# marvinli00/genie2

Hardware: AMD Instinct MI355X
Metric: denoise-steps/sec (N=256, T=1000, batch=8) (higher is better)
Workload: dtype f32 (pair-stack products as 3 f16 MFMAs on 2xf16-split operands, f32 accumulate); 1 GPU; unconditional N=256, T=1000, batch=8 per GPU, random-init base Denoiser (15.7M params), scale=0.6, reverse-loop steps 995..676; parallelism=replica per GPU x1, no data-path collective

## Files before the change

genie2_amd/csrc/common.h:

```cpp
#pragma once
#include <hip/hip_runtime.h>
#include <stdint.h>
#include "../../include/genie_hip.h"

typedef float f32x16 __attribute__((ext_vector_type(16)));
typedef float f32x4 __attribute__((ext_vector_type(4)));

#define GENIE_LN_EPS 1e-5f

#ifdef __HIPCC__

__device__ __forceinline__ f32x16 mfma_8k(const float4 a, const float4 b, f32x16 c) {
    c = __builtin_amdgcn_mfma_f32_32x32x2f32(a.x, b.x, c, 0, 0, 0);
    c = __builtin_amdgcn_mfma_f32_32x32x2f32(a.y, b.y, c, 0, 0, 0);
    c = __builtin_amdgcn_mfma_f32_32x32x2f32(a.z, b.z, c, 0, 0, 0);
    c = __builtin_amdgcn_mfma_f32_32x32x2f32(a.w, b.w, c, 0, 0, 0);
    return c;
}

__device__ __forceinline__ f32x16 zero16() {
    f32x16 z;
#pragma unroll
    for (int i = 0; i < 16; ++i) z[i] = 0.f;
    return z;
// ... 5 lines not shown
    return *reinterpret_cast<const float4*>(wp + ((size_t)(nb * KB + kb) * 64 + lane) * 4);
}

typedef float v4f __attribute__((ext_vector_type(4)));

__device__ __forceinline__ const float* wfrag_ptr(const float* __restrict__ wp, int KB, int nb, int kb, int lane) {
    return wp + ((size_t)(nb * KB + kb) * 64 + lane) * 4;
}
__device__ __forceinline__ void wf_issue(v4f& d, const float* p) {
    asm volatile("global_load_dwordx4 %0, %1, off" : "=v"(d) : "v"(p) : "memory");
}
template <int N>
__device__ __forceinline__ void wf_wait(v4f& a) {
    asm volatile("s_waitcnt vmcnt(%1)" : "+v"(a) : "i"(N) : "memory");
    __builtin_amdgcn_sched_barrier(0);
}
template <int N>
__device__ __forceinline__ void wf_wait(v4f& a, v4f& b) {
    asm volatile("s_waitcnt vmcnt(%2)" : "+v"(a), "+v"(b) : "i"(N) : "memory");
    __builtin_amdgcn_sched_barrier(0);
}
__device__ __forceinline__ f32x16 mfma_8k(const v4f a, const float4 b, f32x16 c) {
    c = __builtin_amdgcn_mfma_f32_32x32x2f32(a.x, b.x, c, 0, 0, 0);
    c = __builtin_amdgcn_mfma_f32_32x32x2f32(a.y, b.y, c, 0, 0, 0);
    c = __builtin_amdgcn_mfma_f32_32x32x2f32(a.z, b.z, c, 0, 0, 0);
    c = __builtin_amdgcn_mfma_f32_32x32x2f32(a.w, b.w, c, 0, 0, 0);
    return c;
}
__device__ __forceinline__ f32x16 mfma_8k(const float4 a, const v4f b, f32x16 c) {
    c = __builtin_amdgcn_mfma_f32_32x32x2f32(a.x, b.x, c, 0, 0, 0);
    c = __builtin_amdgcn_mfma_f32_32x32x2f32(a.y, b.y, c, 0, 0, 0);
    c = __builtin_amdgcn_mfma_f32_32x32x2f32(a.z, b.z, c, 0, 0, 0);
    c = __builtin_amdgcn_mfma_f32_32x32x2f32(a.w, b.w, c, 0, 0, 0);
    return c;
}

__device__ __forceinline__ float4 lfrag(const float* lds, int ld, int r0, int kb, int lane) {
    return *reinterpret_cast<const float4*>(lds + (r0 + (lane & 31)) * ld + kb * 8 + 4 * (lane >> 5));
}

__device__ __forceinline__ float4 lfrag_t(const float* lds, int ld, int i0, int kb, int lane) {
    const float* p = lds + (kb * 8 + 4 * (lane >> 5)) * ld + i0 + (lane & 31);
    return make_float4(p[0], p[ld], p[2 * ld], p[3 * ld]);
}

__device__ __forceinline__ float sigmoidf_(float x) { return 1.0f / (1.0f + expf(-x)); }

__device__ __forceinline__ void ln_rows_128(float* tile, int ld, const float* __restrict__ gamma,
                                            const float* __restrict__ beta, int tid) {
    const int row = tid >> 2, part = tid & 3;
    float* p = tile + row * ld + part * 32;
    float v[32];
#pragma unroll
    for (int q = 0; q < 8; ++q) {
        float4 t = *reinterpret_cast<float4*>(p + 4 * q);
        v[4 * q] = t.x; v[4 * q + 1] = t.y; v[4 * q + 2] = t.z; v[4 * q + 3] = t.w;
    }
    float s = 0.f;
#pragma unroll
    for (int q = 0; q < 32; ++q) s += v[q];
    s += __shfl_xor(s, 1); s += __shfl_xor(s, 2);
    const float mean = s * (1.0f / 128.0f);
    float ss = 0.f;
#pragma unroll
    for (int q = 0; q < 32; ++q) { float d = v[q] - mean; ss += d * d; }
    ss += __shfl_xor(ss, 1); ss += __shfl_xor(ss, 2);
    const float rstd = 1.0f / sqrtf(ss * (1.0f / 128.0f) + GENIE_LN_EPS);
#pragma unroll
    for (int q = 0; q < 8; ++q) {
        const int c = part * 32 + 4 * q;
        float4 g = *reinterpret_cast<const float4*>(gamma + c);
        float4 b = *reinterpret_cast<const float4*>(beta + c);
        float4 o;
        o.x = (v[4 * q] - mean) * rstd * g.x + b.x;
        o.y = (v[4 * q + 1] - mean) * rstd * g.y + b.y;
        o.z = (v[4 * q + 2] - mean) * rstd * g.z + b.z;
        o.w = (v[4 * q + 3] - mean) * rstd * g.w + b.w;
        *reinterpret_cast<float4*>(p + 4 * q) = o;
    }
}


__device__ __forceinline__ void rot_to_quat_dev(const float* r, int code, float* q) {
    const float xx = r[0], xy = r[1], xz = r[2], yx = r[3], yy = r[4], yz = r[5], zx = r[6], zy = r[7], zz = r[8];
    const float d0 = 1.f + xx + yy + zz, d1 = 1.f + xx - yy - zz, d2 = 1.f + yy - xx - zz, d3 = 1.f + zz - xx - yy;
    float c0, c1, c2, c3;
    if (d0 >= d1 && d0 >= d2 && d0 >= d3)      { c0 = d0;      c1 = zy - yz; c2 = xz - zx; c3 = yx - xy; }
    else if (d1 >= d2 && d1 >= d3)             { c0 = zy - yz; c1 = d1;      c2 = xy + yx; c3 = xz + zx; }
    else if (d2 >= d3)                         { c0 = xz - zx; c1 = xy + yx; c2 = d2;      c3 = yz + zy; }
    else                                       { c0 = yx - xy; c1 = xz + zx; c2 = yz + zy; c3 = d3; }
    const float inv = 1.0f / sqrtf(c0 * c0 + c1 * c1 + c2 * c2 + c3 * c3);
    q[0] = c0 * inv; q[1] = c1 * inv; q[2] = c2 * inv; q[3] = c3 * inv;
    if (code > 0) {
        const int m = (code - 1) >> 1;
        const bool want_neg = ((code - 1) & 1) != 0;
        const float comp = q[m];
        if ((comp < 0.f) != want_neg) { q[0] = -q[0]; q[1] = -q[1]; q[2] = -q[2]; q[3] = -q[3]; }
    }
}

#endif


enum KernelClass {
    KC_SINGLE_INPUT = 0, KC_GEMM_ROWS, KC_LAYERNORM, KC_PAIR_STATIC, KC_PAIR_INIT,
    KC_TRIMUL_PROJ, KC_TRIMUL_CONTRACT, KC_TRIMUL_OUT, KC_PAIR_TRANSITION,
    KC_IPA_BIAS, KC_IPA_PREP, KC_IPA_ATTN, KC_BB_UPDATE, KC_STRUCT_ROWS, KC_P_SAMPLE, KC_MISC, KC_PAIR_FUSED_A, KC_PAIR_FUSED_B,
    KC_TR_GEMM, KC_TR_EW, KC_TR_LN, KC_TR_TRANSPOSE, KC_TR_IPA, KC_TR_MISC,
    KC_TRIATT_PROJ, KC_TRIATT_CORE, KC_TRIATT_TRANSPOSE, KC_COUNT
};

struct HxTransW { const unsigned char* img; float *b1s, *b2s; float sx, c1, c2; };

struct HxTriW {
    const unsigned char *img_proj, *img_out;
    float *bias_proj, *bgs, *bzs;
    float sx, cpa, cpb, cg, cx, cgo, cz;
};
struct HxFusedW { const unsigned char* img; };
struct TriMulW {
    float *proj_w;
    float *proj_b;
    float *g_w, *g_b;
    float *z_w, *z_b;
    float *ln_in_g, *ln_in_b, *ln_out_g, *ln_out_b;
    HxTriW hx;
};
struct TriAttW {
    float *ln_g, *ln_b;
    float *wb;
    float *proj_w, *proj_b;
    float *out_w, *out_b;
    float sq, sk, sv;
};
struct PairLayerW {
    TriMulW out, in;
    TriAttW ta_start, ta_end;
    float *pt_ln_g, *pt_ln_b, *pt_w1, *pt_b1, *pt_w2, *pt_b2;
    HxTransW hx_pt;
    HxFusedW fa, fb;
};
struct StructLayerW {
    float *proj_w, *proj_b;
    float *head_w;
    float *out_w, *out_b;
    float *ln_ipa_g, *ln_ipa_b;
    float *t1_w, *t1_b, *t2_w, *t2_b, *t3_w, *t3_b;
    float *ln_tr_g, *ln_tr_b;
    float *bb_w, *bb_b;
};

struct HxGemmW { const float* w; const unsigned char* img; float inv_s; };

struct genie_train_ws;
struct genie_ctx {
    genie_dims_t d;
    genie_train_ws* train;
    int device;
    char err[512];

    bool have_weights;
    float* wdev;
    bool hx;
    unsigned char* hxdev;
    HxGemmW hxg[128]; int n_hxg;
    unsigned hx_launches;
    size_t wdev_floats;
    float *single_w;
    float *pij_w;
    float *relpos_t;
    float *templ_w;
    float *motif_w;
    float *ipa_bias_w, *ipa_bias_b;
    PairLayerW* pair;
    StructLayerW* st;

    bool have_tables;
    float *pos_tab, *chain_tab, *t_tab, *sched;
    int n_pos, n_chain;
    float* sched_host;

    int B, N, NP;
    bool have_feats, has_motif;
    int32_t *f_aatype, *f_rmask, *f_ridx, *f_cidx;
    float *f_pos;
    uint8_t *f_fsm, *f_fstm, *f_ifm;
    float *rmaskf;

    void* ws; size_t ws_bytes;
    float *p, *acm, *bcm, *xcm, *pstatic, *ipa_bias;
    float *spart;
    unsigned *pmax;
    float *xsingle, *s0, *s, *s1, *s2, *h1, *h2, *pij, *proj, *cat;
    float *kT, *v, *qp, *kpT, *vp;
    float *vf, *vmax;
    float *ta_tb, *ta_xn, *ta_qkvg;
    float *rots_w, *trans_w;
    int32_t* tsteps;
    float *loop_z;

    bool prof;
    struct ProfRec { int cls; hipEvent_t a, b; };
    ProfRec* prof_recs; int prof_n, prof_cap;
    double prof_ms[KC_COUNT]; int64_t prof_cnt[KC_COUNT];
    double train_gemm_flop;

    hipStream_t st2; hipEvent_t ev_fork, ev_join;
};

void launch_single_input(genie_ctx* h, hipStream_t st, const int32_t* timesteps);
void launch_gemm_rows(genie_ctx* h, hipStream_t st, const float* A, int lda, int M, int K,
                      const float* Wp, int Nout, const float* bias, const float* res, int ldr,
                      const float* rowmask, int relu, float* out, int ldo, int prof_class = KC_GEMM_ROWS);
void launch_layernorm_rows(genie_ctx* h, hipStream_t st, const float* in, float* out, int M, int C,
                           const float* g, const float* b);
void launch_pair_static(genie_ctx* h, hipStream_t st);
void launch_pair_init(genie_ctx* h, hipStream_t st, const float* trans, const float* rots,
                      const int8_t* codes);
void launch_trimul(genie_ctx* h, hipStream_t st, const TriMulW& w, bool outgoing);
void launch_pair_transition(genie_ctx* h, hipStream_t st, const PairLayerW& w);
void launch_triatt(genie_ctx* h, hipStream_t st, const TriAttW& w, bool starting);
void triatt_ws_floats(const genie_dims_t& d, int B, int N, size_t* tb, size_t* xn, size_t* qkvg);
bool launch_pair_stack_fused(genie_ctx* h, hipStream_t st, float* tap_trimul_out0, float* tap_layer0);
void launch_ipa_bias(genie_ctx* h, hipStream_t st);
void launch_ipa_prep(genie_ctx* h, hipStream_t st, int b0 = 0, int nb = -1);
void launch_ipa_attn(genie_ctx* h, hipStream_t st, int layer, const float* head_w, int b0 = 0, int nb = -1);
size_t ipa_vf_floats(const genie_dims_t& d, int B, int N);
bool ipa_attn_splits(const genie_ctx* h);
void launch_q_sample(genie_ctx* h, hipStream_t st, const float* x0, const float* z, const float* c0, const float* c1, float* trans_out);
void launch_training_loss(genie_ctx* h, hipStream_t st, const float* zp, const float* z, float w, float* losses, float* grad);
void launch_adam(hipStream_t st, size_t n, float* p, const float* g, float* m, float* v, double lr, double b1, double b2, double eps, int step);
void launch_any_nonzero(genie_ctx* h, hipStream_t st, const uint8_t* x, size_t n, unsigned* flag);
bool launch_struct_tail(genie_ctx* h, hipStream_t st, const StructLayerW& S, const float* trans_in, float* z_out, int b0 = 0, int nb = -1);
bool struct_tail_fused(const genie_ctx* h, const StructLayerW& S);
void launch_bb_update(genie_ctx* h, hipStream_t st, const StructLayerW& w, const float* trans_in,
                      float* z_out);
void launch_frenet(genie_ctx* h, hipStream_t st, int mode, int step, float scale, float* trans,
                   float* rots, const float* z, const float* eps);
void launch_reverse_step(genie_ctx* h, hipStream_t st, float a, float bz, float c_scaled, float* trans, float* rots, const float* z,
                         const float* eps);
void launch_fill_i32(genie_ctx* h, hipStream_t st, int32_t* p, int n, int v);
void train_ws_free(genie_ctx* h);

void prof_begin(genie_ctx* h, hipStream_t st, int cls);
void prof_end(genie_ctx* h, hipStream_t st);

struct ProfScope {
    genie_ctx* h; hipStream_t st; bool on;
    ProfScope(genie_ctx* h_, hipStream_t st_, int cls, bool enable = true) : h(h_), st(st_), on(enable && h_->prof) { if (on) prof_begin(h, st, cls); }
    ~ProfScope() { if (on) prof_end(h, st); }
};
```

genie2_amd/csrc/genie_api.hip:

```cpp
#include <stdio.h>
#include <stdlib.h>
#include <string.h>
#include <math.h>
#include <algorithm>
#include <cmath>
#include <new>
#include <string>
#include <vector>

#include "common.h"

void pair_kernels_init();
void pair_fused_kernels_init();
void single_kernels_init(const genie_dims_t& d, int n_max);
void launch_scale_copy(genie_ctx* h, hipStream_t st, const float* in, float* out, int n, float s);
size_t ipa_attn_lds(const genie_dims_t& d, int N);

static char g_create_err[512] = "";

void set_handle_free_error(const char* msg) { snprintf(g_create_err, sizeof g_create_err, "%s", msg); }

#define SET_ERR(h, ...) do { snprintf((h)->err, sizeof((h)->err), __VA_ARGS__); } while (0)
#define HIP_TRY(h, call) do { hipError_t e_ = (call); if (e_ != hipSuccess) { \
    SET_ERR(h, "%s failed: %s (%s:%d)", #call, hipGetErrorString(e_), __FILE__, __LINE__); return GENIE_E_HIP; } } while (0)

static const char* kKernelNames[KC_COUNT] = {
    "single_input", "gemm_rows", "layernorm_rows", "pair_static", "pair_init", "trimul_proj", "trimul_contract",
    "trimul_out", "pair_transition", "ipa_bias", "ipa_prep", "ipa_attn", "bb_update", "struct_rows", "p_sample_frenet", "misc",
    "pair_fused_a", "pair_fused_b", "train_gemm", "train_elementwise", "train_layernorm", "train_transpose", "train_ipa", "train_misc",
    "tri_att_proj", "tri_att_core", "tri_att_transpose"};

void prof_begin(genie_ctx* h, hipStream_t st, int cls) {
    if (h->prof_n == h->prof_cap) {
        const int nc = h->prof_cap ? h->prof_cap * 2 : 1024;
        h->prof_recs = (genie_ctx::ProfRec*)realloc(h->prof_recs, nc * sizeof(genie_ctx::ProfRec));
        h->prof_cap = nc;
    }
    genie_ctx::ProfRec& r = h->prof_recs[h->prof_n];
    r.cls = cls;
    (void)hipEventCreate(&r.a);
    (void)hipEventCreate(&r.b);
    (void)hipEventRecord(r.a, st);
}
void prof_end(genie_ctx* h, hipStream_t st) {
    (void)hipEventRecord(h->prof_recs[h->prof_n].b, st);
    h->prof_n++;
}

static int single_in(const genie_dims_t& d) { return d.c_pos_emb + d.c_chain_emb + d.c_timestep_emb + 23; }
static int ipa_proj_n(const genie_dims_t& d) {
    return d.n_head_ipa * (3 * d.c_hidden_ipa + 3 * d.n_qk_point + 3 * (d.n_qk_point + d.n_v_point));
}
static int ipa_cat_n(const genie_dims_t& d) { return d.n_head_ipa * (d.c_p + d.c_hidden_ipa + 4 * d.n_v_point); }

static const char* check_dims(const genie_dims_t& d) {
    if (d.c_p != 128 || d.c_hidden_mul != 128) return "kernels are specialised for c_p == c_hidden_mul == 128";
    if (d.c_s % 8 || d.c_s > 512) return "c_s must be a multiple of 8 and <= 512";
    if (d.template_dist_n_bin > 40 || d.template_dist_n_bin < 1) return "template_dist_n_bin must be in [1, 40]";
    if (d.n_head_ipa > 16) return "n_head_ipa must be <= 16";
    if (d.pair_transition_n < 1 || d.n_timestep < 1 || d.relpos_k < 0) return "bad dims";
    if (d.n_structure_layer < 1 || d.n_structure_block < 1 || d.n_pair_transform_layer < 0) return "bad layer counts";
    if ((d.n_head_ipa * d.c_hidden_ipa) % 4 || ipa_cat_n(d) % 4 || ipa_proj_n(d) % 4) return "IPA widths must be multiples of 4";
    if (d.n_head_tri < 0) return "n_head_tri must be >= 0";
    if (d.n_head_tri > 0 && d.c_hidden_tri_att != 16 && d.c_hidden_tri_att != 32) return "c_hidden_tri_att must be 16 or 32";
    if (d.n_head_tri > 0 && d.n_head_tri * d.c_hidden_tri_att != 128) return "n_head_tri * c_hidden_tri_att must be 128 (4 heads of 32 or 8 of 16)";
    return nullptr;
}

size_t genie_weight_count(const genie_dims_t* dp) {
    const genie_dims_t& d = *dp;
    size_t n = 0;
    const size_t cs = d.c_s, cp = d.c_p, ch = d.c_hidden_mul;
    n += cs * single_in(d);
    n += 2 * cp * cs + cp * (2 * d.relpos_k + 3) + cp * (d.template_dist_n_bin + 6) + cp * (d.template_dist_n_bin + 2);
    const size_t tm = 4 * (ch * cp + ch) + (cp * cp + cp) + (cp * ch + cp) + 2 * cp + 2 * ch;
    const size_t pt = 2 * cp + (d.pair_transition_n * cp * cp + d.pair_transition_n * cp) + (cp * d.pair_transition_n * cp + cp);
    const size_t hc = (size_t)d.n_head_tri * d.c_hidden_tri_att;
    const size_t ta = d.n_head_tri > 0 ? 2 * cp + d.n_head_tri * cp + 3 * hc * cp + (cp * hc + cp) + (hc * cp + hc) : 0;
    n += (size_t)d.n_pair_transform_layer * (2 * tm + 2 * ta + pt);
    const size_t H = d.n_head_ipa, C = d.c_hidden_ipa, Pq = d.n_qk_point, Pv = d.n_v_point;
    size_t sl = H;
    sl += (H * C) * cs + H * C + (2 * H * C) * cs + 2 * H * C + (3 * H * Pq) * cs + 3 * H * Pq + (3 * H * (Pq + Pv)) * cs + 3 * H * (Pq + Pv);
    sl += H * cp + H + cs * ipa_cat_n(d) + cs;
    sl += 2 * cs + 3 * (cs * cs + cs) + 2 * cs + 6 * cs + 6;
    n += (size_t)d.n_structure_layer * sl;
    return n;
}

int genie_create(const genie_dims_t* dims, int device, genie_handle_t* out) {
    if (!dims || !out) { snprintf(g_create_err, sizeof g_create_err, "genie_create: null argument"); return GENIE_E_ARG; }
    if (const char* m = check_dims(*dims)) { snprintf(g_create_err, sizeof g_create_err, "genie_create: %s", m); return GENIE_E_ARG; }
    int ndev = 0;
    if (hipGetDeviceCount(&ndev) != hipSuccess || device < 0 || device >= ndev) {
        snprintf(g_create_err, sizeof g_create_err, "genie_create: no HIP device %d (found %d)", device, ndev);
        return GENIE_E_HIP;
    }
    genie_ctx* h = new (std::nothrow) genie_ctx();
    if (!h) return GENIE_E_NOMEM;
    memset(h, 0, sizeof(*h));
    h->d = *dims;
    h->device = device;
    if (hipSetDevice(device) != hipSuccess) { delete h; snprintf(g_create_err, sizeof g_create_err, "hipSetDevice failed"); return GENIE_E_HIP; }
    h->pair = new PairLayerW[dims->n_pair_transform_layer > 0 ? dims->n_pair_transform_layer : 1]();
    h->st = new StructLayerW[dims->n_structure_layer]();
    pair_kernels_init();
    pair_fused_kernels_init();
    {
        const char* m = getenv("GENIE_MATH");
        h->hx = !(m && !strcmp(m, "f32"));
    }
    {
        int lo = 0, hi = 0;
        (void)hipDeviceGetStreamPriorityRange(&lo, &hi);
        if (hipStreamCreateWithPriority(&h->st2, hipStreamNonBlocking, hi) != hipSuccess) h->st2 = nullptr;
    }
    if (h->st2 && (hipEventCreateWithFlags(&h->ev_fork, hipEventDisableTiming) != hipSuccess ||
                   hipEventCreateWithFlags(&h->ev_join, hipEventDisableTiming) != hipSuccess)) {
        (void)hipStreamDestroy(h->st2);
        h->st2 = nullptr;
    }
    *out = h;
    return GENIE_OK;
}

static void free_batch(genie_ctx* h) {
    if (h->ws) { (void)hipFree(h->ws); h->ws = nullptr; h->ws_bytes = 0; }
    h->have_feats = false;
}

void genie_destroy(genie_handle_t h) {
    if (!h) return;
    (void)hipSetDevice(h->device);
    free_batch(h);
    train_ws_free(h);
    if (h->wdev) (void)hipFree(h->wdev);
    if (h->hxdev) (void)hipFree(h->hxdev);
    if (h->pos_tab) (void)hipFree(h->pos_tab);
    free(h->sched_host);
    for (int i = 0; i < h->prof_n; ++i) { (void)hipEventDestroy(h->prof_recs[i].a); (void)hipEventDestroy(h->prof_recs[i].b); }
    free(h->prof_recs);
    if (h->st2) { (void)hipStreamSynchronize(h->st2); (void)hipEventDestroy(h->ev_fork); (void)hipEventDestroy(h->ev_join); (void)hipStreamDestroy(h->st2); }
    delete[] h->pair;
    delete[] h->st;
    delete h;
}

const char* genie_last_error(genie_handle_t h) { return h ? h->err : g_create_err; }
size_t genie_workspace_bytes(genie_handle_t h) { return h ? h->ws_bytes : 0; }

namespace {
struct Img {
    std::vector<float> data;
    size_t add(size_t n) {
        const size_t off = (data.size() + 63) & ~(size_t)63;
        data.resize(off + n, 0.f);
        return off;
    }
    size_t raw(const float* src, size_t n) { const size_t o = add(n); memcpy(&data[o], src, n * sizeof(float)); return o; }
    size_t pack(const float* W, int rows, int cols) {
        const int NB = (rows + 31) / 32, KB = (cols + 7) / 8;
        const size_t o = add((size_t)NB * KB * 256);
        float* p = &data[o];
        for (int nb = 0; nb < NB; ++nb)
            for (int kb = 0; kb < KB; ++kb)
                for (int lane = 0; lane < 64; ++lane)
                    for (int e = 0; e < 4; ++e) {
                        const int r = nb * 32 + (lane & 31), k = kb * 8 + 4 * (lane >> 5) + e;
                        p[(((size_t)nb * KB + kb) * 64 + lane) * 4 + e] = (r < rows && k < cols) ? W[(size_t)r * cols + k] : 0.f;
                    }
        return o;
    }
};
uint16_t f2h(float f) {
    uint32_t x; memcpy(&x, &f, 4);
    const uint16_t sign = (uint16_t)((x >> 16) & 0x8000);
    x &= 0x7FFFFFFFu;
    if (x >= 0x7F800000u) return (uint16_t)(sign | (x > 0x7F800000u ? 0x7E00 : 0x7C00));
    if (x >= 0x477FF000u) return (uint16_t)(sign | 0x7C00);
    if (x < 0x38800000u) {
        float a; memcpy(&a, &x, 4);
        return (uint16_t)(sign | (uint16_t)nearbyintf(a * 16777216.0f));
    }
    const uint32_t mant = x & 0x7FFFFFu, rem = mant & 0x1FFFu;
    uint32_t r = (((x >> 23) - 112u) << 10) | (mant >> 13);
    if (rem > 0x1000u || (rem == 0x1000u && (r & 1u))) ++r;
    return (uint16_t)(sign | r);
}
float h2f(uint16_t v) {
    const int e = (v >> 10) & 31, m = v & 1023;
    float r = e == 0 ? ldexpf((float)m, -24) : e == 31 ? (m ? NAN : INFINITY) : ldexpf((float)(1024 + m), e - 25);
    return (v & 0x8000) ? -r : r;
}
float p2floor(double x) { return (x > 0 && std::isfinite(x)) ? (float)ldexp(1.0, (int)floor(log2(x))) : 1.0f; }
struct HxImg {
    std::vector<uint16_t> d;
    size_t begin() { d.resize((d.size() + 127) & ~(size_t)127); return d.size() * 2; }
    template <class F> void unit(F get) {
        const size_t o = d.size();
        d.resize(o + 1024);
        for (int lane = 0; lane < 64; ++lane)
            for (int e = 0; e < 8; ++e) {
                const float v = get(lane & 31, lane >> 5, e);
                const uint16_t hi = f2h(v);
                d[o + lane * 8 + e] = hi;
                d[o + 512 + lane * 8 + e] = f2h(v - h2f(hi));
            }
    }
};
double max_abs(const float* w, size_t n) { double m = 0; for (size_t i = 0; i < n; ++i) m = std::max(m, (double)fabsf(w[i])); return m; }
double hx_bound(const float* W, const float* b, int rows, int cols) {
    double m = 0;
    for (int r = 0; r < rows; ++r) {
        double ss = 0;
        for (int k = 0; k < cols; ++k) ss += (double)W[(size_t)r * cols + k] * W[(size_t)r * cols + k];
        m = std::max(m, sqrt(ss * cols) + fabs((double)b[r]));
    }
    return m;
}
constexpr float HX_SX = 1024.0f;

struct Cur {
    const float* p; size_t left;
    const float* take(size_t n) { if (n > left) { left = 0; return nullptr; } const float* r = p; p += n; left -= n; return r; }
};
void fold_ln(std::vector<float>& W, std::vector<float>& b, int rows, int cols, const float* g, const float* beta) {
    for (int r = 0; r < rows; ++r) {
        double acc = b[r];
        for (int k = 0; k < cols; ++k) acc += (double)W[(size_t)r * cols + k] * beta[k];
        b[r] = (float)acc;
        for (int k = 0; k < cols; ++k) W[(size_t)r * cols + k] *= g[k];
    }
}
std::vector<float> vcat(std::initializer_list<std::pair<const float*, size_t>> parts) {
    std::vector<float> v;
    for (auto& pr : parts) v.insert(v.end(), pr.first, pr.first + pr.second);
    return v;
}
}

int genie_load_weights(genie_handle_t h, const float* blob, size_t n_floats) {
    if (!h || !blob) return GENIE_E_ARG;
    const genie_dims_t& d = h->d;
    if (n_floats != genie_weight_count(&d)) {
        SET_ERR(h, "genie_load_weights: got %zu floats, dims need %zu", n_floats, genie_weight_count(&d));
        return GENIE_E_ARG;
    }
    HIP_TRY(h, hipSetDevice(h->device));
    const size_t cs = d.c_s, cp = d.c_p, ch = d.c_hidden_mul;
    Cur c{blob, n_floats};
    Img img;
    HxImg hx;
    std::vector<std::pair<float**, size_t>> fix;
    std::vector<std::pair<const unsigned char**, size_t>> hxfix;
    auto slot = [&](float** s, size_t off) { fix.push_back({s, off}); };
    struct GemmFix { float** slot; size_t hx_off; float inv_s; };
    std::vector<GemmFix> gfix;
    auto pack_gemm = [&](float** s, const float* W, int rows, int cols) {
        slot(s, img.pack(W, rows, cols));
        const float sw = p2floor(16384.0 / max_abs(W, (size_t)rows * cols));
        gfix.push_back({s, hx.begin(), 1.0f / sw});
        const int NB = (rows + 31) / 32, KC = (cols + 15) / 16;
        for (int nb = 0; nb < NB; ++nb)
            for (int kc = 0; kc < KC; ++kc)
                hx.unit([&](int j, int hh, int e) {
                    const int r = 32 * nb + j, k = 16 * kc + 8 * hh + e;
                    return (r < rows && k < cols) ? W[(size_t)r * cols + k] * sw : 0.f; });
    };

    size_t ones_off, zeros_off;
    {
        std::vector<float> one(512, 1.f), zero(512, 0.f);
        ones_off = img.raw(one.data(), one.size());
        zeros_off = img.raw(zero.data(), zero.size());
    }
    const int nsi = single_in(d);
    pack_gemm(&h->single_w, c.take(cs * nsi), (int)cs, nsi);
    {
        const float* wi = c.take(cp * cs);
        const float* wj = c.take(cp * cs);
        auto v = vcat({{wi, cp * cs}, {wj, cp * cs}});
        pack_gemm(&h->pij_w, v.data(), (int)(2 * cp), (int)cs);
    }
    {
        const int nr = 2 * d.relpos_k + 3;
        const float* w = c.take(cp * nr);
        std::vector<float> t((size_t)nr * cp);
        for (int o = 0; o < (int)cp; ++o) for (int k = 0; k < nr; ++k) t[(size_t)k * cp + o] = w[(size_t)o * nr + k];
        slot(&h->relpos_t, img.raw(t.data(), t.size()));
    }
    {
        const int kt = d.template_dist_n_bin + 6, km = d.template_dist_n_bin + 2;
        const float* wt = c.take(cp * kt);
        const float* wm = c.take(cp * km);
        std::vector<float> t((size_t)cp * 48, 0.f), m((size_t)cp * 48, 0.f);
// ... 128 lines not shown
    {
        auto ck = [](int kc, int hh, int e) { return 16 * kc + (e & 3) + 8 * (e >> 2) + 4 * hh; };
        auto emit_O = [&](const TmSave& t) {
            for (int which = 0; which < 2; ++which)
                for (int st = 0; st < 2; ++st)
                    for (int obl = 0; obl < 2; ++obl)
                        for (int kc = 0; kc < 8; ++kc) {
                            const std::vector<float>& m = which == 0 ? t.zw : t.gw;
                            const float sc = which == 0 ? t.szo : t.sgo;
                            const size_t ob = 2 * st + obl;
                            hx.unit([&](int i, int hh, int e) { return m[(32 * ob + i) * cp + ck(kc, hh, e)] * sc; });
                        }
        };
        auto emit_T = [&](const PtSave& t) {
            const size_t nh = (size_t)d.pair_transition_n * cp;
            for (size_t hb = 0; hb < nh / 32; ++hb) {
                for (int kc = 0; kc < 8; ++kc)
                    hx.unit([&](int i, int hh, int e) { return t.w1v[(32 * hb + i) * cp + ck(kc, hh, e)] * t.s1; });
                for (int cc = 0; cc < 2; ++cc)
                    for (int ob = 0; ob < 4; ++ob)
                        hx.unit([&](int j, int hh, int e) { return t.w2[(size_t)(32 * ob + j) * nh + 32 * hb + ck(cc, hh, e)] * t.s2; });
            }
        };
        auto emit_P = [&](const TmSave& t) {
            for (size_t pass = 0; pass < 8; ++pass)
                for (int kc = 0; kc < 8; ++kc) {
                    hx.unit([&](int i, int hh, int e) { return t.w[(32 * pass + i) * cp + ck(kc, hh, e)] * t.sp; });
                    hx.unit([&](int i, int hh, int e) { return t.w[(2 * ch + 32 * pass + i) * cp + ck(kc, hh, e)] * t.sg; });
                }
        };
        for (int l = 0; l < d.n_pair_transform_layer; ++l) {
            hxfix.push_back({&h->pair[l].fa.img, hx.begin()});
            emit_O(tm_save[2 * l]); emit_P(tm_save[2 * l + 1]);
            hxfix.push_back({&h->pair[l].fb.img, hx.begin()});
            emit_O(tm_save[2 * l + 1]); emit_T(pt_save[l]);
            if (l + 1 < d.n_pair_transform_layer) emit_P(tm_save[2 * l + 2]);
        }
    }
    const size_t H = d.n_head_ipa, C = d.c_hidden_ipa, Pq = d.n_qk_point, Pv = d.n_v_point;
    const size_t ncat = ipa_cat_n(d);
    std::vector<float> wb_all, bb_all;
    for (int l = 0; l < d.n_structure_layer; ++l) {
        StructLayerW& S = h->st[l];
        const float* hw = c.take(H);
        const float* q_w = c.take(H * C * cs);            const float* q_b = c.take(H * C);
        const float* kv_w = c.take(2 * H * C * cs);       const float* kv_b = c.take(2 * H * C);
        const float* qp_w = c.take(3 * H * Pq * cs);      const float* qp_b = c.take(3 * H * Pq);
        const float* kp_w = c.take(3 * H * (Pq + Pv) * cs); const float* kp_b = c.take(3 * H * (Pq + Pv));
        const float* b_w = c.take(H * cp);                const float* b_b = c.take(H);
        const float* o_w = c.take(cs * ncat);             const float* o_b = c.take(cs);
        const float* li_g = c.take(cs); const float* li_b = c.take(cs);
        const float* t1w = c.take(cs * cs); const float* t1b = c.take(cs);
        const float* t2w = c.take(cs * cs); const float* t2b = c.take(cs);
        const float* t3w = c.take(cs * cs); const float* t3b = c.take(cs);
        const float* lt_g = c.take(cs); const float* lt_b = c.take(cs);
        const float* bw = c.take(6 * cs); const float* bbs = c.take(6);
        if (!bbs) { SET_ERR(h, "genie_load_weights: blob too short"); return GENIE_E_ARG; }
        slot(&S.head_w, img.raw(hw, H));
        auto w = vcat({{q_w, H * C * cs}, {kv_w, 2 * H * C * cs}, {qp_w, 3 * H * Pq * cs}, {kp_w, 3 * H * (Pq + Pv) * cs}});
        auto bv = vcat({{q_b, H * C}, {kv_b, 2 * H * C}, {qp_b, 3 * H * Pq}, {kp_b, 3 * H * (Pq + Pv)}});
        pack_gemm(&S.proj_w, w.data(), ipa_proj_n(d), (int)cs);
        slot(&S.proj_b, img.raw(bv.data(), bv.size()));
        wb_all.insert(wb_all.end(), b_w, b_w + H * cp);
        bb_all.insert(bb_all.end(), b_b, b_b + H);
        pack_gemm(&S.out_w, o_w, (int)cs, (int)ncat); slot(&S.out_b, img.raw(o_b, cs));
        slot(&S.ln_ipa_g, img.raw(li_g, cs)); slot(&S.ln_ipa_b, img.raw(li_b, cs));
        pack_gemm(&S.t1_w, t1w, (int)cs, (int)cs); slot(&S.t1_b, img.raw(t1b, cs));
        pack_gemm(&S.t2_w, t2w, (int)cs, (int)cs); slot(&S.t2_b, img.raw(t2b, cs));
        pack_gemm(&S.t3_w, t3w, (int)cs, (int)cs); slot(&S.t3_b, img.raw(t3b, cs));
        slot(&S.ln_tr_g, img.raw(lt_g, cs)); slot(&S.ln_tr_b, img.raw(lt_b, cs));
        slot(&S.bb_w, img.raw(bw, 6 * cs)); slot(&S.bb_b, img.raw(bbs, 6));
    }
    pack_gemm(&h->ipa_bias_w, wb_all.data(), (int)(d.n_structure_layer * H), (int)cp);
    slot(&h->ipa_bias_b, img.raw(bb_all.data(), bb_all.size()));
    if (c.left != 0) { SET_ERR(h, "genie_load_weights: %zu floats left over", c.left); return GENIE_E_ARG; }

    if (h->wdev) { (void)hipFree(h->wdev); h->wdev = nullptr; }
    img.add(64);
    HIP_TRY(h, hipMalloc((void**)&h->wdev, img.data.size() * sizeof(float)));
    HIP_TRY(h, hipMemcpy(h->wdev, img.data.data(), img.data.size() * sizeof(float), hipMemcpyHostToDevice));
    h->wdev_floats = img.data.size();
    for (auto& f : fix) *f.first = h->wdev + f.second;
    if (h->hxdev) { (void)hipFree(h->hxdev); h->hxdev = nullptr; }
    hx.begin();
    HIP_TRY(h, hipMalloc((void**)&h->hxdev, hx.d.size() * 2 + 256));
    HIP_TRY(h, hipMemcpy(h->hxdev, hx.d.data(), hx.d.size() * 2, hipMemcpyHostToDevice));
    for (auto& f : hxfix) *f.first = h->hxdev + f.second;
    h->n_hxg = 0;
    const int hxg_cap = (int)(sizeof(h->hxg) / sizeof(h->hxg[0]));
    if ((int)gfix.size() > hxg_cap) { SET_ERR(h, "genie_load_weights: %zu row-GEMM weights exceed the %d hx image slots", gfix.size(), hxg_cap); return GENIE_E_ARG; }
    for (auto& g : gfix) h->hxg[h->n_hxg++] = HxGemmW{*g.slot, h->hxdev + g.hx_off, g.inv_s};
    h->have_weights = true;
    return GENIE_OK;
}

int genie_set_tables(genie_handle_t h, const float* pos_tab, int n_pos, const float* chain_tab, int n_chain,
                     const float* t_tab, const float* sched) {
    if (!h || !pos_tab || !chain_tab || !t_tab || !sched || n_pos < 1 || n_chain < 1) return GENIE_E_ARG;
    HIP_TRY(h, hipSetDevice(h->device));
    const genie_dims_t& d = h->d;
    const size_t T1 = d.n_timestep + 1;
    const size_t a = (size_t)n_pos * d.c_pos_emb, b = (size_t)n_chain * d.c_chain_emb, c = T1 * d.c_timestep_emb, s = 4 * T1;
    if (h->pos_tab) (void)hipFree(h->pos_tab);
    HIP_TRY(h, hipMalloc((void**)&h->pos_tab, (a + b + c + s) * sizeof(float)));
    h->chain_tab = h->pos_tab + a;
    h->t_tab = h->chain_tab + b;
    h->sched = h->t_tab + c;
    HIP_TRY(h, hipMemcpy(h->pos_tab, pos_tab, a * sizeof(float), hipMemcpyHostToDevice));
    HIP_TRY(h, hipMemcpy(h->chain_tab, chain_tab, b * sizeof(float), hipMemcpyHostToDevice));
    HIP_TRY(h, hipMemcpy(h->t_tab, t_tab, c * sizeof(float), hipMemcpyHostToDevice));
    HIP_TRY(h, hipMemcpy(h->sched, sched, s * sizeof(float), hipMemcpyHostToDevice));
    free(h->sched_host);
    h->sched_host = (float*)malloc(s * sizeof(float));
    memcpy(h->sched_host, sched, s * sizeof(float));
    h->n_pos = n_pos;
    h->n_chain = n_chain;
    h->have_tables = true;
    return GENIE_OK;
}

__global__ void k_mask_to_float(const int32_t* m, float* f, int n) {
    const int i = blockIdx.x * blockDim.x + threadIdx.x;
    if (i < n) f[i] = (float)m[i];
}

int genie_prepare_features(genie_handle_t h, genie_stream_t stream, int B, int N, const genie_features_t* f) {
    if (!h || !f || B < 1 || N < 2) return GENIE_E_ARG;
    if (!h->have_weights) { SET_ERR(h, "genie_prepare_features: weights not loaded"); return GENIE_E_STATE; }
    const genie_dims_t& d = h->d;
    if (ipa_attn_lds(d, N) > 160 * 1024) { SET_ERR(h, "N = %d exceeds the attention kernel's LDS budget", N); return GENIE_E_ARG; }
    if ((size_t)24 * N * sizeof(float) > 160 * 1024) { SET_ERR(h, "N = %d exceeds the Frenet kernel's LDS budget (96 B per residue)", N); return GENIE_E_ARG; }
    {
        const size_t np = (size_t)((N + 31) / 32 * 32);
        const size_t pair_bytes = (size_t)B * np * np * d.c_p * sizeof(float);
        if (pair_bytes >= ((size_t)1 << 31)) {
            SET_ERR(h, "batch %d x N %d: a pair tensor of %zu bytes exceeds the 2 GiB the kernels address; split the batch", B, N, pair_bytes);
            return GENIE_E_ARG;
        }
    }
    HIP_TRY(h, hipSetDevice(h->device));
    hipStream_t st = (hipStream_t)stream;
    const int NP = (N + 31) / 32 * 32;
    const size_t M = (size_t)B * N, P = M * N;
    const size_t cs = d.c_s, cp = d.c_p;
    const int H = d.n_head_ipa, C = d.c_hidden_ipa, Pq = d.n_qk_point, Pv = d.n_v_point;
    const int ldx = (single_in(d) + 7) / 8 * 8;

    struct Seg { void** p; size_t bytes; };
    std::vector<Seg> segs;
    auto want = [&](void* pp, size_t bytes) { segs.push_back({(void**)pp, (bytes + 255) & ~(size_t)255}); };
    want(&h->p, P * cp * 4); want(&h->pstatic, P * cp * 4);
    want(&h->acm, (size_t)B * cp * NP * NP * 4); want(&h->bcm, (size_t)B * cp * NP * NP * 4); want(&h->xcm, (size_t)B * cp * NP * NP * 4);
    want(&h->ipa_bias, (size_t)d.n_structure_layer * H * P * 4);
    want(&h->xsingle, M * ldx * 4);
    want(&h->s0, M * cs * 4); want(&h->s, M * cs * 4); want(&h->s1, M * cs * 4); want(&h->s2, M * cs * 4);
    want(&h->h1, M * cs * 4); want(&h->h2, M * cs * 4);
    want(&h->pij, M * 2 * cp * 4); want(&h->proj, M * ipa_proj_n(d) * 4); want(&h->cat, M * ipa_cat_n(d) * 4);
    want(&h->kT, M * H * C * 4); want(&h->v, M * H * C * 4); want(&h->qp, M * H * Pq * 3 * 4);
    want(&h->kpT, M * H * Pq * 3 * 4); want(&h->vp, M * H * Pv * 3 * 4);
    want(&h->vf, ipa_vf_floats(d, B, N) * 4); want(&h->vmax, M * 2 * 4);
    want(&h->rots_w, M * 9 * 4); want(&h->trans_w, M * 3 * 4); want(&h->loop_z, M * 3 * 4);
    want(&h->tsteps, (size_t)B * 4); want(&h->rmaskf, M * 4); want(&h->pmax, 4); want(&h->spart, 3 * M * cs * 4);
    want(&h->f_aatype, M * 20 * 4); want(&h->f_rmask, M * 4); want(&h->f_ridx, M * 4); want(&h->f_cidx, M * 4);
    want(&h->f_pos, M * 3 * 4); want(&h->f_fsm, M); want(&h->f_fstm, P); want(&h->f_ifm, M);
    if (d.n_head_tri > 0) {
        size_t ntb, nxn, nq;
        triatt_ws_floats(d, B, N, &ntb, &nxn, &nq);
        want(&h->ta_tb, ntb * 4); want(&h->ta_xn, nxn * 4); want(&h->ta_qkvg, nq * 4);
    }
    size_t total = 0;
    for (auto& s : segs) total += s.bytes;
    if (total > h->ws_bytes) {
        free_batch(h);
        hipError_t e = hipMalloc(&h->ws, total);
        if (e != hipSuccess) { SET_ERR(h, "workspace hipMalloc(%zu MB) failed: %s", total >> 20, hipGetErrorString(e)); return GENIE_E_NOMEM; }
        h->ws_bytes = total;
    }
    size_t off = 0;
    for (auto& s : segs) { *s.p = (char*)h->ws + off; off += s.bytes; }
    h->B = B; h->N = N; h->NP = NP;

    HIP_TRY(h, hipMemcpyAsync(h->f_aatype, f->aatype, M * 20 * 4, hipMemcpyDeviceToDevice, st));
    HIP_TRY(h, hipMemcpyAsync(h->f_pos, f->atom_positions, M * 3 * 4, hipMemcpyDeviceToDevice, st));
    HIP_TRY(h, hipMemcpyAsync(h->f_rmask, f->residue_mask, M * 4, hipMemcpyDeviceToDevice, st));
    HIP_TRY(h, hipMemcpyAsync(h->f_ridx, f->residue_index, M * 4, hipMemcpyDeviceToDevice, st));
    HIP_TRY(h, hipMemcpyAsync(h->f_cidx, f->chain_index, M * 4, hipMemcpyDeviceToDevice, st));
    HIP_TRY(h, hipMemcpyAsync(h->f_fsm, f->fixed_sequence_mask, M, hipMemcpyDeviceToDevice, st));
    HIP_TRY(h, hipMemcpyAsync(h->f_fstm, f->fixed_structure_mask, P, hipMemcpyDeviceToDevice, st));
    HIP_TRY(h, hipMemcpyAsync(h->f_ifm, f->interface_mask, M, hipMemcpyDeviceToDevice, st));
    hipLaunchKernelGGL(k_mask_to_float, dim3((unsigned)((M + 255) / 256)), dim3(256), 0, st, h->f_rmask, h->rmaskf, (int)M);
    HIP_TRY(h, hipMemsetAsync(h->acm, 0, (size_t)B * cp * NP * NP * 4, st));
    HIP_TRY(h, hipMemsetAsync(h->vf, 0, ipa_vf_floats(d, B, N) * 4, st));
    HIP_TRY(h, hipMemsetAsync(h->bcm, 0, (size_t)B * cp * NP * NP * 4, st));
    single_kernels_init(d, N);
    {
        unsigned any = 0;
        HIP_TRY(h, hipMemsetAsync(h->pmax, 0, sizeof(unsigned), st));
        launch_any_nonzero(h, st, h->f_fstm, P, h->pmax);
        HIP_TRY(h, hipMemcpyAsync(&any, h->pmax, sizeof(unsigned), hipMemcpyDeviceToHost, st));
        HIP_TRY(h, hipStreamSynchronize(st));
        h->has_motif = any != 0;
    }
    launch_pair_static(h, st);
    HIP_TRY(h, hipGetLastError());
    h->have_feats = true;
    return GENIE_OK;
}

static int denoise_internal(genie_ctx* h, hipStream_t st, const float* trans, const float* rots, const int32_t* ts_dev,
                            const int8_t* codes, float* z_out, const genie_taps_t* taps) {
    const genie_dims_t& d = h->d;
    const int B = h->B, N = h->N, M = B * N;
    const size_t P = (size_t)M * N;
    const int cs = d.c_s, cp = d.c_p;
    const int ldx = (single_in(d) + 7) / 8 * 8;
    auto d2d = [&](void* dst, const void* src, size_t bytes) { return hipMemcpyAsync(dst, src, bytes, hipMemcpyDeviceToDevice, st); };

    h->hx_launches = 1;
    launch_scale_copy(h, st, trans, h->trans_w, M * 3, d.rescale);
    HIP_TRY(h, d2d(h->rots_w, rots, (size_t)M * 9 * 4));

    launch_single_input(h, st, ts_dev);
    launch_gemm_rows(h, st, h->xsingle, ldx, M, ldx, h->single_w, cs, nullptr, nullptr, 0, h->rmaskf, 0, h->s0, cs);
    if (taps && taps->s) HIP_TRY(h, d2d(taps->s, h->s0, (size_t)M * cs * 4));

    launch_gemm_rows(h, st, h->s0, cs, M, cs, h->pij_w, 2 * cp, nullptr, nullptr, 0, nullptr, 0, h->pij, 2 * cp);
    launch_pair_init(h, st, h->trans_w, h->rots_w, codes);
    if (taps && taps->p_init) HIP_TRY(h, d2d(taps->p_init, h->p, P * cp * 4));

    const bool fused = launch_pair_stack_fused(h, st, taps ? taps->p_trimul_out0 : nullptr, taps ? taps->p_layer0 : nullptr);
    for (int l = 0; l < (fused ? 0 : d.n_pair_transform_layer); ++l) {
        launch_trimul(h, st, h->pair[l].out, true);
        if (l == 0 && taps && taps->p_trimul_out0) HIP_TRY(h, d2d(taps->p_trimul_out0, h->p, P * cp * 4));
        launch_trimul(h, st, h->pair[l].in, false);
        if (d.n_head_tri > 0) {
            launch_triatt(h, st, h->pair[l].ta_start, true);
            launch_triatt(h, st, h->pair[l].ta_end, false);
            if (l == 0 && taps && taps->p_tri_att0) HIP_TRY(h, d2d(taps->p_tri_att0, h->p, P * cp * 4));
        }
        launch_pair_transition(h, st, h->pair[l]);
        if (l == 0 && taps && taps->p_layer0) HIP_TRY(h, d2d(taps->p_layer0, h->p, P * cp * 4));
    }
    if (taps && taps->p) HIP_TRY(h, d2d(taps->p, h->p, P * cp * 4));

    launch_ipa_bias(h, st);
    HIP_TRY(h, d2d(h->s, h->s0, (size_t)M * cs * 4));
    if (taps && taps->states) HIP_TRY(h, d2d(taps->states, h->s0, (size_t)M * cs * 4));
    int n_state = 1;
    const int nproj = ipa_proj_n(d), ncat = ipa_cat_n(d);
    bool split = h->st2 && B >= 2 && M >= 1024 && ipa_attn_splits(h) && !getenv("GENIE_NO_STRUCT_SPLIT");
    for (int l = 0; split && l < d.n_structure_layer; ++l) split = struct_tail_fused(h, h->st[l]);
    const int n_half = split ? 2 : 1;
    const int n_layers = d.n_structure_block * d.n_structure_layer;
    hipStream_t hstream[2] = {st, h->st2};
    if (split) {
        HIP_TRY(h, hipEventRecord(h->ev_fork, st));
        HIP_TRY(h, hipStreamWaitEvent(h->st2, h->ev_fork, 0));
    }
    for (int half = 0; half < n_half; ++half) {
        hipStream_t hs = hstream[half];
        const int b0 = (int)((long long)B * half / n_half), nb = (int)((long long)B * (half + 1) / n_half) - b0;
        const size_t r0 = (size_t)b0 * N, nr = (size_t)nb * N;
        int li = 0;
        for (int blk = 0; blk < d.n_structure_block; ++blk) {
            for (int l = 0; l < d.n_structure_layer; ++l, ++li) {
                const StructLayerW& S = h->st[l];
                const bool last = li == n_layers - 1;
                launch_gemm_rows(h, hs, h->s + r0 * cs, cs, (int)nr, cs, S.proj_w, nproj, S.proj_b, nullptr, 0, nullptr, 0, h->proj + r0 * nproj, nproj);
                launch_ipa_prep(h, hs, b0, nb);
                launch_ipa_attn(h, hs, l, S.head_w, b0, nb);
                if (li == 0 && taps && taps->ipa_cat0) HIP_TRY(h, hipMemcpyAsync(taps->ipa_cat0 + r0 * ncat, h->cat + r0 * ncat, nr * ncat * 4, hipMemcpyDeviceToDevice, hs));
                auto state_tap = [&]() -> hipError_t {
                    return (taps && taps->states) ? hipMemcpyAsync(taps->states + (size_t)(1 + li) * M * cs + r0 * cs, h->s + r0 * cs, nr * cs * 4, hipMemcpyDeviceToDevice, hs)
                                                  : hipSuccess;
                };
                if (launch_struct_tail(h, hs, S, last ? trans : nullptr, last ? z_out : nullptr, b0, nb)) { HIP_TRY(h, state_tap()); continue; }
                launch_gemm_rows(h, hs, h->cat, ncat, M, ncat, S.out_w, cs, S.out_b, h->s, cs, nullptr, 0, h->s1, cs);
                launch_layernorm_rows(h, hs, h->s1, h->s2, M, cs, S.ln_ipa_g, S.ln_ipa_b);
                launch_gemm_rows(h, hs, h->s2, cs, M, cs, S.t1_w, cs, S.t1_b, nullptr, 0, nullptr, 1, h->h1, cs);
                launch_gemm_rows(h, hs, h->h1, cs, M, cs, S.t2_w, cs, S.t2_b, nullptr, 0, nullptr, 1, h->h2, cs);
                launch_gemm_rows(h, hs, h->h2, cs, M, cs, S.t3_w, cs, S.t3_b, h->s2, cs, nullptr, 0, h->s1, cs);
                launch_layernorm_rows(h, hs, h->s1, h->s, M, cs, S.ln_tr_g, S.ln_tr_b);
                launch_bb_update(h, hs, S, last ? trans : nullptr, last ? z_out : nullptr);
                HIP_TRY(h, state_tap());
            }
        }
    }
    if (split) {
        for (int q = 1; q < n_half; ++q) {
            HIP_TRY(h, hipEventRecord(h->ev_join, hstream[q]));
            HIP_TRY(h, hipStreamWaitEvent(st, h->ev_join, 0));
        }
    }
    (void)n_state;
    if (taps && taps->s_final) HIP_TRY(h, d2d(taps->s_final, h->s, (size_t)M * cs * 4));
    if (taps && taps->rots_out) HIP_TRY(h, d2d(taps->rots_out, h->rots_w, (size_t)M * 9 * 4));
    if (taps && taps->trans_out) launch_scale_copy(h, st, h->trans_w, taps->trans_out, M * 3, 1.0f / d.rescale);
    HIP_TRY(h, hipGetLastError());
    return GENIE_OK;
}

static int check_ready(genie_ctx* h, const char* who) {
    if (!h) return GENIE_E_ARG;
    if (!h->have_weights || !h->have_tables || !h->have_feats) {
        SET_ERR(h, "%s: call genie_load_weights, genie_set_tables and genie_prepare_features first", who);
        return GENIE_E_STATE;
    }
    if (hipSetDevice(h->device) != hipSuccess) { SET_ERR(h, "hipSetDevice failed"); return GENIE_E_HIP; }
    return GENIE_OK;
}

int genie_denoise(genie_handle_t h, genie_stream_t stream, const float* trans, const float* rots, const int32_t* timesteps,
                  const int8_t* quat_codes, float* z_out, const genie_taps_t* taps) {
    if (int rc = check_ready(h, "genie_denoise")) return rc;
    if (!trans || !rots || !timesteps || !z_out) { SET_ERR(h, "genie_denoise: null tensor"); return GENIE_E_ARG; }
    return denoise_internal(h, (hipStream_t)stream, trans, rots, timesteps, quat_codes, z_out, taps);
}

int genie_frenet(genie_handle_t h, genie_stream_t stream, const float* trans, float* rots_out) {
    if (!h || !h->have_feats) { if (h) SET_ERR(h, "genie_frenet: no batch bound"); return h ? GENIE_E_STATE : GENIE_E_ARG; }
    if (!trans || !rots_out) return GENIE_E_ARG;
    HIP_TRY(h, hipSetDevice(h->device));
    launch_frenet(h, (hipStream_t)stream, 0, 0, 0.f, const_cast<float*>(trans), rots_out, nullptr, nullptr);
    HIP_TRY(h, hipGetLastError());
    return GENIE_OK;
}

int genie_adam_step(genie_stream_t stream, size_t n, float* p, const float* g, float* m, float* v, double lr, double beta1, double beta2,
                    double eps, int step) {
    if (!p || !g || !m || !v || step < 1) return GENIE_E_ARG;
    if (n == 0) return GENIE_OK;
    launch_adam((hipStream_t)stream, n, p, g, m, v, lr, beta1, beta2, eps, step);
    return hipGetLastError() == hipSuccess ? GENIE_OK : GENIE_E_HIP;
}

int genie_q_sample(genie_handle_t h, genie_stream_t stream, const float* x0, const float* z, const float* c_x0, const float* c_z,
                   float* trans_out, float* rots_out) {
    if (!h || !h->have_feats) { if (h) SET_ERR(h, "genie_q_sample: no batch bound"); return h ? GENIE_E_STATE : GENIE_E_ARG; }
    if (!x0 || !z || !c_x0 || !c_z || !trans_out || !rots_out) { SET_ERR(h, "genie_q_sample: null tensor"); return GENIE_E_ARG; }
    HIP_TRY(h, hipSetDevice(h->device));
    launch_q_sample(h, (hipStream_t)stream, x0, z, c_x0, c_z, trans_out);
    launch_frenet(h, (hipStream_t)stream, 0, 0, 0.f, trans_out, rots_out, nullptr, nullptr);
    HIP_TRY(h, hipGetLastError());
    return GENIE_OK;
}

int genie_training_loss(genie_handle_t h, genie_stream_t stream, const float* z_pred, const float* z, float condition_loss_weight,
                        float* losses_out, float* grad_out) {
    if (!h || !h->have_feats) { if (h) SET_ERR(h, "genie_training_loss: no batch bound"); return h ? GENIE_E_STATE : GENIE_E_ARG; }
    if (!z_pred || !z || !losses_out) { SET_ERR(h, "genie_training_loss: null tensor"); return GENIE_E_ARG; }
    HIP_TRY(h, hipSetDevice(h->device));
    launch_training_loss(h, (hipStream_t)stream, z_pred, z, condition_loss_weight, losses_out, grad_out);
    HIP_TRY(h, hipGetLastError());
    return GENIE_OK;
}

int genie_p_sample(genie_handle_t h, genie_stream_t stream, int step, float scale, float* trans_inout, float* rots_out,
                   const float* z, const float* eps) {
    if (int rc = check_ready(h, "genie_p_sample")) return rc;
    if (step < 1 || step > h->d.n_timestep || !trans_inout || !rots_out || !z) { SET_ERR(h, "genie_p_sample: bad argument"); return GENIE_E_ARG; }
    launch_frenet(h, (hipStream_t)stream, 1, step, scale, trans_inout, rots_out, z, eps);
    HIP_TRY(h, hipGetLastError());
    return GENIE_OK;
}

int genie_sample_loop(genie_handle_t h, genie_stream_t stream, float scale, const float* noise, const int8_t* quat_codes,
                      int first_step, int last_step, float* trans_io, float* rots_io, float* record) {
    if (int rc = check_ready(h, "genie_sample_loop")) return rc;
    const int T = h->d.n_timestep;
    if (!noise || !trans_io || !rots_io || first_step > T || last_step < 1 || first_step < last_step) {
        SET_ERR(h, "genie_sample_loop: bad argument");
        return GENIE_E_ARG;
    }
    hipStream_t st = (hipStream_t)stream;
    const size_t n3 = (size_t)h->B * h->N * 3, nn = (size_t)h->B * h->N * h->N;
    if (first_step == T) {
        HIP_TRY(h, hipMemcpyAsync(trans_io, noise, n3 * 4, hipMemcpyDeviceToDevice, st));
        launch_frenet(h, st, 0, 0, 0.f, trans_io, rots_io, nullptr, nullptr);
    }
    int it = 0;
    for (int step = first_step; step >= last_step; --step, ++it) {
        launch_fill_i32(h, st, h->tsteps, h->B, step);
        const int8_t* codes = quat_codes ? quat_codes + (size_t)it * nn : nullptr;
        if (int rc = denoise_internal(h, st, trans_io, rots_io, h->tsteps, codes, h->loop_z, nullptr)) return rc;
        const float* eps = (step == 1) ? nullptr : noise + (size_t)(T - step + 1) * n3;
        launch_frenet(h, st, 1, step, scale, trans_io, rots_io, h->loop_z, eps);
        if (record) HIP_TRY(h, hipMemcpyAsync(record + (size_t)it * n3, trans_io, n3 * 4, hipMemcpyDeviceToDevice, st));
    }
    HIP_TRY(h, hipGetLastError());
    return GENIE_OK;
}

int genie_reverse_step(genie_handle_t h, genie_stream_t stream, float a, float bz, float c_scaled, float* trans_inout, float* rots_out,
                       const float* z, const float* eps) {
    if (int rc = check_ready(h, "genie_reverse_step")) return rc;
    if (!trans_inout || !rots_out || !z) { SET_ERR(h, "genie_reverse_step: null tensor"); return GENIE_E_ARG; }
    if (!std::isfinite(a) || !std::isfinite(bz) || !std::isfinite(c_scaled)) {
        SET_ERR(h, "genie_reverse_step: non-finite coefficient (a = %g, bz = %g, c_scaled = %g)", a, bz, c_scaled);
        return GENIE_E_ARG;
    }
    launch_reverse_step(h, (hipStream_t)stream, a, bz, c_scaled, trans_inout, rots_out, z, eps);
    HIP_TRY(h, hipGetLastError());
    return GENIE_OK;
}

int genie_sample_loop_steps(genie_handle_t h, genie_stream_t stream, int n_iter, const int32_t* steps, const float* coef, const float* noise,
                            const int8_t* quat_codes, int start_from_noise, float* trans_io, float* rots_io, float* record) {
    if (int rc = check_ready(h, "genie_sample_loop_steps")) return rc;
    const int T = h->d.n_timestep;
    if (n_iter < 1) { SET_ERR(h, "genie_sample_loop_steps: n_iter = %d, needs at least 1", n_iter); return GENIE_E_ARG; }
    if (!steps || !coef || !trans_io || !rots_io) { SET_ERR(h, "genie_sample_loop_steps: null steps, coef, trans_io or rots_io"); return GENIE_E_ARG; }
    if (!noise && (start_from_noise || n_iter > 1)) {
        SET_ERR(h, "genie_sample_loop_steps: null noise (needed for the initial state and for every iteration but the last)");
        return GENIE_E_ARG;
    }
    for (int i = 0; i < n_iter; ++i) {
        if (steps[i] < 1 || steps[i] > T) { SET_ERR(h, "genie_sample_loop_steps: steps[%d] = %d outside 1..%d", i, steps[i], T); return GENIE_E_ARG; }
        if (i && steps[i] >= steps[i - 1]) {
            SET_ERR(h, "genie_sample_loop_steps: steps not strictly decreasing (steps[%d] = %d after %d)", i, steps[i], steps[i - 1]);
            return GENIE_E_ARG;
        }
        for (int k = 0; k < 3; ++k)
            if (!std::isfinite(coef[3 * i + k])) { SET_ERR(h, "genie_sample_loop_steps: non-finite coefficient coef[%d][%d]", i, k); return GENIE_E_ARG; }
    }
    hipStream_t st = (hipStream_t)stream;
    const size_t n3 = (size_t)h->B * h->N * 3, nn = (size_t)h->B * h->N * h->N;
    if (start_from_noise) {
        HIP_TRY(h, hipMemcpyAsync(trans_io, noise, n3 * 4, hipMemcpyDeviceToDevice, st));
        launch_frenet(h, st, 0, 0, 0.f, trans_io, rots_io, nullptr, nullptr);
    }
    for (int it = 0; it < n_iter; ++it) {
        launch_fill_i32(h, st, h->tsteps, h->B, steps[it]);
        const int8_t* codes = quat_codes ? quat_codes + (size_t)it * nn : nullptr;
        if (int rc = denoise_internal(h, st, trans_io, rots_io, h->tsteps, codes, h->loop_z, nullptr)) return rc;
        const float* eps = (it == n_iter - 1) ? nullptr : noise + (size_t)(it + 1) * n3;
        launch_reverse_step(h, st, coef[3 * it], coef[3 * it + 1], coef[3 * it + 2], trans_io, rots_io, h->loop_z, eps);
        if (record) HIP_TRY(h, hipMemcpyAsync(record + (size_t)it * n3, trans_io, n3 * 4, hipMemcpyDeviceToDevice, st));
    }
    HIP_TRY(h, hipGetLastError());
    return GENIE_OK;
}

int genie_set_math(genie_handle_t h, int mode) {
    if (!h || (mode != GENIE_MATH_F32 && mode != GENIE_MATH_HX)) return GENIE_E_ARG;
    h->hx = mode == GENIE_MATH_HX;
    return GENIE_OK;
}
int genie_get_math(genie_handle_t h) { return h && h->hx ? GENIE_MATH_HX : GENIE_MATH_F32; }

int genie_profile_enable(genie_handle_t h, int enable) {
    if (!h) return GENIE_E_ARG;
    h->prof = enable != 0;
    return GENIE_OK;
}

int genie_profile_read(genie_handle_t h, const char** names, double* total_ms, int64_t* launches, int cap) {
    if (!h) return GENIE_E_ARG;
    (void)hipSetDevice(h->device);
    for (int i = 0; i < h->prof_n; ++i) {
        genie_ctx::ProfRec& r = h->prof_recs[i];
        (void)hipEventSynchronize(r.b);
        float ms = 0.f;
        if (hipEventElapsedTime(&ms, r.a, r.b) == hipSuccess) { h->prof_ms[r.cls] += ms; h->prof_cnt[r.cls] += 1; }
        (void)hipEventDestroy(r.a);
        (void)hipEventDestroy(r.b);
    }
    h->prof_n = 0;
    int n = 0;
    for (int k = 0; k < KC_COUNT && n < cap; ++k) {
        if (names) names[n] = kKernelNames[k];
        if (total_ms) total_ms[n] = h->prof_ms[k];
        if (launches) launches[n] = h->prof_cnt[k];
        ++n;
    }
    for (int k = 0; k < KC_COUNT; ++k) { h->prof_ms[k] = 0; h->prof_cnt[k] = 0; }
    return n;
}
```

genie2_amd/csrc/genie_train.hip:

```cpp
#include <math.h>
#include <stdio.h>
#include <string.h>
#include <vector>
#include "common.h"
#include "train.h"

namespace {
struct TriOff { size_t ap_w, ap_b, ag_w, ag_b, bp_w, bp_b, bg_w, bg_b, g_w, g_b, z_w, z_b, lni_g, lni_b, lno_g, lno_b; };
struct PairOff { TriOff out, in; size_t ln_g, ln_b, w1, b1, w2, b2; };
struct StructOff {
    size_t head, q_w, q_b, kv_w, kv_b, qp_w, qp_b, kvp_w, kvp_b, b_w, b_b, o_w, o_b, ln1_g, ln1_b, t1w, t1b, t2w, t2b, t3w, t3b, ln2_g, ln2_b,
        bb_w, bb_b;
};
struct Offs { size_t single_w, wi, wj, wrel, wt, wm; std::vector<PairOff> pair; std::vector<StructOff> st; size_t total; };

Offs make_offsets(const genie_dims_t& d) {
    Offs o;
    size_t c = 0;
    auto take = [&](size_t n) { const size_t r = c; c += n; return r; };
    const size_t cs = d.c_s, cp = d.c_p, ch = d.c_hidden_mul;
    const size_t nsi = d.c_pos_emb + d.c_chain_emb + d.c_timestep_emb + 23;
    o.single_w = take(cs * nsi);
    o.wi = take(cp * cs); o.wj = take(cp * cs);
    o.wrel = take(cp * (2 * d.relpos_k + 3));
// ... 21 lines not shown
        s.kv_w = take(2 * H * C * cs); s.kv_b = take(2 * H * C);
        s.qp_w = take(3 * H * Pq * cs); s.qp_b = take(3 * H * Pq);
        s.kvp_w = take(3 * H * (Pq + Pv) * cs); s.kvp_b = take(3 * H * (Pq + Pv));
        s.b_w = take(H * cp); s.b_b = take(H);
        s.o_w = take(cs * ncat); s.o_b = take(cs);
        s.ln1_g = take(cs); s.ln1_b = take(cs);
        s.t1w = take(cs * cs); s.t1b = take(cs); s.t2w = take(cs * cs); s.t2b = take(cs); s.t3w = take(cs * cs); s.t3b = take(cs);
        s.ln2_g = take(cs); s.ln2_b = take(cs);
        s.bb_w = take(6 * cs); s.bb_b = take(6);
        o.st.push_back(s);
    }
    o.total = c;
    return o;
}

struct Arena {
    char* base = nullptr; size_t off = 0, peak = 0; bool dry = true;
    float* f(size_t n) {
        const size_t bytes = (n * sizeof(float) + 255) & ~(size_t)255;
        float* r = dry ? nullptr : reinterpret_cast<float*>(base + off);
        off += bytes;
        if (off > peak) peak = off;
        return r;
    }
};

struct TriSave { float *xhat, *rstd, *ap, *ag, *bp, *bg, *acm, *bcm, *xhat_o, *rstd_o, *u, *g; };
struct TransSave { float *xhat, *rstd, *h; unsigned* hmask; };
struct PairSave { TriSave out, in; TransSave tr; };
struct StructSave {
    float *s_in, *q, *kv, *qplin, *kvplin, *qp, *kp, *vp, *att, *cat, *xhat1, *rstd1, *s2, *h1, *h2, *xhat2, *rstd2, *s4, *bb, *R, *T;
};
}

struct genie_train_ws { void* kept = nullptr; size_t kept_bytes = 0; void* tmp = nullptr; size_t tmp_bytes = 0; FoldEntry* fold_tab = nullptr; int fold_n = 0; };

void train_ws_free(genie_ctx* h) {
    if (!h->train) return;
    if (h->train->kept) (void)hipFree(h->train->kept);
    if (h->train->tmp) (void)hipFree(h->train->tmp);
    if (h->train->fold_tab) (void)hipFree(h->train->fold_tab);
    delete h->train;
    h->train = nullptr;
}

#define TR_ERR(...) do { snprintf(h->err, sizeof(h->err), __VA_ARGS__); } while (0)

namespace {
struct Run {
    genie_ctx* h; hipStream_t st; bool dry; int terms;
    const float* W; float* G;
    Arena K, T;
    int B, N, M; long long P;

    void gemm(const GemmP& p) {
        if (dry) return;
        h->train_gemm_flop += 2.0 * p.M * p.N * (double)p.K * p.batch;
        ProfScope ps_(h, st, KC_TR_GEMM);
        launch_gemm(st, p, terms);
    }
    void lin_fwd(const float* X, long long ldx, long long R, int K, size_t w, long long b_off, int O, float* Y, int mode = 0, bool relu = false) {
        GemmP p{X, W + w, Y, b_off >= 0 ? W + b_off : nullptr, (int)R, O, K, ldx, 1, 1, K, O, 1, 1, 1, 0, 0, 0, 0, 0, 0, 1, 1.0f, mode};
        p.relu = relu ? 1 : 0;
        gemm(p);
    }
    void lin_bwd_x(const float* dY, long long R, int O, size_t w, int K, float* dX, long long lddx, bool accumulate, const float* relu_out = nullptr,
                   const unsigned* relu_mask = nullptr) {
        GemmP p{dY, W + w, dX, nullptr, (int)R, K, O, O, 1, K, 1, lddx, 1, 1, 1, 0, 0, 0, 0, 0, 0, 1, 1.0f, accumulate ? 1 : 0};
        if (relu_mask) p.mask_in = relu_mask;
        else p.gate = relu_out;
        gemm(p);
    }
    void lin_bwd_x_ptr(const float* dY, long long R, int O, const float* Wc, int K, float* dX, long long lddx) {
        GemmP p{dY, Wc, dX, nullptr, (int)R, K, O, O, 1, K, 1, lddx, 1, 1, 1, 0, 0, 0, 0, 0, 0, 1, 1.0f, 0};
        gemm(p);
    }
    void lin_bwd_w(const float* dY, long long R, int O, const float* X, long long ldx, int K, size_t w, long long b_off) {
        if (!G) return;
        GemmP p{dY, X, G + w, nullptr, O, K, (int)R, 1, O, ldx, 1, K, 1, 1, 1, 0, 0, 0, 0, 0, 0, gemm_splits(O, K, R, 1), 1.0f, 2};
        p.asum = b_off >= 0 ? G + b_off : nullptr;
        gemm(p);
    }
    void lin_fwd_ln(const float* Xhat, long long R, int K, int O, float* Y, const float* fold, bool relu = false, const float* fold_b = nullptr,
                    unsigned* mask_out = nullptr) {
        GemmP p{Xhat, fold, Y, fold_b ? fold_b : fold ? fold + (size_t)O * K : nullptr, (int)R, O, K, K, 1, 1, K, O, 1, 1, 1, 0, 0, 0, 0, 0, 0, 1, 1.0f, 0};
        p.relu = relu ? 1 : 0;
        p.mask_out = mask_out;
        gemm(p);
    }
    void lin_fwd_ln_cat(const float* Xhat, long long R, int K, int O, int nb, float* const* Y, const float* fold, const float* fold_b) {
        GemmP p{Xhat, fold, Y[0], fold_b, (int)R, nb * O, K, K, 1, 1, K, O, 1, 1, 1, 0, 0, 0, 0, 0, 0, 1, 1.0f, 0};
        p.cblk = O; p.cblk_m = 0;
        for (int k = 0; k < nb; ++k) p.ctab[k] = Y[k] - Y[0];
        gemm(p);
    }
    void lin_bwd_w_ln(const float* dY, long long R, int O, const float* Xhat, int K, size_t w, size_t b_off, size_t g_off, size_t beta_off, long long lddy = 0) {
        if (!G) return;
        GemmP p{dY, Xhat, G + w, nullptr, O, K, (int)R, 1, lddy ? lddy : O, K, 1, K, 1, 1, 1, 0, 0, 0, 0, 0, 0, gemm_splits(O, K, R, 1), 1.0f, 2};
        p.asum = G + b_off;
        p.colscale = W + g_off;
        gemm(p);
    }
    void lin_bwd_w_ln_cat(const float* dYcat, long long R, int O, int nb, const float* Xhat, int K, const size_t* w, const size_t* b_off, size_t g_off,
                          size_t beta_off) {
        if (!G) return;
        GemmP p{dYcat, Xhat, G, nullptr, nb * O, K, (int)R, 1, (long long)nb * O, K, 1, K, 1, 1, 1, 0, 0, 0, 0, 0, 0, gemm_splits((long long)nb * O, K, R, 1), 1.0f, 2};
        p.asum = G;
        p.colscale = W + g_off;
        p.cblk = O; p.cblk_m = 1;
        for (int k = 0; k < nb; ++k) { p.ctab[k] = (long long)w[k]; p.atab[k] = (long long)b_off[k]; }
        gemm(p);
    }
    void ln_fwd(const float* x, size_t g, size_t b, float* y, float* xhat, float* rstd, long long R, int C) {
        if (dry) return;
        ProfScope ps_(h, st, KC_TR_LN);
        launch_ln_fwd(st, x, W + g, W + b, y, xhat, rstd, R, C);
    }
    void ln_bwd(const float* dy, const float* xhat, const float* rstd, size_t g, size_t b, float* dx, long long R, int C, bool accumulate) {
        if (dry) return;
        ProfScope ps_(h, st, KC_TR_LN);
        launch_ln_bwd(st, dy, xhat, rstd, W + g, dx, R, C, accumulate ? 1 : 0, G ? G + g : nullptr, G ? G + b : nullptr);
    }
    template <class F> void ew(long long n, F f) { if (dry) return; ProfScope ps_(h, st, KC_TR_EW); launch_ew(st, n, f); }
    void transpose(const float* in, float* out, int Bt, int R, int C, bool to_cm) { if (dry) return; ProfScope ps_(h, st, KC_TR_TRANSPOSE); launch_transpose(st, in, out, Bt, R, C, to_cm); }
};
}

static int train_run(genie_ctx* h, hipStream_t st, bool dry, const float* Wd, float* Gd, const float* trans0, const float* rots0,
                     const int32_t* ts_dev, const float* z_target, const int8_t* codes, float cond_w, const genie_train_opts_t& opt,
                     float* losses_out, float* z_pred_out, size_t* kept_bytes, size_t* tmp_bytes, const float* dz_in = nullptr,
                     float* dtrans_out = nullptr) {
    const genie_dims_t& d = h->d;
    const Offs O = make_offsets(d);
    Run r;
    r.h = h; r.st = st; r.dry = dry; r.terms = opt.fast_math == 1 ? 1 : (opt.fast_math == 2 ? 2 : 3); r.W = Wd; r.G = Gd;
    r.B = h->B; r.N = h->N; r.M = h->B * h->N; r.P = (long long)r.M * h->N;
    r.K.dry = r.T.dry = dry;
    if (!dry) { r.K.base = (char*)h->train->kept; r.T.base = (char*)h->train->tmp; }
    const int B = r.B, N = r.N, M = r.M;
    const long long P = r.P;
    const int cs = d.c_s, cp = d.c_p, ch = d.c_hidden_mul;
    const int nh = d.pair_transition_n * cp;
    const int H = d.n_head_ipa, C = d.c_hidden_ipa, Pq = d.n_qk_point, Pv = d.n_v_point;
    const int ncat = H * (cp + C + 4 * Pv);
    const int nbin = d.template_dist_n_bin, kt = nbin + 6, km = nbin + 2, kr = 2 * d.relpos_k + 3, nf = kt + km + kr;
    const int nsi = d.c_pos_emb + d.c_chain_emb + d.c_timestep_emb + 23, ldx = (nsi + 7) / 8 * 8;
    const bool train = opt.train_mode != 0;
    const float r_tri = train ? opt.tri_dropout : 0.f, r_ipa = train ? opt.ipa_dropout : 0.f, r_tr = train ? opt.transition_dropout : 0.f;
    const uint32_t seed = opt.seed;
    const float* rm = h->rmaskf;
    const int L = d.n_pair_transform_layer, SL = d.n_structure_layer;
    Arena& K = r.K; Arena& T = r.T;

    if (!dry) launch_single_input(h, st, ts_dev);
    const float* xs = h->xsingle;
    float* tr = K.f((size_t)M * 3);
    { const float sc = d.rescale; r.ew((long long)M * 3, [=] __device__(long long i) { tr[i] = trans0[i] * sc; }); }
    float* s0 = K.f((size_t)M * cs);
    r.lin_fwd(xs, ldx, M, nsi, O.single_w, -1, cs, s0);
    r.ew((long long)M * cs, [=] __device__(long long i) { s0[i] *= rm[i / cs]; });
    float* Fm = K.f((size_t)P * nf);
    if (!dry) launch_pair_features(st, tr, rots0, codes, rm, h->f_fstm, h->f_fsm, h->f_pos, h->f_ridx, h->f_cidx, Fm, B, N, nbin,
                                   d.template_dist_min, d.template_dist_step, d.relpos_k);
    float* z = K.f((size_t)P * cp);
    {
        size_t mark = T.off;
        float* pi = T.f((size_t)M * cp); float* pj = T.f((size_t)M * cp);
        r.lin_fwd(s0, cs, M, cs, O.wi, -1, cp, pi);
        r.lin_fwd(s0, cs, M, cs, O.wj, -1, cp, pj);
        r.lin_fwd(Fm, nf, P, kt, O.wt, -1, cp, z, 0);
        r.lin_fwd(Fm + kt, nf, P, km, O.wm, -1, cp, z, 1);
        r.lin_fwd(Fm + kt + km, nf, P, kr, O.wrel, -1, cp, z, 1);
        if (cp % 4 == 0) {
            r.ew(P * cp / 4, [=] __device__(long long e4) {
                const long long e = e4 * 4, row = e / cp; const int c = (int)(e % cp);
                const int j = (int)(row % N); const long long bi = row / N; const long long b = bi / N;
                const float m = rm[bi] * rm[b * N + j];
                float4 zv = *reinterpret_cast<const float4*>(z + e);
                const float4 a = *reinterpret_cast<const float4*>(pi + bi * cp + c), bb = *reinterpret_cast<const float4*>(pj + (b * N + j) * cp + c);
                zv.x = (zv.x + a.x + bb.x) * m; zv.y = (zv.y + a.y + bb.y) * m; zv.z = (zv.z + a.z + bb.z) * m; zv.w = (zv.w + a.w + bb.w) * m;
                *reinterpret_cast<float4*>(z + e) = zv;
            });
        } else
        r.ew(P * cp, [=] __device__(long long e) {
            const long long row = e / cp; const int c = (int)(e % cp);
            const int j = (int)(row % N); const long long bi = row / N; const long long b = bi / N;
            z[e] = (z[e] + pi[bi * cp + c] + pj[(b * N + j) * cp + c]) * (rm[bi] * rm[b * N + j]);
        });
        T.off = mark;
    }
    std::vector<PairSave> ps(L);
    std::vector<FoldEntry> fold_plan;
    std::vector<size_t> fold_tri((size_t)L * 2 * 7), fold_tr(L);
    size_t fold_floats = 0;
    {
        auto plan = [&](size_t w, size_t b, size_t g, size_t be, int Oo, int Kk) {
            fold_plan.push_back(FoldEntry{(long long)w, (long long)b, (long long)g, (long long)be, (long long)fold_floats,
                                          (long long)(fold_floats + (size_t)Oo * Kk), -1, Oo, Kk});
            const size_t at = fold_floats;
            fold_floats += ((size_t)Oo * Kk + Oo + 63) / 64 * 64;
            return at;
        };
        auto plan5 = [&](const size_t (&w)[5], const size_t (&b)[5], size_t g, size_t be, int Oo, int Kk, size_t* f) {
            const size_t raw0 = fold_floats + ((size_t)5 * Oo * Kk + 5 * Oo + 63) / 64 * 64;
            for (int k = 0; k < 5; ++k) {
                f[k] = fold_floats + (size_t)k * Oo * Kk;
                fold_plan.push_back(FoldEntry{(long long)w[k], (long long)b[k], (long long)g, (long long)be, (long long)f[k],
                                              (long long)(fold_floats + (size_t)5 * Oo * Kk + (size_t)k * Oo), (long long)(raw0 + (size_t)k * Oo * Kk), Oo, Kk});
            }
            f[6] = raw0;
            fold_floats = raw0 + (size_t)5 * Oo * Kk;
        };
        for (int l = 0; l < L; ++l) {
            for (int dir = 0; dir < 2; ++dir) {
                const TriOff& t = dir == 0 ? O.pair[l].out : O.pair[l].in;
                size_t* f = &fold_tri[((size_t)l * 2 + dir) * 7];
                if (ch == cp) {
                    const size_t w5[5] = {t.ap_w, t.ag_w, t.bp_w, t.bg_w, t.g_w}, b5[5] = {t.ap_b, t.ag_b, t.bp_b, t.bg_b, t.g_b};
                    plan5(w5, b5, t.lni_g, t.lni_b, ch, cp, f);
                } else {
                    f[0] = plan(t.ap_w, t.ap_b, t.lni_g, t.lni_b, ch, cp); f[1] = plan(t.ag_w, t.ag_b, t.lni_g, t.lni_b, ch, cp);
                    f[2] = plan(t.bp_w, t.bp_b, t.lni_g, t.lni_b, ch, cp); f[3] = plan(t.bg_w, t.bg_b, t.lni_g, t.lni_b, ch, cp);
                    f[4] = plan(t.g_w, t.g_b, t.lni_g, t.lni_b, cp, cp);
                }
                f[5] = plan(t.z_w, t.z_b, t.lno_g, t.lno_b, cp, ch);
            }
            fold_tr[l] = plan(O.pair[l].w1, O.pair[l].b1, O.pair[l].ln_g, O.pair[l].ln_b, nh, cp);
        }
    }
    float* foldbuf = K.f(fold_floats);
    if (!dry && !fold_plan.empty()) {
        genie_train_ws* tw = h->train;
        if (tw->fold_n != (int)fold_plan.size()) {
            if (tw->fold_tab) (void)hipFree(tw->fold_tab);
            (void)hipMalloc((void**)&tw->fold_tab, fold_plan.size() * sizeof(FoldEntry));
            (void)hipMemcpyAsync(tw->fold_tab, fold_plan.data(), fold_plan.size() * sizeof(FoldEntry), hipMemcpyHostToDevice, st);
            (void)hipStreamSynchronize(st);
            tw->fold_n = (int)fold_plan.size();
        }
        ProfScope ps_(h, st, KC_TR_EW);
        launch_fold_ln_table(st, Wd, foldbuf, tw->fold_tab, tw->fold_n, nh > ch ? (nh > cp ? nh : cp) : (ch > cp ? ch : cp));
    }
    const bool cmf = train_cm_fusable(ch);
    auto tri_fwd = [&](const TriOff& t, TriSave& s, bool outgoing, uint32_t tag, const size_t* fo) {
        s.xhat = K.f(P * cp); s.rstd = K.f(P); s.ag = K.f(P * ch); s.bg = K.f(P * ch);
        if (!cmf) { s.ap = K.f(P * ch); s.bp = K.f(P * ch); }
        s.acm = K.f(P * ch); s.bcm = K.f(P * ch); s.xhat_o = K.f(P * ch); s.rstd_o = K.f(P); s.u = K.f(P * cp); s.g = K.f(P * cp);
        size_t mark = T.off;
        if (cmf) { s.ap = T.f(P * ch); s.bp = T.f(P * ch); }
        r.ln_fwd(z, t.lni_g, t.lni_b, nullptr, s.xhat, s.rstd, P, cp);
        auto fw = [&](int k) -> const float* { return dry ? nullptr : foldbuf + fo[k]; };
        const bool cat5 = ch == cp;
        if (cat5) {
            float* const Y5[5] = {s.ap, s.ag, s.bp, s.bg, s.g};
            r.lin_fwd_ln_cat(s.xhat, P, cp, ch, 5, Y5, fw(0), dry ? nullptr : fw(0) + (size_t)5 * ch * cp);
        } else {
            r.lin_fwd_ln(s.xhat, P, cp, ch, s.ap, fw(0));
            r.lin_fwd_ln(s.xhat, P, cp, ch, s.ag, fw(1));
            r.lin_fwd_ln(s.xhat, P, cp, ch, s.bp, fw(2));
            r.lin_fwd_ln(s.xhat, P, cp, ch, s.bg, fw(3));
        }
        float *xcm, *xn;
        if (cmf) {
            if (!dry) { ProfScope ps_(h, st, KC_TR_TRANSPOSE); launch_gate_to_cm(st, s.ap, s.ag, s.bp, s.bg, rm, s.acm, s.bcm, B, N, ch); }
            xcm = T.f(P * ch);
            xn = s.ap;
        } else {
            float* arm = T.f(P * ch); float* brm = T.f(P * ch);
            const float *ap = s.ap, *ag = s.ag, *bp = s.bp, *bg = s.bg;
            r.ew(P * ch, [=] __device__(long long e) {
                const long long row = e / ch; const int j = (int)(row % N); const long long bi = row / N; const long long b = bi / N;
                const float m = rm[bi] * rm[b * N + j];
                arm[e] = ap[e] * m / (1.0f + expf(-ag[e]));
                brm[e] = bp[e] * m / (1.0f + expf(-bg[e]));
            });
            r.transpose(arm, s.acm, B, N * N, ch, true); r.transpose(brm, s.bcm, B, N * N, ch, true);
            xcm = arm; xn = arm;
        }
        {
            GemmP g{s.acm, s.bcm, xcm, nullptr, N, N, N, 0, 0, 0, 0, N, 1, B * ch, ch, (long long)ch * N * N, (long long)N * N,
                    (long long)ch * N * N, (long long)N * N, (long long)ch * N * N, (long long)N * N, 1, 1.0f, 0};
            if (outgoing) { g.am = N; g.ak = 1; g.bk = 1; g.bn = N; }
            else { g.am = 1; g.ak = N; g.bk = N; g.bn = 1; }
            r.gemm(g);
        }
        (void)xn;
        if (cmf) {
            if (!dry) { ProfScope ps_(h, st, KC_TR_LN); launch_ln_from_cm(st, xcm, Wd + t.lno_g, Wd + t.lno_b, nullptr, s.xhat_o, s.rstd_o, B, N * N, ch); }
        } else {
            float* xrm = T.f(P * ch);
            r.transpose(xcm, xrm, B, N * N, ch, false);
            r.ln_fwd(xrm, t.lno_g, t.lno_b, nullptr, s.xhat_o, s.rstd_o, P, ch);
        }
        r.lin_fwd_ln(s.xhat_o, P, ch, cp, s.u, fw(5));
        if (!cat5) r.lin_fwd_ln(s.xhat, P, cp, cp, s.g, fw(4));
        {
            float *u = s.u, *g = s.g;
            if (cp % 4 == 0) {
                r.ew(P * cp / 4, [=] __device__(long long e4) {
                    const long long e = e4 * 4, row = e / cp; const int c = (int)(e % cp);
                    const int j = (int)(row % N); const long long b = row / ((long long)N * N);
                    float4 gv = *reinterpret_cast<const float4*>(g + e);
                    const float4 uv = *reinterpret_cast<const float4*>(u + e);
                    float4 zv = *reinterpret_cast<const float4*>(z + e);
                    gv.x = 1.0f / (1.0f + expf(-gv.x)); gv.y = 1.0f / (1.0f + expf(-gv.y)); gv.z = 1.0f / (1.0f + expf(-gv.z)); gv.w = 1.0f / (1.0f + expf(-gv.w));
                    *reinterpret_cast<float4*>(g + e) = gv;
                    const uint64_t di = (uint64_t)((b * N + j) * cp + c);
                    const bool dr = r_tri > 0.f;
// ... 453 lines not shown
```

genie2_amd/csrc/pair_kernels.hip:

```cpp
#include "common.h"

#define LDZ 132


template <bool AMAX = false>
__device__ __forceinline__ float load_tile64(float* tile, const float* __restrict__ src, size_t row_stride,
                                             int nvalid, int tid) {
    const int c4 = tid & 31;
    const int r0 = tid >> 5;
    float4 v[8];
    const int last = max(nvalid - 1, 0);
#pragma unroll
    for (int u = 0; u < 8; ++u) {
        const int r = min(r0 + 8 * u, last);
        v[u] = *reinterpret_cast<const float4*>(src + (size_t)r * row_stride + c4 * 4);
    }
#pragma unroll
    for (int u = 0; u < 8; ++u) {
        const int r = r0 + 8 * u;
        if (r >= nvalid) v[u] = make_float4(0.f, 0.f, 0.f, 0.f);
        *reinterpret_cast<float4*>(tile + r * LDZ + c4 * 4) = v[u];
    }
    float am = 0.f;
    if constexpr (AMAX) {
// ... 36 lines not shown
    };
    auto gload = [&](int w, int kc) {
        int mi, i0, j0;
        decode(w, mi, i0, j0);
        const int mclamp = min(mi, n_mat - 1);
        const int mbase = mclamp * NP * NP * 4 + kc * 128;
#pragma unroll
        for (int u = 0; u < NU; ++u) {
            const int ia = min(i0 + 32 * u, NP - 32), jb = min(j0 + 32 * u, NP - 32);
            rA[u] = __builtin_bit_cast(v4, __builtin_amdgcn_raw_buffer_load_b128(ra, vload, mbase + ia * NP * 4, 0));
            rB[u] = __builtin_bit_cast(v4, __builtin_amdgcn_raw_buffer_load_b128(rb, vload, mbase + jb * NP * 4, 0));
            if (i0 + 32 * u >= NP) rA[u] = v4{0.f, 0.f, 0.f, 0.f};
            if (j0 + 32 * u >= NP) rB[u] = v4{0.f, 0.f, 0.f, 0.f};
        }
    };
    auto swrite = [&](int buf) {
        float* sa = sm + buf * 2 * TM * LDK + slds;
#pragma unroll
        for (int u = 0; u < NU; ++u) {
            *reinterpret_cast<v4*>(sa + 32 * u * LDK) = rA[u];
            *reinterpret_cast<v4*>(sa + TM * LDK + 32 * u * LDK) = rB[u];
        }
    };

    f32x16 acc[WT][WT];
#pragma unroll
    for (int m = 0; m < WT; ++m)
#pragma unroll
        for (int n = 0; n < WT; ++n) acc[m][n] = zero16();

    int w = blockIdx.x;
    if (w >= n_tiles) return;
    const int my_tiles = (n_tiles - 1 - w) / gridDim.x + 1;
    const int total = my_tiles * nk;
    gload(w, 0);
    swrite(0);
    __syncthreads();
    int kc = 0;
    for (int it = 0; it < total; ++it) {
        const bool last_chunk = kc == nk - 1;
        const int wn_next = last_chunk ? w + gridDim.x : w;
        const int kc_next = last_chunk ? 0 : kc + 1;
        if (it + 1 < total) gload(wn_next, kc_next);
        const float* sa = sm + (it & 1) * 2 * TM * LDK;
        const float* sb = sa + TM * LDK;
#pragma unroll
        for (int kb = 0; kb < 4; ++kb) {
            float4 af[WT], bf[WT];
#pragma unroll
            for (int m = 0; m < WT; ++m) af[m] = lfrag(sa, LDK, (wm * WT + m) * 32, kb, lane);
#pragma unroll
            for (int n = 0; n < WT; ++n) bf[n] = lfrag(sb, LDK, (wn * WT + n) * 32, kb, lane);
#pragma unroll
            for (int m = 0; m < WT; ++m)
#pragma unroll
                for (int n = 0; n < WT; ++n) acc[m][n] = mfma_8k(af[m], bf[n], acc[m][n]);
        }
        if (last_chunk) {
            int mi, i0, j0;
            decode(w, mi, i0, j0);
            if (mi < n_mat) {
                const int vst = ((4 * (lane >> 5)) * NP + (lane & 31)) * 4;
#pragma unroll
                for (int m = 0; m < WT; ++m)
#pragma unroll
                    for (int n = 0; n < WT; ++n) {
                        const int ib = i0 + (wm * WT + m) * 32, jb = j0 + (wn * WT + n) * 32;
                        if (ib < NP && jb < NP) {
                            const int sbase = ((mi * NP + ib) * NP + jb) * 4;
#pragma unroll
                            for (int r = 0; r < 16; ++r) {
                                const float v = acc[m][n][r];
                                __builtin_amdgcn_raw_buffer_store_b32(__builtin_bit_cast(unsigned, v), rx, vst,
                                                                      sbase + ((r & 3) + 8 * (r >> 2)) * NP * 4, 0);
                            }
                        }
                        acc[m][n] = zero16();
                    }
            }
        }
        if (it + 1 < total) swrite((it + 1) & 1);
        __syncthreads();
        w = wn_next;
        kc = kc_next;
    }
}

__global__ __launch_bounds__(256) void k_ipa_bias(const float* __restrict__ z, const float* __restrict__ wp,
                                                  const float* __restrict__ bias, float* __restrict__ out,
                                                  int B, int N, int LH, int rev, unsigned* pmax) {
    extern __shared__ __attribute__((aligned(16))) float sm[];
    const int tid = threadIdx.x, lane = tid & 63, wave = tid >> 6;
    const int ntile = (N + 127) >> 7;
    const int bid = rev ? (int)(gridDim.x - 1 - blockIdx.x) : (int)blockIdx.x;
    const int st = bid % ntile;
    const int i = (bid / ntile) % N;
    const int b = bid / (ntile * N);
    const int t0 = st * 128;
    const int nvalid = min(128, N - t0);
    const float* src = z + (((size_t)b * N + i) * N + t0) * 128;
    float am = load_tile64<true>(sm, src, 128, nvalid, tid);
    if (nvalid > 64) {
        am = fmaxf(am, load_tile64<true>(sm + 64 * LDZ, src + (size_t)64 * 128, 128, nvalid - 64, tid));
    } else {
        for (int u = tid; u < 64 * LDZ / 4; u += 256) reinterpret_cast<float4*>(sm + 64 * LDZ)[u] = make_float4(0.f, 0.f, 0.f, 0.f);
    }
#pragma unroll
    for (int o = 32; o > 0; o >>= 1) am = fmaxf(am, __shfl_xor(am, o));
    if (lane == 0 && __float_as_uint(am) > *reinterpret_cast<volatile unsigned*>(pmax)) atomicMax(pmax, __float_as_uint(am));
    __syncthreads();
    const int nbo = (LH + 31) >> 5;
    const int t = wave * 32 + (lane & 31);
    for (int ob = 0; ob < nbo; ++ob) {
        f32x16 acc = zero16();
#pragma unroll 4
        for (int kb = 0; kb < 16; ++kb)
            acc = mfma_8k(wfrag(wp, 16, ob, kb, lane), lfrag(sm, LDZ, wave * 32, kb, lane), acc);
#pragma unroll
        for (int r = 0; r < 16; ++r) {
            const int o = ob * 32 + acc_row(r, lane);
            if (o < LH && t < nvalid) out[(((size_t)o * B + b) * N + i) * N + t0 + t] = acc[r] + bias[o];
        }
    }
}

__device__ __forceinline__ void soft_bins(float* frow, float d, float dmin, float dstep, int nbin, float pm, int part) {
    float x[10];
    float mx = -3.0e38f;
#pragma unroll
    for (int q = 0; q < 10; ++q) {
        const int k = part + 4 * q;
        x[q] = (k < nbin) ? -4.0f * fabsf(d - (dmin + (float)k * dstep)) : -3.0e38f;
        mx = fmaxf(mx, x[q]);
    }
    mx = fmaxf(mx, __shfl_xor(mx, 1));
    mx = fmaxf(mx, __shfl_xor(mx, 2));
    float s = 0.f;
#pragma unroll
    for (int q = 0; q < 10; ++q) {
        const int k = part + 4 * q;
        x[q] = (k < nbin) ? expf(x[q] - mx) : 0.f;
        s += x[q];
    }
    s += __shfl_xor(s, 1);
    s += __shfl_xor(s, 2);
#pragma unroll
    for (int q = 0; q < 10; ++q) {
        const int k = part + 4 * q;
        if (k < nbin) frow[k] = (x[q] / s) * pm;
    }
}

#define LDF 52
template <bool TABLE>
__global__ __launch_bounds__(256) void k_pair_init(const float* __restrict__ trans, const float* __restrict__ rots,
                                                   const int8_t* __restrict__ codes, const float* __restrict__ rmask,
                                                   const uint8_t* __restrict__ fstm, const float* __restrict__ pij,
                                                   const float* __restrict__ pstatic, const float* __restrict__ wt,
                                                   float* __restrict__ p, int N, float dmin, float dstep, int nbin,
                                                   const int32_t* __restrict__ ridx, const int32_t* __restrict__ cidx,
                                                   const float* __restrict__ relpos_t, int relpos_k) {
    __shared__ __attribute__((aligned(16))) float ft[64 * LDF];
    __shared__ float pmk[64];
    __shared__ int dsel[64];
    __shared__ float same[64];
    const int tid = threadIdx.x, lane = tid & 63, wave = tid >> 6;
    const int ntile = (N + 63) >> 6;
    const int st = blockIdx.x % ntile;
    const int i = (blockIdx.x / ntile) % N;
    const int b = blockIdx.x / (ntile * N);
    const int t0 = st * 64;
    const int nvalid = min(64, N - t0);
    {
        const int jl = tid >> 2, part = tid & 3;
        float* frow = ft + jl * LDF;
        if (jl < nvalid) {
            const int j = t0 + jl;
            const float pm = rmask[b * N + i] * rmask[b * N + j];
            const float* xi = trans + ((size_t)b * N + i) * 3;
            const float* xj = trans + ((size_t)b * N + j) * 3;
            const float dx = xi[0] - xj[0], dy = xi[1] - xj[1], dz = xi[2] - xj[2];
            const float d = sqrtf(1e-10f + ((dx * dx + dy * dy) + dz * dz));
            soft_bins(frow, d, dmin, dstep, nbin, pm, part);
            if (part == 0) {
                const float* Ri = rots + ((size_t)b * N + i) * 9;
                const float* Rj = rots + ((size_t)b * N + j) * 9;
                float r[9];
#pragma unroll
                for (int a = 0; a < 3; ++a)
#pragma unroll
                    for (int c = 0; c < 3; ++c)
                        r[a * 3 + c] = Rj[a * 3 + 0] * Ri[0 * 3 + c] + Rj[a * 3 + 1] * Ri[1 * 3 + c] + Rj[a * 3 + 2] * Ri[2 * 3 + c];
                float q[4];
                const size_t pidx = ((size_t)b * N + i) * N + j;
                rot_to_quat_dev(r, codes ? (int)codes[pidx] : 0, q);
                const float f = fstm[pidx] ? 1.f : 0.f;
                frow[nbin + 0] = q[0] * pm; frow[nbin + 1] = q[1] * pm; frow[nbin + 2] = q[2] * pm; frow[nbin + 3] = q[3] * pm;
                frow[nbin + 4] = f; frow[nbin + 5] = f;
                for (int k = nbin + 6; k < 48; ++k) frow[k] = 0.f;
                pmk[jl] = pm;
                if (TABLE) {
                    const bool sc = cidx[b * N + i] == cidx[b * N + j];
                    int dd = ridx[b * N + i] - ridx[b * N + j] + relpos_k;
                    dd = max(0, min(dd, 2 * relpos_k));
                    dsel[jl] = sc ? dd : 2 * relpos_k + 1;
                    same[jl] = sc ? 1.f : 0.f;
                }
            }
        } else {
            for (int k = part; k < 48; k += 4) frow[k] = 0.f;
            if (part == 0) pmk[jl] = 0.f;
        }
    }
    __syncthreads();
    f32x16 a0 = zero16(), a1 = zero16();
#pragma unroll
    for (int kb = 0; kb < 6; ++kb) {
        const float4 w = wfrag(wt, 6, wave, kb, lane);
        a0 = mfma_8k(lfrag(ft, LDF, 0, kb, lane), w, a0);
        a1 = mfma_8k(lfrag(ft, LDF, 32, kb, lane), w, a1);
    }
    const int ch = wave * 32 + (lane & 31);
    const float pi_c = pij[((size_t)b * N + i) * 256 + ch];
    const float w_same = TABLE ? relpos_t[(2 * relpos_k + 2) * 128 + ch] : 0.f;
    const size_t prow0 = ((size_t)b * N + i) * N + t0;
#pragma unroll
    for (int r = 0; r < 16; ++r) {
#pragma unroll
        for (int hf = 0; hf < 2; ++hf) {
            const int t = acc_row(r, lane) + 32 * hf;
            if (t < nvalid) {
                const float acc = hf ? a1[r] : a0[r];
                const float pj_c = pij[((size_t)b * N + t0 + t) * 256 + 128 + ch];
                const size_t o = (prow0 + t) * 128 + ch;
                const float stat = TABLE ? (relpos_t[dsel[t] * 128 + ch] + same[t] * w_same) + 0.f : pstatic[o];
                p[o] = (acc + pi_c + pj_c + stat) * pmk[t];
            }
        }
    }
}

#define LDM 52
template <bool MOTIF>
__global__ __launch_bounds__(256) void k_pair_static(const float* __restrict__ pos, const int32_t* __restrict__ ridx,
                                                     const int32_t* __restrict__ cidx, const uint8_t* __restrict__ fsm,
                                                     const uint8_t* __restrict__ fstm, const float* __restrict__ relpos_t,
                                                     const float* __restrict__ wm, float* __restrict__ pstatic, int N,
                                                     int relpos_k, float dmin, float dstep, int nbin) {
    __shared__ __attribute__((aligned(16))) float ft[64 * LDM];
    __shared__ int dsel[64];
    __shared__ float same[64];
    const int tid = threadIdx.x, lane = tid & 63, wave = tid >> 6;
    const int ntile = (N + 63) >> 6;
    const int st = blockIdx.x % ntile;
    const int i = (blockIdx.x / ntile) % N;
    const int b = blockIdx.x / (ntile * N);
    const int t0 = st * 64;
    const int nvalid = min(64, N - t0);
    {
        const int jl = tid >> 2, part = tid & 3;
        float* frow = ft + jl * LDM;
        if (jl < nvalid) {
            const int j = t0 + jl;
            const size_t pidx = ((size_t)b * N + i) * N + j;
            if (MOTIF) {
                const float f = fstm[pidx] ? 1.f : 0.f;
                const float pm = ((fsm[b * N + i] && fsm[b * N + j]) ? 1.f : 0.f) * f;
                const float* xi = pos + ((size_t)b * N + i) * 3;
                const float* xj = pos + ((size_t)b * N + j) * 3;
                const float dx = xi[0] - xj[0], dy = xi[1] - xj[1], dz = xi[2] - xj[2];
                const float d = sqrtf(1e-10f + ((dx * dx + dy * dy) + dz * dz));
                soft_bins(frow, d, dmin, dstep, nbin, pm, part);
                if (part == 0) { frow[nbin] = f; frow[nbin + 1] = f; for (int k = nbin + 2; k < 48; ++k) frow[k] = 0.f; }
            }
            if (part == 0) {
                const bool sc = cidx[b * N + i] == cidx[b * N + j];
                int dd = ridx[b * N + i] - ridx[b * N + j] + relpos_k;
                dd = max(0, min(dd, 2 * relpos_k));
                dsel[jl] = sc ? dd : 2 * relpos_k + 1;
                same[jl] = sc ? 1.f : 0.f;
            }
        } else if (MOTIF) {
            for (int k = part; k < 48; k += 4) frow[k] = 0.f;
        }
    }
    __syncthreads();
    f32x16 a0 = zero16(), a1 = zero16();
    if (MOTIF) {
#pragma unroll
        for (int kb = 0; kb < 6; ++kb) {
            const float4 w = wfrag(wm, 6, wave, kb, lane);
            a0 = mfma_8k(lfrag(ft, LDM, 0, kb, lane), w, a0);
            a1 = mfma_8k(lfrag(ft, LDM, 32, kb, lane), w, a1);
        }
    }
    const int ch = wave * 32 + (lane & 31);
    const float w_same = relpos_t[(2 * relpos_k + 2) * 128 + ch];
    const size_t prow0 = ((size_t)b * N + i) * N + t0;
#pragma unroll
    for (int r = 0; r < 16; ++r) {
#pragma unroll
        for (int hf = 0; hf < 2; ++hf) {
            const int t = acc_row(r, lane) + 32 * hf;
            if (t < nvalid) {
                const float acc = hf ? a1[r] : a0[r];
                pstatic[(prow0 + t) * 128 + ch] = (relpos_t[dsel[t] * 128 + ch] + same[t] * w_same) + acc;
            }
        }
    }
}

__global__ void k_any_nonzero(const uint8_t* __restrict__ x, size_t n, unsigned* __restrict__ flag) {
    unsigned any = 0;
    for (size_t i = (size_t)blockIdx.x * blockDim.x + threadIdx.x; i < n; i += (size_t)gridDim.x * blockDim.x) any |= x[i];
    if (any) atomicOr(flag, 1u);
}
void launch_any_nonzero(genie_ctx* h, hipStream_t st, const uint8_t* x, size_t n, unsigned* flag) {
    ProfScope ps(h, st, KC_MISC);
    hipLaunchKernelGGL(k_any_nonzero, dim3(256), dim3(256), 0, st, x, n, flag);
}

void launch_pair_static(genie_ctx* h, hipStream_t st) {
    ProfScope ps(h, st, KC_PAIR_STATIC);
    const int N = h->N, ntile = (N + 63) / 64;
    dim3 grid(h->B * N * ntile);
    if (h->has_motif)
        hipLaunchKernelGGL(k_pair_static<true>, grid, dim3(256), 0, st, h->f_pos, h->f_ridx, h->f_cidx, h->f_fsm, h->f_fstm,
                           h->relpos_t, h->motif_w, h->pstatic, N, h->d.relpos_k, h->d.template_dist_min,
                           h->d.template_dist_step, h->d.template_dist_n_bin);
    else
        hipLaunchKernelGGL(k_pair_static<false>, grid, dim3(256), 0, st, h->f_pos, h->f_ridx, h->f_cidx, h->f_fsm, h->f_fstm,
                           h->relpos_t, h->motif_w, h->pstatic, N, h->d.relpos_k, h->d.template_dist_min,
                           h->d.template_dist_step, h->d.template_dist_n_bin);
}

void launch_pair_init(genie_ctx* h, hipStream_t st, const float* trans, const float* rots, const int8_t* codes) {
    ProfScope ps(h, st, KC_PAIR_INIT);
    const int N = h->N, ntile = (N + 63) / 64;
    if (!h->has_motif)
        hipLaunchKernelGGL(k_pair_init<true>, dim3(h->B * N * ntile), dim3(256), 0, st, trans, rots, codes, h->rmaskf, h->f_fstm,
                           h->pij, h->pstatic, h->templ_w, h->p, N, h->d.template_dist_min, h->d.template_dist_step,
                           h->d.template_dist_n_bin, h->f_ridx, h->f_cidx, h->relpos_t, h->d.relpos_k);
    else
        hipLaunchKernelGGL(k_pair_init<false>, dim3(h->B * N * ntile), dim3(256), 0, st, trans, rots, codes, h->rmaskf, h->f_fstm,
                           h->pij, h->pstatic, h->templ_w, h->p, N, h->d.template_dist_min, h->d.template_dist_step,
                           h->d.template_dist_n_bin, h->f_ridx, h->f_cidx, h->relpos_t, h->d.relpos_k);
}

void launch_trimul_proj_wl(genie_ctx* h, hipStream_t st, const TriMulW& w, bool outgoing);
void launch_trimul_out_wl(genie_ctx* h, hipStream_t st, const TriMulW& w);
void launch_pair_transition_wl(genie_ctx* h, hipStream_t st, const PairLayerW& w);

void launch_trimul_hx(genie_ctx* h, hipStream_t st, const TriMulW& w, bool outgoing);
void launch_trimul(genie_ctx* h, hipStream_t st, const TriMulW& w, bool outgoing) {
    if (h->hx) { launch_trimul_hx(h, st, w, outgoing); return; }
    const int NP = h->NP;
    {
        ProfScope ps(h, st, KC_TRIMUL_PROJ);
        launch_trimul_proj_wl(h, st, w, outgoing);
    }
    {
        ProfScope ps(h, st, KC_TRIMUL_CONTRACT);
        const int BC = h->B * h->d.c_hidden_mul;
        const unsigned cm_bytes = (unsigned)((size_t)BC * NP * NP * 4);
        static int num_cu = 0;
        if (!num_cu) { int dev = 0; hipDeviceProp_t pr; (void)hipGetDevice(&dev); (void)hipGetDeviceProperties(&pr, dev); num_cu = pr.multiProcessorCount > 0 ? pr.multiProcessorCount : 256; }
        if (NP >= 128) {
            const int tiles = (NP + 127) / 128;
            const int n_tiles = tiles * tiles * ((BC + 7) / 8) * 8;
            const size_t lds = 2 * 2 * 128 * LDK * sizeof(float);
            hipLaunchKernelGGL(k_trimul_contract<2>, dim3(n_tiles < 2 * num_cu ? n_tiles : 2 * num_cu), dim3(256), lds, st, h->acm,
                               h->bcm, h->xcm, NP, BC, cm_bytes);
        } else {
            const int tiles = (NP + 63) / 64;
            const int n_tiles = tiles * tiles * ((BC + 7) / 8) * 8;
            const size_t lds = 2 * 2 * 64 * LDK * sizeof(float);
            hipLaunchKernelGGL(k_trimul_contract<1>, dim3(n_tiles < 4 * num_cu ? n_tiles : 4 * num_cu), dim3(256), lds, st, h->acm,
                               h->bcm, h->xcm, NP, BC, cm_bytes);
        }
    }
    {
        ProfScope ps(h, st, KC_TRIMUL_OUT);
        launch_trimul_out_wl(h, st, w);
    }
}

void launch_pair_transition_hx(genie_ctx* h, hipStream_t st, const PairLayerW& w);
void launch_pair_transition(genie_ctx* h, hipStream_t st, const PairLayerW& w) {
    ProfScope ps(h, st, KC_PAIR_TRANSITION);
    if (h->hx) launch_pair_transition_hx(h, st, w);
    else launch_pair_transition_wl(h, st, w);
}

bool launch_ipa_bias_hx(genie_ctx* h, hipStream_t st);
void launch_ipa_bias(genie_ctx* h, hipStream_t st) {
    ProfScope ps(h, st, KC_IPA_BIAS);
    if (launch_ipa_bias_hx(h, st)) return;
    const int N = h->N, ntile = (N + 127) / 128;
    const int LH = h->d.n_structure_layer * h->d.n_head_ipa;
    const size_t lds = 128 * LDZ * sizeof(float);
    (void)hipMemsetAsync(h->pmax, 0, sizeof(unsigned), st);
    hipLaunchKernelGGL(k_ipa_bias, dim3(h->B * N * ntile), dim3(256), lds, st, h->p, h->ipa_bias_w, h->ipa_bias_b, h->ipa_bias,
                       h->B, N, LH, h->hx ? (int)(h->hx_launches & 1) : 0, h->pmax);
}

void pair_wl_kernels_init();
void pair_hx_kernels_init();
void pair_kernels_init() {
    pair_wl_kernels_init();
    pair_hx_kernels_init();
    (void)hipFuncSetAttribute(reinterpret_cast<const void*>(k_trimul_contract<2>), hipFuncAttributeMaxDynamicSharedMemorySize,
                        2 * 2 * 128 * LDK * sizeof(float));
    (void)hipFuncSetAttribute(reinterpret_cast<const void*>(k_ipa_bias), hipFuncAttributeMaxDynamicSharedMemorySize,
                        128 * LDZ * sizeof(float));
}
```

genie2_amd/csrc/single_kernels.hip:

```cpp
#include <algorithm>
#include <type_traits>
#include "hx.h"

__global__ void k_single_input(float* __restrict__ x, int ldx, const float* __restrict__ pos_tab, int n_pos, int c_pos,
                               const float* __restrict__ chain_tab, int n_chain, int c_chain,
                               const float* __restrict__ t_tab, int c_t, const int32_t* __restrict__ timesteps,
                               const int32_t* __restrict__ ridx, const int32_t* __restrict__ cidx,
                               const int32_t* __restrict__ aatype, const uint8_t* __restrict__ fsm,
                               const uint8_t* __restrict__ ifm, int N, int n_timestep) {
    const int row = blockIdx.x;
    const int b = row / N;
    float* xr = x + (size_t)row * ldx;
    const int ri = min(max(ridx[row], 0), n_pos - 1);
    const int ci = min(max(cidx[row], 0), n_chain - 1);
    const int ts = min(max(timesteps[b], 0), n_timestep);
    const float f = fsm[row] ? 1.f : 0.f;
    const int o1 = c_pos, o2 = o1 + c_chain, o3 = o2 + c_t, o4 = o3 + 20;
    for (int c = threadIdx.x; c < ldx; c += blockDim.x) {
        float v;
        if (c < o1) v = pos_tab[(size_t)ri * c_pos + c];
        else if (c < o2) v = chain_tab[(size_t)ci * c_chain + (c - o1)];
        else if (c < o3) v = t_tab[(size_t)ts * c_t + (c - o2)];
        else if (c < o4) v = (float)aatype[(size_t)row * 20 + (c - o3)] * f;
        else if (c < o4 + 2) v = f;
// ... 823 lines not shown
            const float mean = row16_sum(sum) / (float)C;
            float ss = 0.f;
#pragma unroll
            for (int q = 0; q < C / 64; ++q) {
                const float dx = v[q].x - mean, dy = v[q].y - mean, dz = v[q].z - mean, dw = v[q].w - mean;
                ss += (dx * dx + dy * dy) + (dz * dz + dw * dw);
            }
            const float rstd = 1.0f / sqrtf(row16_sum(ss) / (float)C + GENIE_LN_EPS);
#pragma unroll
            for (int q = 0; q < C / 64; ++q) {
                const int c = 64 * q + 4 * l16;
                const float4 gq = *reinterpret_cast<const float4*>(g + c), bq = *reinterpret_cast<const float4*>(bta + c);
                float4 y;
                y.x = (v[q].x - mean) * rstd * gq.x + bq.x; y.y = (v[q].y - mean) * rstd * gq.y + bq.y;
                y.z = (v[q].z - mean) * rstd * gq.z + bq.z; y.w = (v[q].w - mean) * rstd * gq.w + bq.w;
                *reinterpret_cast<float4*>(T + rrow * SR_LD + c) = y;
                if (gout && r0 + rrow < M) *reinterpret_cast<float4*>(gout + (size_t)(r0 + rrow) * C + c) = y;
            }
        }
        __syncthreads();
    };

    auto dpp_max = [](float m, auto ctrl_tag) {
        constexpr int CTRL = decltype(ctrl_tag)::value;
        return fmaxf(m, __builtin_bit_cast(float, __builtin_amdgcn_update_dpp(0, __builtin_bit_cast(int, m), CTRL, 0xf, 0xf, false)));
    };
    auto split_store = [&](float4 v, int row, int kc) {
        float m = fmaxf(fmaxf(fabsf(v.x), fabsf(v.y)), fmaxf(fabsf(v.z), fabsf(v.w)));
        m = dpp_max(m, std::integral_constant<int, 0xB1>{});
        m = dpp_max(m, std::integral_constant<int, 0x4E>{});
        m = dpp_max(m, std::integral_constant<int, 0x124>{});
        m = dpp_max(m, std::integral_constant<int, 0x128>{});
        const int e = (int)((__builtin_bit_cast(unsigned, m) >> 23) & 255u);
        const bool tiny = e < 16;
        const float sc = tiny ? 1.0f : __builtin_bit_cast(float, (unsigned)(268 - e) << 23);
        const float isc = tiny ? 1.0f : __builtin_bit_cast(float, (unsigned)(e - 14) << 23);
        unsigned h01, l01, h23, l23;
        hx_split2(v.x, v.y, sc, h01, l01);
        hx_split2(v.z, v.w, sc, h23, l23);
        unsigned char* d = sa + kc * (2 * 32 * GH_ROWB) + row * GH_ROWB + l16 * 8;
        *reinterpret_cast<uint2*>(d) = make_uint2(h01, h23);
        *reinterpret_cast<uint2*>(d + 32 * GH_ROWB) = make_uint2(l01, l23);
        if (l16 == 0) sinv[kc * 32 + row] = isc;
    };

    auto linear = [&](const float* A, const unsigned char* __restrict__ Wx, const unsigned char* Wnext, float inv_sw,
                      const float* bias, bool relu, const float* res, float* out) {
        const unsigned char* wb = Wx + (size_t)wsel * KC * 2048;
#pragma unroll
        for (int i = 0; i < 32 * (C / 4) / NT; ++i) {
            const int u = tid + i * NT, rc = u >> 4, row = rc / NKC, kc = rc - row * NKC;
            split_store(*reinterpret_cast<const float4*>(A + row * SR_LD + kc * 64 + l16 * 4), row, kc);
        }
        __syncthreads();
        f32x16 acc = zero16();
        const int foff = (lane & 31) * GH_ROWB + (lane >> 5) * 16;
#pragma unroll 1
        for (int kc = 0; kc < NKC; ++kc) {
            const unsigned char* cur = sa + kc * (2 * 32 * GH_ROWB) + foff;
            f32x16 part = zero16();
#pragma unroll
            for (int q = 0; q < 4; ++q) {
                const h8 ah = *reinterpret_cast<const h8*>(cur + q * 32);
                const h8 al = *reinterpret_cast<const h8*>(cur + 32 * GH_ROWB + q * 32);
                wf_wait<2 * SR_PD - 2>(wh[q], wl[q]);
                const h8 bh = __builtin_bit_cast(h8, wh[q]), bl = __builtin_bit_cast(h8, wl[q]);
                MFH3(ah, al, bh, bl, part);
                __builtin_amdgcn_sched_barrier(0);
                unit_issue(wb, wh[q], wl[q], kc * 4 + q + SR_PD);
            }
            const float* si = sinv + kc * 32 + 4 * (lane >> 5);
#pragma unroll
            for (int g = 0; g < 4; ++g) {
                const float4 iv = *reinterpret_cast<const float4*>(si + 8 * g);
                acc[4 * g] = fmaf(part[4 * g], iv.x, acc[4 * g]); acc[4 * g + 1] = fmaf(part[4 * g + 1], iv.y, acc[4 * g + 1]);
                acc[4 * g + 2] = fmaf(part[4 * g + 2], iv.z, acc[4 * g + 2]); acc[4 * g + 3] = fmaf(part[4 * g + 3], iv.w, acc[4 * g + 3]);
            }
        }
#pragma unroll
        for (int u = 0; u < SR_PD; ++u) wf_wait<0>(wh[u], wl[u]);
        if (Wnext) ring_fill(Wnext);
        const int col = wave * 32 + (lane & 31);
        const float bc = bias[col];
#pragma unroll
        for (int r = 0; r < 16; ++r) {
            const int row = acc_row(r, lane);
            float v = fmaf(acc[r], inv_sw, bc);
            if (relu) v = fmaxf(v, 0.f);
            if (res) v += res[row * SR_LD + col];
            out[row * SR_LD + col] = v;
        }
        __syncthreads();
    };

    layernorm(T0, g1, be1, nullptr);
    linear(T0, W1, W2, i1, b1, true, nullptr, T1);
    linear(T1, W2, W3, i2, b2, true, nullptr, T1);
    linear(T1, W3, nullptr, i3, b3, false, T0, T1);
    for (int u = tid; u < 6 * C / 4; u += NT)
        reinterpret_cast<float4*>(T0)[u] = reinterpret_cast<const float4*>(bbw)[u];
    layernorm(T1, g2, be2, s_out);

    if (splitter) {
        float acc[6] = {0.f, 0.f, 0.f, 0.f, 0.f, 0.f};
#pragma unroll
        for (int q = 0; q < C / 64; ++q) {
            const int c = 64 * q + 4 * l16;
            const float4 xv = *reinterpret_cast<const float4*>(T1 + rrow * SR_LD + c);
#pragma unroll
            for (int o = 0; o < 6; ++o) {
                const float4 wv = *reinterpret_cast<const float4*>(T0 + o * C + c);
                acc[o] += (xv.x * wv.x + xv.y * wv.y) + (xv.z * wv.z + xv.w * wv.w);
            }
        }
#pragma unroll
        for (int o = 0; o < 6; ++o) acc[o] = row16_sum(acc[o]) + bbb[o];
        const int row = r0 + rrow;
        if (l16 == 0 && row < M) {
            const float qb = acc[0], qc = acc[1], qd = acc[2];
            const float den = sqrtf(((qb * qb + qc * qc) + qd * qd) + 1.0f);
            const float a = 1.0f / den, bq = qb / den, c = qc / den, d = qd / den;
            float U[9];
            U[0] = a * a + bq * bq - c * c - d * d; U[1] = 2 * bq * c - 2 * a * d;          U[2] = 2 * bq * d + 2 * a * c;
            U[3] = 2 * bq * c + 2 * a * d;          U[4] = a * a - bq * bq + c * c - d * d; U[5] = 2 * c * d - 2 * a * bq;
            U[6] = 2 * bq * d - 2 * a * c;          U[7] = 2 * c * d + 2 * a * bq;          U[8] = a * a - bq * bq - c * c + d * d;
            float* R = rots + (size_t)row * 9;
            float* t = trans + (size_t)row * 3;
            float Rn[9], rr[9];
#pragma unroll
            for (int k = 0; k < 9; ++k) rr[k] = frm[rrow * 12 + k];
#pragma unroll
            for (int xx = 0; xx < 3; ++xx)
#pragma unroll
                for (int y = 0; y < 3; ++y) Rn[xx * 3 + y] = rr[xx * 3 + 0] * U[0 * 3 + y] + rr[xx * 3 + 1] * U[1 * 3 + y] + rr[xx * 3 + 2] * U[2 * 3 + y];
            const float tx = rr[0] * acc[3] + rr[1] * acc[4] + rr[2] * acc[5] + frm[rrow * 12 + 9];
            const float ty = rr[3] * acc[3] + rr[4] * acc[4] + rr[5] * acc[5] + frm[rrow * 12 + 10];
            const float tz = rr[6] * acc[3] + rr[7] * acc[4] + rr[8] * acc[5] + frm[rrow * 12 + 11];
#pragma unroll
            for (int k = 0; k < 9; ++k) R[k] = Rn[k];
            t[0] = tx; t[1] = ty; t[2] = tz;
            if (z_out) {
                z_out[(size_t)row * 3 + 0] = trans_in[(size_t)row * 3 + 0] - tx * inv_rescale;
                z_out[(size_t)row * 3 + 1] = trans_in[(size_t)row * 3 + 1] - ty * inv_rescale;
                z_out[(size_t)row * 3 + 2] = trans_in[(size_t)row * 3 + 2] - tz * inv_rescale;
            }
        }
    }
}

__global__ __launch_bounds__(256) void k_p_sample_frenet(int mode, float* __restrict__ trans, float* __restrict__ rots,
                                                         const float* __restrict__ z, const float* __restrict__ eps,
                                                         const int32_t* __restrict__ rmask, const int32_t* __restrict__ cidx,
                                                         int N, float alpha, float sqrt_alpha, float somac, float sqrt_beta,
                                                         float scale, float a, float bz, float c_scaled) {
    extern __shared__ __attribute__((aligned(16))) float sm[];
    float* x = sm;
    float* tv = x + 3 * N;
    float* base = tv + 3 * N;
    float* st1 = base + 9 * N;
    __shared__ int s_len;
    const int b = blockIdx.x, tid = threadIdx.x;
    float* tr = trans + (size_t)b * N * 3;
    if (tid == 0) s_len = 0;
    __syncthreads();
    int cnt = 0;
    for (int n = tid; n < N; n += 256) cnt += rmask[b * N + n];
    atomicAdd(&s_len, cnt);
    if (mode == 1) {
        const float w_z = (1.0f - alpha) / somac;
        const float inv_sa = 1.0f / sqrt_alpha;
        for (int u = tid; u < 3 * N; u += 256) {
            const float m = (float)rmask[b * N + u / 3];
            float v = inv_sa * (tr[u] - w_z * z[(size_t)b * N * 3 + u]);
            v = v * m;
            if (eps) { v = v + scale * sqrt_beta * eps[(size_t)b * N * 3 + u]; v = v * m; }
            x[u] = v;
            tr[u] = v;
        }
    } else if (mode == 2) {
        for (int u = tid; u < 3 * N; u += 256) {
            const float m = (float)rmask[b * N + u / 3];
            float v = a * tr[u] + bz * z[(size_t)b * N * 3 + u];
            v = v * m;
            if (eps) { v = v + c_scaled * eps[(size_t)b * N * 3 + u]; v = v * m; }
            x[u] = v;
            tr[u] = v;
        }
    } else {
        for (int u = tid; u < 3 * N; u += 256) x[u] = tr[u];
    }
    __syncthreads();
    const int len = s_len;
    for (int n = tid; n < N - 1; n += 256) {
        const float dx = x[3 * n + 3] - x[3 * n], dy = x[3 * n + 4] - x[3 * n + 1], dz = x[3 * n + 5] - x[3 * n + 2];
        const float nr = sqrtf(1e-10f + ((dx * dx + dy * dy) + dz * dz));
        tv[3 * n] = dx / nr; tv[3 * n + 1] = dy / nr; tv[3 * n + 2] = dz / nr;
    }
    __syncthreads();
    for (int n = tid; n < N; n += 256) {
        float R[9] = {1.f, 0.f, 0.f, 0.f, 1.f, 0.f, 0.f, 0.f, 1.f};
        if (n >= 1 && n < len - 1) {
            const int m = n - 1;
            const float ax = tv[3 * m], ay = tv[3 * m + 1], az = tv[3 * m + 2];
            const float bx = tv[3 * m + 3], by = tv[3 * m + 4], bz = tv[3 * m + 5];
            float cx = ay * bz - az * by, cy = az * bx - ax * bz, cz = ax * by - ay * bx;
            const float nr = sqrtf(1e-10f + ((cx * cx + cy * cy) + cz * cz));
            cx /= nr; cy /= nr; cz /= nr;
            const float nx = cy * bz - cz * by, ny = cz * bx - cx * bz, nz = cx * by - cy * bx;
            R[0] = bx; R[1] = cx; R[2] = nx;
            R[3] = by; R[4] = cy; R[5] = ny;
            R[6] = bz; R[7] = cz; R[8] = nz;
        }
#pragma unroll
        for (int k = 0; k < 9; ++k) base[9 * n + k] = R[k];
    }
    __syncthreads();
    const int32_t* ch = cidx + b * N;
    for (int n = tid; n < N; n += 256) {
        int srcn = n;
        if (n < len && (n == 0 || ch[n] != ch[n - 1])) srcn = n + 1;
#pragma unroll
        for (int k = 0; k < 9; ++k) st1[9 * n + k] = (srcn < N) ? base[9 * srcn + k] : ((k % 4 == 0) ? 1.f : 0.f);
    }
    __syncthreads();
    float* ro = rots + (size_t)b * N * 9;
    for (int n = tid; n < N; n += 256) {
        int k = n;
        if (n < len) {
            while (k >= 0 && (k == len - 1 || ch[k] != ch[k + 1])) --k;
            if (k < 0) k = N - 1;
        }
#pragma unroll
        for (int q = 0; q < 9; ++q) ro[9 * n + q] = st1[9 * k + q];
    }
}

__global__ void k_fill_i32(int32_t* p, int n, int v) {
    const int i = blockIdx.x * blockDim.x + threadIdx.x;
    if (i < n) p[i] = v;
}

__global__ void k_scale_copy(const float* __restrict__ in, float* __restrict__ out, int n, float s) {
    const int i = blockIdx.x * blockDim.x + threadIdx.x;
    if (i < n) out[i] = in[i] * s;
}

template <int H, int C, int PQ, int PV, int Q, int MF>
__global__ __launch_bounds__(MF ? 128 * Q : 512, MF ? 4 : 1) void k_ipa_attn_q(const float* __restrict__ proj, int ldp, const float* __restrict__ kT,
                                                    const float* __restrict__ v, const float* __restrict__ qp,
                                                    const float* __restrict__ kpT, const float* __restrict__ vp,
                                                    const float* __restrict__ bias, const float* __restrict__ z,
                                                    const float* __restrict__ rots, const float* __restrict__ trans,
                                                    const float* __restrict__ rmask, const float* __restrict__ head_w,
                                                    float* __restrict__ cat, int B, int N, int layer, int rev,
                                                    const unsigned* __restrict__ pmax, int b0,
                                                    const float* __restrict__ vf, const float* __restrict__ vmax) {
    constexpr int NT = MF ? 128 * Q : 512;
    constexpr int CP = 128, HC = H * C, NQP = H * PQ * 3, NPT = H * PV * 3, NCAT = HC + H * PV * 4 + H * CP, HH = H / (NT / 256);
    static_assert(H % (NT / 256) == 0 && C % 4 == 0 && HC + NPT <= 512, "shape");
    static_assert(!MF || H <= 16, "matrix-pipe o_pair: 2 Q waves = Q queries x 2 channel halves");
    extern __shared__ __attribute__((aligned(16))) float sm[];
    const int NP8 = (N + 7) & ~7;
    const int NPA = NP8 + 4;
    float* att = sm;
    float* sq = att + Q * H * NPA;
    float* sqp = sq + Q * HC;
    float* shw = sqp + Q * NQP;
    float* opt = shw + 16;
    float* red = opt + Q * NPT;
    const int tid = threadIdx.x, lane = tid & 63, wave = tid >> 6;
    const int groups = (N + Q - 1) / Q;
    const int bid = rev ? (int)(gridDim.x - 1 - blockIdx.x) : (int)blockIdx.x;
    const int b = b0 + bid / groups, i0 = (bid % groups) * Q;
    const int nq = min(Q, N - i0);
    for (int u = tid; u < Q * HC; u += NT) { const int q = u / HC; sq[u] = proj[(size_t)(b * N + min(i0 + q, N - 1)) * ldp + (u - q * HC)]; }
    for (int u = tid; u < Q * NQP; u += NT) { const int q = u / NQP; sqp[u] = qp[(size_t)(b * N + min(i0 + q, N - 1)) * NQP + (u - q * NQP)]; }
    if (tid < H) {
        const float g = head_w[tid];
        const float sp = (g > 20.f) ? g : log1pf(expf(g));
        shw[tid] = sp * sqrtf(1.0f / (3.0f * ((float)PQ * 9.0f / 2.0f)));
    }
    __syncthreads();
    const float s_qk = sqrtf(1.0f / (3.0f * (float)C)), s_b = sqrtf(1.0f / 3.0f);
    {
        const int hg = tid >> 8;
        for (int j = tid & 255; j < NP8; j += 256) {
            const int jc = min(j, N - 1);
            const float mj = rmask[b * N + jc];
            float sqm[Q];
#pragma unroll
            for (int q = 0; q < Q; ++q) sqm[q] = 1e5f * (rmask[b * N + min(i0 + q, N - 1)] * mj - 1.0f);
#pragma unroll 1
            for (int h2 = 0; h2 < HH; ++h2) {
                const int hh = hg * HH + h2;
                const float* kc = kT + (((size_t)b * H + hh) * C) * N + jc;
                float kv[C];
#pragma unroll
                for (int c = 0; c < C; ++c) kv[c] = kc[(size_t)c * N];
                const float* kp = kpT + ((((size_t)b * H + hh) * PQ) * 3) * N + jc;
                float kpv[PQ * 3];
#pragma unroll
                for (int c = 0; c < PQ * 3; ++c) kpv[c] = kp[(size_t)c * N];
                float bia[Q];
#pragma unroll
                for (int q = 0; q < Q; ++q) bia[q] = bias[((((size_t)layer * H + hh) * B + b) * N + min(i0 + q, N - 1)) * N + jc];
                const float hw = shw[hh];
#pragma unroll
                for (int q = 0; q < Q; ++q) {
                    const float* qv = sq + q * HC + hh * C;
                    float qk = 0.f;
#pragma unroll
                    for (int c = 0; c < C; ++c) qk += qv[c] * kv[c];
                    float a = qk * s_qk;
                    a += s_b * bia[q];
                    const float* qpv = sqp + q * NQP + hh * PQ * 3;
                    float pt = 0.f;
#pragma unroll
                    for (int pp = 0; pp < PQ; ++pp) {
                        const float dx = qpv[pp * 3 + 0] - kpv[pp * 3 + 0];
                        const float dy = qpv[pp * 3 + 1] - kpv[pp * 3 + 1];
                        const float dz = qpv[pp * 3 + 2] - kpv[pp * 3 + 2];
                        pt += ((dx * dx + dy * dy) + dz * dz) * hw;
                    }
                    a += pt * (-0.5f);
                    a += sqm[q];
                    att[(q * H + hh) * NPA + j] = (j < N) ? a : -3.0e38f;
                }
            }
        }
    }
    __syncthreads();
    {
        auto dpp = [](float m, auto ctrl_tag) {
            constexpr int CTRL = decltype(ctrl_tag)::value;
            return __builtin_bit_cast(float, __builtin_amdgcn_update_dpp(0, __builtin_bit_cast(int, m), CTRL, 0xf, 0xf, false));
        };
        const int l16 = lane & 15;
        for (int rr = wave * 4 + (lane >> 4); rr < Q * H; rr += NT / 16) {
            float* ar = att + rr * NPA;
            float mx = -3.0e38f;
            for (int j = 4 * l16; j < NP8; j += 64) {
                const float4 v = *reinterpret_cast<const float4*>(ar + j);
                mx = fmaxf(mx, fmaxf(fmaxf(v.x, v.y), fmaxf(v.z, v.w)));
            }
            mx = fmaxf(mx, dpp(mx, std::integral_constant<int, 0xB1>{})); mx = fmaxf(mx, dpp(mx, std::integral_constant<int, 0x4E>{}));
            mx = fmaxf(mx, dpp(mx, std::integral_constant<int, 0x124>{})); mx = fmaxf(mx, dpp(mx, std::integral_constant<int, 0x128>{}));
            float sum = 0.f;
            for (int j = 4 * l16; j < NP8; j += 64) {
                float4 v = *reinterpret_cast<const float4*>(ar + j);
                v.x = expf(v.x - mx); v.y = expf(v.y - mx); v.z = expf(v.z - mx); v.w = expf(v.w - mx);
                *reinterpret_cast<float4*>(ar + j) = v;
                sum += (v.x + v.y) + (v.z + v.w);
            }
            sum += dpp(sum, std::integral_constant<int, 0xB1>{}); sum += dpp(sum, std::integral_constant<int, 0x4E>{});
            sum += dpp(sum, std::integral_constant<int, 0x124>{}); sum += dpp(sum, std::integral_constant<int, 0x128>{});
            for (int j = 4 * l16; j < NP8; j += 64) {
                float4 v = *reinterpret_cast<const float4*>(ar + j);
                v.x /= sum; v.y /= sum; v.z /= sum; v.w /= sum;
                *reinterpret_cast<float4*>(ar + j) = v;
            }
        }
    }
    __syncthreads();
    constexpr int JP = MF ? (NT / 64 >= H ? 1 : 2) : 1;
    constexpr int PARTS = JP;
    float* osum = opt + Q * NPT;
    if constexpr (MF) {
        static_assert(Q <= 16 && Q % 4 == 0 && C == 16 && PV * 3 <= 32 && (JP == 1 || ((NT / 64) % JP == 0 && H % (NT / 64 / JP) == 0)), "matrix-pipe o / o_pt");
        constexpr int HG = JP == 1 ? H : NT / 64 / JP, HL = H / HG, NBK = 1 + (PV * 3 + 15) / 16;
        const int KS = (N + 31) >> 5, ksm = (KS + JP - 1) / JP;
        const int hg = wave / JP, jh = wave % JP, m = lane & 15, g = lane >> 4;
        const int ks0 = jh * ksm, nks = hg < HG ? max(min(KS - ks0, ksm), 0) : 0, nit = nks * HL;
        float mv = 0.f, mp = 0.f;
        for (int j = lane; j < (N + 7) >> 3; j += 64) {
            const float2 t = *reinterpret_cast<const float2*>(vmax + ((size_t)b * ((N + 7) >> 3) + j) * 2);
            mv = fmaxf(mv, t.x); mp = fmaxf(mp, t.y);
        }
#pragma unroll
        for (int o = 32; o > 0; o >>= 1) { mv = fmaxf(mv, __shfl_xor(mv, o)); mp = fmaxf(mp, __shfl_xor(mp, o)); }
        const int exv = min(max((int)((__float_as_uint(mv) >> 23) & 0xff), 28), 254), exp_ = min(max((int)((__float_as_uint(mp) >> 23) & 0xff), 28), 254);
        const float sv = __uint_as_float((unsigned)(267 - exv) << 23), sp = __uint_as_float((unsigned)(267 - exp_) << 23);
        const float iv = __uint_as_float((unsigned)(exv - 27) << 23), ip = __uint_as_float((unsigned)(exp_ - 27) << 23);
        const float sa = (m < Q) ? 16384.0f : 0.0f;
        const float* ar = att + (size_t)min(m, Q - 1) * H * NPA + 8 * g;
        const float* vb = vf + ((size_t)b * H * NBK * KS) * 512 + lane * 8;
        f32x4 acc[NBK];
// ... 163 lines not shown
    for (int q = 0; q < nq; ++q) {
        const int row = b * N + i0 + q;
        float4 acc[H];
#pragma unroll
        for (int hh = 0; hh < H; ++hh) acc[hh] = make_float4(0.f, 0.f, 0.f, 0.f);
        const float* zr = z + ((size_t)row * N) * CP + c4 * 4;
        const float* aq = att + q * H * NPA;
        for (int jb = jg * 8; jb < NP8; jb += 128) {
            float4 zz[8];
#pragma unroll
            for (int k = 0; k < 8; ++k) zz[k] = *reinterpret_cast<const float4*>(zr + (size_t)min(jb + k, N - 1) * CP);
#pragma unroll
            for (int hh = 0; hh < H; ++hh) {
                const float4 a0 = *reinterpret_cast<const float4*>(aq + hh * NPA + jb), a1 = *reinterpret_cast<const float4*>(aq + hh * NPA + jb + 4);
                const float a[8] = {a0.x, a0.y, a0.z, a0.w, a1.x, a1.y, a1.z, a1.w};
#pragma unroll
                for (int k = 0; k < 8; ++k) {
                    acc[hh].x += a[k] * zz[k].x; acc[hh].y += a[k] * zz[k].y; acc[hh].z += a[k] * zz[k].z; acc[hh].w += a[k] * zz[k].w;
                }
            }
        }
#pragma unroll
        for (int hh = 0; hh < H; ++hh) {
            acc[hh].x += __shfl_xor(acc[hh].x, 32); acc[hh].y += __shfl_xor(acc[hh].y, 32);
            acc[hh].z += __shfl_xor(acc[hh].z, 32); acc[hh].w += __shfl_xor(acc[hh].w, 32);
        }
        if (wave < 4 && lane < 32) {
#pragma unroll
            for (int hh = 0; hh < H; ++hh) *reinterpret_cast<float4*>(red + ((size_t)wave * H + hh) * CP + c4 * 4) = acc[hh];
        }
        __syncthreads();
        if (wave >= 4 && lane < 32) {
#pragma unroll
            for (int hh = 0; hh < H; ++hh) {
                float4* pr = reinterpret_cast<float4*>(red + ((size_t)(wave - 4) * H + hh) * CP + c4 * 4);
                float4 t = *pr;
                t.x += acc[hh].x; t.y += acc[hh].y; t.z += acc[hh].z; t.w += acc[hh].w;
                *pr = t;
            }
        }
        __syncthreads();
        {
            float* op = cat + (size_t)row * NCAT + HC + H * PV * 4;
            constexpr int tot = H * CP;
            for (int u = tid; u < tot; u += 512) op[u] = (red[u] + red[tot + u]) + (red[2 * tot + u] + red[3 * tot + u]);
        }
        __syncthreads();
    }
    }
    if constexpr (PARTS == 2) {
        for (int u = tid; u < nq * (HC + NPT); u += NT) {
            const int q = u / (HC + NPT), col = u - q * (HC + NPT);
            const float sum = osum[q * (HC + NPT) + col] + osum[(Q + q) * (HC + NPT) + col];
            if (col < HC) cat[(size_t)(b * N + i0 + q) * NCAT + col] = sum;
            else opt[q * NPT + (col - HC)] = sum;
        }
        __syncthreads();
    }
    {
        constexpr int np = H * PV;
        for (int u = tid; u < nq * np; u += NT) {
            const int q = u / np, w = u - q * np;
            const int row = b * N + i0 + q;
            const float* R = rots + (size_t)row * 9;
            const float* t = trans + (size_t)row * 3;
            const float* o3 = opt + q * NPT + w * 3;
            const float x = o3[0] - t[0], y = o3[1] - t[1], zc = o3[2] - t[2];
            const float lx = R[0] * x + R[3] * y + R[6] * zc;
            const float ly = R[1] * x + R[4] * y + R[7] * zc;
            const float lz = R[2] * x + R[5] * y + R[8] * zc;
            float* crow = cat + (size_t)row * NCAT;
            crow[HC + w] = lx;
            crow[HC + np + w] = ly;
            crow[HC + 2 * np + w] = lz;
            crow[HC + 3 * np + w] = sqrtf(((lx * lx + ly * ly) + lz * lz) + 1e-8f);
        }
    }
}

__global__ void k_q_sample(const float* __restrict__ x0, const float* __restrict__ z, const float* __restrict__ c0,
                           const float* __restrict__ c1, float* __restrict__ out, int n_per_b, int total) {
    const int u = blockIdx.x * blockDim.x + threadIdx.x;
    if (u < total) { const int b = u / n_per_b; out[u] = c0[b] * x0[u] + c1[b] * z[u]; }
}

__global__ __launch_bounds__(256) void k_training_loss(const float* __restrict__ zp, const float* __restrict__ z,
                                                       const int32_t* __restrict__ rmask, const uint8_t* __restrict__ fsm, int B, int N,
                                                       float w, float* __restrict__ losses, float* __restrict__ stats, float* __restrict__ grad) {
    __shared__ float red[4][4];
    const int b = blockIdx.x, tid = threadIdx.x, lane = tid & 63, wave = tid >> 6;
    float v[4] = {0.f, 0.f, 0.f, 0.f};
    for (int n = tid; n < N; n += 256) {
        const size_t o = ((size_t)b * N + n) * 3;
        const float dx = zp[o] - z[o], dy = zp[o + 1] - z[o + 1], dz = zp[o + 2] - z[o + 2];
        const float err = sqrtf(1e-10f + ((dx * dx + dy * dy) + dz * dz));
        const float m = (float)rmask[b * N + n], f = fsm[b * N + n] ? 1.f : 0.f;
        const float mc = m * f, mi = m * (1.f - f);
        v[0] += err * mc; v[1] += err * mi; v[2] += mc; v[3] += mi;
    }
#pragma unroll
    for (int k = 0; k < 4; ++k) {
#pragma unroll
        for (int o = 32; o > 0; o >>= 1) v[k] += __shfl_xor(v[k], o);
        if (lane == 0) red[wave][k] = v[k];
    }
    __syncthreads();
#pragma unroll
    for (int k = 0; k < 4; ++k) v[k] = (red[0][k] + red[1][k]) + (red[2][k] + red[3][k]);
    if (tid == 0) {
        losses[2 + b] = v[0]; losses[2 + B + b] = v[1];
        stats[2 * b] = (v[0] + v[1]) / (v[2] + v[3]);
        stats[2 * b + 1] = (w * v[0] + v[1]) / (w * v[2] + v[3]);
    }
    if (grad) {
        const float coef = 1.0f / ((float)B * (w * v[2] + v[3]));
        for (int n = tid; n < N; n += 256) {
            const size_t o = ((size_t)b * N + n) * 3;
            const float dx = zp[o] - z[o], dy = zp[o + 1] - z[o + 1], dz = zp[o + 2] - z[o + 2];
            const float err = sqrtf(1e-10f + ((dx * dx + dy * dy) + dz * dz));
            const float m = (float)rmask[b * N + n], f = fsm[b * N + n] ? 1.f : 0.f;
            const float g = coef * (w * m * f + m * (1.f - f)) / err;
            grad[o] = g * dx; grad[o + 1] = g * dy; grad[o + 2] = g * dz;
        }
    }
}
__global__ void k_training_loss_mean(const float* __restrict__ stats, int B, float* __restrict__ losses) {
    if (threadIdx.x == 0) {
        float u = 0.f, wl = 0.f;
        for (int b = 0; b < B; ++b) { u += stats[2 * b]; wl += stats[2 * b + 1]; }
        losses[0] = u / (float)B; losses[1] = wl / (float)B;
    }
}

__global__ __launch_bounds__(256) void k_adam(float* __restrict__ p, const float* __restrict__ g, float* __restrict__ m,
                                              float* __restrict__ v, size_t n, float omb1, float b2, float omb2, float eps,
                                              float step_size, float sqrt_bc2) {
    for (size_t i = (size_t)blockIdx.x * 256 + threadIdx.x; i < n; i += (size_t)gridDim.x * 256) {
        const float gi = g[i];
        const float mi = m[i] + (gi - m[i]) * omb1;
        const float vi = v[i] * b2 + omb2 * (gi * gi);
        m[i] = mi; v[i] = vi;
        const float denom = sqrtf(vi) / sqrt_bc2 + eps;
        p[i] = p[i] - step_size * (mi / denom);
    }
}
void launch_adam(hipStream_t st, size_t n, float* p, const float* g, float* m, float* v, double lr, double b1, double b2, double eps,
                 int step) {
    const double bc1 = 1.0 - pow(b1, step), bc2 = 1.0 - pow(b2, step);
    const size_t blocks = (n + 255) / 256;
    hipLaunchKernelGGL(k_adam, dim3((unsigned)(blocks < 4096 ? blocks : 4096)), dim3(256), 0, st, p, g, m, v, n,
                       (float)(1.0 - b1), (float)b2, (float)(1.0 - b2), (float)eps, (float)(lr / bc1), (float)sqrt(bc2));
}

void launch_single_input(genie_ctx* h, hipStream_t st, const int32_t* timesteps) {
    ProfScope ps(h, st, KC_SINGLE_INPUT);
    const genie_dims_t& d = h->d;
    const int ldx = (d.c_pos_emb + d.c_chain_emb + d.c_timestep_emb + 23 + 7) / 8 * 8;
    hipLaunchKernelGGL(k_single_input, dim3(h->B * h->N), dim3(256), 0, st, h->xsingle, ldx, h->pos_tab, h->n_pos, d.c_pos_emb,
                       h->chain_tab, h->n_chain, d.c_chain_emb, h->t_tab, d.c_timestep_emb, timesteps, h->f_ridx, h->f_cidx,
                       h->f_aatype, h->f_fsm, h->f_ifm, h->N, d.n_timestep);
}

void launch_gemm_rows(genie_ctx* h, hipStream_t st, const float* A, int lda, int M, int K, const float* Wp, int Nout,
                      const float* bias, const float* res, int ldr, const float* rowmask, int relu, float* out, int ldo, int prof_class) {
    ProfScope ps(h, st, prof_class);
    dim3 grid((M + 31) / 32, (Nout + 127) / 128);
    if (h->hx) {
        for (int i = 0; i < h->n_hxg; ++i)
            if (h->hxg[i].w == Wp) {
                hipLaunchKernelGGL(k_gemm_rows_hx, grid, dim3(256), 0, st, A, lda, M, K, h->hxg[i].img, Nout, h->hxg[i].inv_s, bias, res,
                                   ldr, rowmask, relu, out, ldo, (size_t)0);
                return;
            }
    }
    hipLaunchKernelGGL(k_gemm_rows, grid, dim3(256), 0, st, A, lda, M, K, Wp, Nout, bias, res, ldr, rowmask, relu, out, ldo);
}

void launch_layernorm_rows(genie_ctx* h, hipStream_t st, const float* in, float* out, int M, int C, const float* g,
                           const float* b) {
    ProfScope ps(h, st, KC_LAYERNORM);
    hipLaunchKernelGGL(k_layernorm_rows, dim3((M + 3) / 4), dim3(256), 0, st, in, out, M, C, g, b);
}

static bool ipa_attn_mfma_av(const genie_ctx* h);
void launch_ipa_prep(genie_ctx* h, hipStream_t st, int b0, int nb) {
    ProfScope ps(h, st, KC_IPA_PREP);
    const genie_dims_t& d = h->d;
    if (nb < 0) { b0 = 0; nb = h->B; }
    const int ldp = d.n_head_ipa * (3 * d.c_hidden_ipa + 3 * d.n_qk_point + 3 * (d.n_qk_point + d.n_v_point));
    if (ipa_attn_mfma_av(h)) {
        hipLaunchKernelGGL(k_ipa_prep_frag, dim3(nb * ((h->N + 7) / 8)), dim3(256), 0, st, h->proj, ldp, h->rots_w, h->trans_w, h->kT, h->qp,
                           h->kpT, h->vf, h->vmax, h->N, d.n_head_ipa, d.c_hidden_ipa, d.n_qk_point, d.n_v_point, b0);
        return;
    }
    hipLaunchKernelGGL(k_ipa_prep, dim3(nb * h->N), dim3(256), 0, st, h->proj, ldp, h->rots_w, h->trans_w, h->kT, h->v, h->qp,
                       h->kpT, h->vp, h->N, d.n_head_ipa, d.c_hidden_ipa, d.n_qk_point, d.n_v_point, b0 * h->N);
}

static bool ipa_is_base(const genie_dims_t& d) {
    return d.n_head_ipa == 12 && d.c_hidden_ipa == 16 && d.n_qk_point == 4 && d.n_v_point == 8 && d.c_p == 128;
}
#define IPA_Q 4
static size_t ipa_attn_t1_lds(const genie_dims_t& d, int N) {
    return ((size_t)d.n_head_ipa * ((N + 7) & ~7) + 4 * d.n_head_ipa * d.c_p + d.n_head_ipa * d.n_v_point * 3) * sizeof(float);
}
static size_t ipa_attn_q_lds(const genie_dims_t& d, int N, bool mf = false);
static bool ipa_use_q(const genie_dims_t& d, int N) { return ipa_attn_q_lds(d, N) <= 160 * 1024; }
static size_t ipa_attn_t_lds(const genie_dims_t& d, int N) { return ipa_use_q(d, N) ? ipa_attn_q_lds(d, N) : ipa_attn_t1_lds(d, N); }
static size_t ipa_attn_q_lds(const genie_dims_t& d, int N, bool mf) {
    const size_t H = d.n_head_ipa, Q = IPA_Q;
    return (Q * H * (((N + 7) & ~7) + 4) + Q * H * d.c_hidden_ipa + Q * H * d.n_qk_point * 3 + 16 +
            Q * H * d.n_v_point * 3 + (mf ? 0 : 4 * H * d.c_p) +
            (mf ? 2 * Q * H * (d.c_hidden_ipa + 3 * d.n_v_point) : 0)) * sizeof(float);
}
size_t ipa_attn_lds(const genie_dims_t& d, int N) {
    if (ipa_is_base(d)) return ipa_attn_t_lds(d, N);
    return ((size_t)d.n_head_ipa * N + 8 * d.n_head_ipa * d.c_p + d.n_head_ipa * d.n_v_point * 3) * sizeof(float);
}

static bool ipa_attn_mfma_av(const genie_ctx* h) { return h->hx && ipa_is_base(h->d) && ipa_use_q(h->d, h->N); }
size_t ipa_vf_floats(const genie_dims_t& d, int B, int N) {
    return ipa_is_base(d) ? (size_t)B * d.n_head_ipa * (1 + (3 * d.n_v_point + 15) / 16) * ((N + 31) / 32) * 512 : 64;
}
bool ipa_attn_splits(const genie_ctx* h) { return ipa_is_base(h->d) && ipa_use_q(h->d, h->N); }
void launch_ipa_attn(genie_ctx* h, hipStream_t st, int layer, const float* head_w, int b0, int nb) {
    ProfScope ps(h, st, KC_IPA_ATTN);
    const genie_dims_t& d = h->d;
    if (nb < 0 || !ipa_attn_splits(h)) { b0 = 0; nb = h->B; }
    const int ldp = d.n_head_ipa * (3 * d.c_hidden_ipa + 3 * d.n_qk_point + 3 * (d.n_qk_point + d.n_v_point));
    if (ipa_is_base(d) && !ipa_use_q(d, h->N)) {
        hipLaunchKernelGGL((k_ipa_attn_t<12, 16, 4, 8>), dim3(h->B * h->N), dim3(256), ipa_attn_t1_lds(d, h->N), st, h->proj, ldp,
                           h->kT, h->v, h->qp, h->kpT, h->vp, h->ipa_bias, h->p, h->rots_w, h->trans_w, h->rmaskf, head_w, h->cat,
                           h->B, h->N, layer);
        return;
    }
    if (ipa_is_base(d)) {
        const dim3 grid(nb * ((h->N + IPA_Q - 1) / IPA_Q));
        const int rev = (int)((layer ^ h->hx_launches ^ 1) & 1);
        if (h->hx)
            hipLaunchKernelGGL((k_ipa_attn_q<12, 16, 4, 8, IPA_Q, 1>), grid, dim3(512), ipa_attn_q_lds(d, h->N, true), st, h->proj, ldp,
                               h->kT, h->v, h->qp, h->kpT, h->vp, h->ipa_bias, h->p, h->rots_w, h->trans_w, h->rmaskf, head_w, h->cat,
                               h->B, h->N, layer, rev, h->pmax, b0, h->vf, h->vmax);
        else
            hipLaunchKernelGGL((k_ipa_attn_q<12, 16, 4, 8, IPA_Q, 0>), grid, dim3(512), ipa_attn_q_lds(d, h->N), st, h->proj, ldp,
                               h->kT, h->v, h->qp, h->kpT, h->vp, h->ipa_bias, h->p, h->rots_w, h->trans_w, h->rmaskf, head_w, h->cat,
                               h->B, h->N, layer, rev, h->pmax, b0, nullptr, nullptr);
        return;
    }
    hipLaunchKernelGGL(k_ipa_attn, dim3(h->B * h->N), dim3(256), ipa_attn_lds(d, h->N), st, h->proj, ldp, h->kT, h->v, h->qp,
                       h->kpT, h->vp, h->ipa_bias, h->p, h->rots_w, h->trans_w, h->rmaskf, head_w, h->cat, h->B, h->N,
                       d.n_head_ipa, d.c_hidden_ipa, d.n_qk_point, d.n_v_point, d.c_p, layer);
}

void launch_bb_update(genie_ctx* h, hipStream_t st, const StructLayerW& w, const float* trans_in, float* z_out) {
    ProfScope ps(h, st, KC_BB_UPDATE);
    const int M = h->B * h->N;
    hipLaunchKernelGGL(k_bb_update, dim3((M + 3) / 4), dim3(256), 0, st, h->s, h->d.c_s, w.bb_w, w.bb_b, h->rots_w, h->trans_w,
                       M, trans_in, z_out, 1.0f / h->d.rescale);
}

static size_t struct_rows_lds() { return (size_t)2 * 32 * SR_LD * 4 + 6 * (2 * 32 * GH_ROWB + 32 * 4) + 32 * 12 * 4; }
static const HxGemmW* hx_image(const genie_ctx* h, const float* Wp) {
    for (int i = 0; i < h->n_hxg; ++i)
        if (h->hxg[i].w == Wp) return &h->hxg[i];
    return nullptr;
}
bool struct_tail_fused(const genie_ctx* h, const StructLayerW& S) {
    if (!h->hx || h->d.c_s != 384 || getenv("GENIE_NO_STRUCT_FUSE")) return false;
    return hx_image(h, S.out_w) && hx_image(h, S.t1_w) && hx_image(h, S.t2_w) && hx_image(h, S.t3_w);
}
bool launch_struct_tail(genie_ctx* h, hipStream_t st, const StructLayerW& S, const float* trans_in, float* z_out, int b0, int nb) {
    if (!struct_tail_fused(h, S)) return false;
    const HxGemmW *w0 = hx_image(h, S.out_w), *w1 = hx_image(h, S.t1_w), *w2 = hx_image(h, S.t2_w), *w3 = hx_image(h, S.t3_w);
    if (nb < 0) { b0 = 0; nb = h->B; }
    const int Mall = h->B * h->N, M = nb * h->N, cs = h->d.c_s, ncat = h->d.n_head_ipa * (h->d.c_p + h->d.c_hidden_ipa + 4 * h->d.n_v_point);
    const size_t zs = (size_t)Mall * cs, r0 = (size_t)b0 * h->N;
    {
        ProfScope ps(h, st, KC_GEMM_ROWS);
        hipLaunchKernelGGL(k_gemm_rows_hx, dim3((M + 31) / 32, (cs + 127) / 128, SR_KSPLIT), dim3(256), 0, st, h->cat + r0 * ncat, ncat, M, ncat,
                           w0->img, cs, w0->inv_s, nullptr, nullptr, 0, nullptr, 0, h->spart + r0 * cs, cs, zs);
    }
    ProfScope ps(h, st, KC_STRUCT_ROWS);
    const int nrb = (M + 31) / 32;
    hipLaunchKernelGGL((k_struct_rows_hx<12>), dim3(nrb + 64), dim3(768), struct_rows_lds(), st, h->spart + r0 * cs, SR_KSPLIT, zs, S.out_b, h->s + r0 * cs,
                       S.ln_ipa_g, S.ln_ipa_b, w1->img, w1->inv_s, S.t1_b, w2->img, w2->inv_s, S.t2_b, w3->img, w3->inv_s, S.t3_b,
                       S.ln_tr_g, S.ln_tr_b, S.bb_w, S.bb_b, h->s + r0 * cs, h->rots_w + r0 * 9, h->trans_w + r0 * 3, M, trans_in ? trans_in + r0 * 3 : nullptr,
                       z_out ? z_out + r0 * 3 : nullptr, 1.0f / h->d.rescale, nrb);
    return true;
}

void launch_q_sample(genie_ctx* h, hipStream_t st, const float* x0, const float* z, const float* c0, const float* c1, float* trans_out) {
    ProfScope ps(h, st, KC_MISC);
    const int total = h->B * h->N * 3;
    hipLaunchKernelGGL(k_q_sample, dim3((total + 255) / 256), dim3(256), 0, st, x0, z, c0, c1, trans_out, h->N * 3, total);
}
void launch_training_loss(genie_ctx* h, hipStream_t st, const float* zp, const float* z, float w, float* losses, float* grad) {
    ProfScope ps(h, st, KC_MISC);
    float* stats = h->loop_z;
    hipLaunchKernelGGL(k_training_loss, dim3(h->B), dim3(256), 0, st, zp, z, h->f_rmask, h->f_fsm, h->B, h->N, w, losses, stats, grad);
    hipLaunchKernelGGL(k_training_loss_mean, dim3(1), dim3(64), 0, st, stats, h->B, losses);
}

void launch_frenet(genie_ctx* h, hipStream_t st, int mode, int step, float scale, float* trans, float* rots, const float* z,
                   const float* eps) {
    ProfScope ps(h, st, KC_P_SAMPLE);
    float al = 1.f, sa = 1.f, so = 1.f, sb = 0.f;
    if (mode == 1) {
        const int T1 = h->d.n_timestep + 1;
        al = h->sched_host[0 * T1 + step];
        sa = h->sched_host[1 * T1 + step];
        so = h->sched_host[2 * T1 + step];
        sb = h->sched_host[3 * T1 + step];
    }
    const size_t lds = (size_t)(3 + 3 + 9 + 9) * h->N * sizeof(float);
    hipLaunchKernelGGL(k_p_sample_frenet, dim3(h->B), dim3(256), lds, st, mode, trans, rots, z, eps, h->f_rmask, h->f_cidx, h->N,
                       al, sa, so, sb, scale, 0.f, 0.f, 0.f);
}

void launch_reverse_step(genie_ctx* h, hipStream_t st, float a, float bz, float c_scaled, float* trans, float* rots, const float* z,
                         const float* eps) {
    ProfScope ps(h, st, KC_P_SAMPLE);
    const size_t lds = (size_t)(3 + 3 + 9 + 9) * h->N * sizeof(float);
    hipLaunchKernelGGL(k_p_sample_frenet, dim3(h->B), dim3(256), lds, st, 2, trans, rots, z, eps, h->f_rmask, h->f_cidx, h->N,
                       1.f, 1.f, 1.f, 0.f, 0.f, a, bz, c_scaled);
}

int genie_frenet_frames(genie_stream_t stream, int B, int N, const float* coords, const int32_t* chains, const int32_t* mask,
                        float* rots_out) {
    if (!coords || !chains || !mask || !rots_out || B < 1 || N < 2) return GENIE_E_ARG;
    const size_t lds = (size_t)24 * N * sizeof(float);
    if (lds > 160 * 1024) return GENIE_E_ARG;
    if (lds > 64 * 1024)
        (void)hipFuncSetAttribute(reinterpret_cast<const void*>(k_p_sample_frenet), hipFuncAttributeMaxDynamicSharedMemorySize, (int)lds);
    hipLaunchKernelGGL(k_p_sample_frenet, dim3(B), dim3(256), lds, (hipStream_t)stream, 0, const_cast<float*>(coords), rots_out,
                       (const float*)nullptr, (const float*)nullptr, mask, chains, N, 1.f, 1.f, 1.f, 0.f, 0.f, 0.f, 0.f, 0.f);
    return hipGetLastError() == hipSuccess ? GENIE_OK : GENIE_E_HIP;
}

void launch_fill_i32(genie_ctx* h, hipStream_t st, int32_t* p, int n, int v) {
    ProfScope ps(h, st, KC_MISC);
    hipLaunchKernelGGL(k_fill_i32, dim3((n + 255) / 256), dim3(256), 0, st, p, n, v);
}

void launch_scale_copy(genie_ctx* h, hipStream_t st, const float* in, float* out, int n, float s) {
    ProfScope ps(h, st, KC_MISC);
    hipLaunchKernelGGL(k_scale_copy, dim3((n + 255) / 256), dim3(256), 0, st, in, out, n, s);
}

void single_kernels_init(const genie_dims_t& d, int n_max) {
    (void)hipFuncSetAttribute(reinterpret_cast<const void*>(k_p_sample_frenet), hipFuncAttributeMaxDynamicSharedMemorySize,
                        (int)std::min<size_t>((size_t)24 * n_max * sizeof(float), 160 * 1024));
    (void)hipFuncSetAttribute(reinterpret_cast<const void*>(k_struct_rows_hx<12>), hipFuncAttributeMaxDynamicSharedMemorySize,
                        (int)struct_rows_lds());
    if (ipa_is_base(d)) {
        if (ipa_use_q(d, n_max)) {
            (void)hipFuncSetAttribute(reinterpret_cast<const void*>(k_ipa_attn_q<12, 16, 4, 8, IPA_Q, 0>),
                                hipFuncAttributeMaxDynamicSharedMemorySize, (int)ipa_attn_q_lds(d, n_max));
            (void)hipFuncSetAttribute(reinterpret_cast<const void*>(k_ipa_attn_q<12, 16, 4, 8, IPA_Q, 1>),
                                hipFuncAttributeMaxDynamicSharedMemorySize, (int)ipa_attn_q_lds(d, n_max, true));
        } else
            (void)hipFuncSetAttribute(reinterpret_cast<const void*>(k_ipa_attn_t<12, 16, 4, 8>), hipFuncAttributeMaxDynamicSharedMemorySize,
                                (int)ipa_attn_t1_lds(d, n_max));
    } else
        (void)hipFuncSetAttribute(reinterpret_cast<const void*>(k_ipa_attn), hipFuncAttributeMaxDynamicSharedMemorySize,
                            (int)ipa_attn_lds(d, n_max));
}
```

Baseline: 111.7 batch-steps/s.

## Prefetch next step's timestep-dependent single front on a low-priority side stream

The timestep-only front of each denoise step (single input embedding, single projection, pair-input projection, and layer-0 IPA projection) is double-buffered and launched for step t-1 on a new low-priority stream while step t's last structure layer runs. The sampler kernels also write the rescaled trans and rots work buffers directly, so the scale/copy at the start of the next step is skipped, and the s0-to-s copy is removed by reading s0 in place. The aim is to hide the front GEMMs and small per-step launches off the critical path, at the cost of extra buffers, extra events, and possible contention with the IPA and struct-tail kernels.

```diff
diff --git a/genie2_amd/csrc/common.h b/genie2_amd/csrc/common.h
--- a/genie2_amd/csrc/common.h
+++ b/genie2_amd/csrc/common.h
@@ -181,6 +181,8 @@
 
 struct HxGemmW { const float* w; const unsigned char* img; float inv_s; };
 
+struct StepFront { int32_t* tsteps; float *xsingle, *s0, *pij, *proj0; };
+
 struct genie_train_ws;
 struct genie_ctx {
     genie_dims_t d;
@@ -220,12 +222,12 @@
     float *p, *acm, *bcm, *xcm, *pstatic, *ipa_bias;
     float *spart;
     unsigned *pmax;
-    float *xsingle, *s0, *s, *s1, *s2, *h1, *h2, *pij, *proj, *cat;
+    StepFront front[2];
+    float *s, *s1, *s2, *h1, *h2, *proj, *cat;
     float *kT, *v, *qp, *kpT, *vp;
     float *vf, *vmax;
     float *ta_tb, *ta_xn, *ta_qkvg;
     float *rots_w, *trans_w;
-    int32_t* tsteps;
     float *loop_z;
 
     bool prof;
@@ -235,9 +237,10 @@
     double train_gemm_flop;
 
     hipStream_t st2; hipEvent_t ev_fork, ev_join;
-};
-
-void launch_single_input(genie_ctx* h, hipStream_t st, const int32_t* timesteps);
+    hipStream_t st3; hipEvent_t ev_gate, ev_front[2];
+};
+
+void launch_single_input(genie_ctx* h, hipStream_t st, const int32_t* timesteps, float* xsingle);
 void launch_gemm_rows(genie_ctx* h, hipStream_t st, const float* A, int lda, int M, int K,
                       const float* Wp, int Nout, const float* bias, const float* res, int ldr,
                       const float* rowmask, int relu, float* out, int ldo, int prof_class = KC_GEMM_ROWS);
@@ -245,29 +248,29 @@
                            const float* g, const float* b);
 void launch_pair_static(genie_ctx* h, hipStream_t st);
 void launch_pair_init(genie_ctx* h, hipStream_t st, const float* trans, const float* rots,
-                      const int8_t* codes);
+                      const int8_t* codes, const float* pij);
 void launch_trimul(genie_ctx* h, hipStream_t st, const TriMulW& w, bool outgoing);
 void launch_pair_transition(genie_ctx* h, hipStream_t st, const PairLayerW& w);
 void launch_triatt(genie_ctx* h, hipStream_t st, const TriAttW& w, bool starting);
 void triatt_ws_floats(const genie_dims_t& d, int B, int N, size_t* tb, size_t* xn, size_t* qkvg);
 bool launch_pair_stack_fused(genie_ctx* h, hipStream_t st, float* tap_trimul_out0, float* tap_layer0);
 void launch_ipa_bias(genie_ctx* h, hipStream_t st);
-void launch_ipa_prep(genie_ctx* h, hipStream_t st, int b0 = 0, int nb = -1);
-void launch_ipa_attn(genie_ctx* h, hipStream_t st, int layer, const float* head_w, int b0 = 0, int nb = -1);
+void launch_ipa_prep(genie_ctx* h, hipStream_t st, const float* proj, int b0 = 0, int nb = -1);
+void launch_ipa_attn(genie_ctx* h, hipStream_t st, int layer, const float* head_w, const float* proj, int b0 = 0, int nb = -1);
 size_t ipa_vf_floats(const genie_dims_t& d, int B, int N);
 bool ipa_attn_splits(const genie_ctx* h);
 void launch_q_sample(genie_ctx* h, hipStream_t st, const float* x0, const float* z, const float* c0, const float* c1, float* trans_out);
 void launch_training_loss(genie_ctx* h, hipStream_t st, const float* zp, const float* z, float w, float* losses, float* grad);
 void launch_adam(hipStream_t st, size_t n, float* p, const float* g, float* m, float* v, double lr, double b1, double b2, double eps, int step);
 void launch_any_nonzero(genie_ctx* h, hipStream_t st, const uint8_t* x, size_t n, unsigned* flag);
-bool launch_struct_tail(genie_ctx* h, hipStream_t st, const StructLayerW& S, const float* trans_in, float* z_out, int b0 = 0, int nb = -1);
+bool launch_struct_tail(genie_ctx* h, hipStream_t st, const StructLayerW& S, const float* s_in, const float* trans_in, float* z_out, int b0 = 0, int nb = -1);
 bool struct_tail_fused(const genie_ctx* h, const StructLayerW& S);
 void launch_bb_update(genie_ctx* h, hipStream_t st, const StructLayerW& w, const float* trans_in,
                       float* z_out);
 void launch_frenet(genie_ctx* h, hipStream_t st, int mode, int step, float scale, float* trans,
-                   float* rots, const float* z, const float* eps);
+                   float* rots, const float* z, const float* eps, bool to_work = false);
 void launch_reverse_step(genie_ctx* h, hipStream_t st, float a, float bz, float c_scaled, float* trans, float* rots, const float* z,
-                         const float* eps);
+                         const float* eps, bool to_work = false);
 void launch_fill_i32(genie_ctx* h, hipStream_t st, int32_t* p, int n, int v);
 void train_ws_free(genie_ctx* h);
 
diff --git a/genie2_amd/csrc/genie_api.hip b/genie2_amd/csrc/genie_api.hip
--- a/genie2_amd/csrc/genie_api.hip
+++ b/genie2_amd/csrc/genie_api.hip
@@ -119,6 +119,17 @@
         (void)hipStreamDestroy(h->st2);
         h->st2 = nullptr;
     }
+    {
+        int lo = 0, hi = 0;
+        (void)hipDeviceGetStreamPriorityRange(&lo, &hi);
+        if (hipStreamCreateWithPriority(&h->st3, hipStreamNonBlocking, lo) != hipSuccess) h->st3 = nullptr;
+    }
+    if (h->st3 && (hipEventCreateWithFlags(&h->ev_gate, hipEventDisableTiming) != hipSuccess ||
+                   hipEventCreateWithFlags(&h->ev_front[0], hipEventDisableTiming) != hipSuccess ||
+                   hipEventCreateWithFlags(&h->ev_front[1], hipEventDisableTiming) != hipSuccess)) {
+        (void)hipStreamDestroy(h->st3);
+        h->st3 = nullptr;
+    }
     *out = h;
     return GENIE_OK;
 }
@@ -140,6 +151,11 @@
     for (int i = 0; i < h->prof_n; ++i) { (void)hipEventDestroy(h->prof_recs[i].a); (void)hipEventDestroy(h->prof_recs[i].b); }
     free(h->prof_recs);
     if (h->st2) { (void)hipStreamSynchronize(h->st2); (void)hipEventDestroy(h->ev_fork); (void)hipEventDestroy(h->ev_join); (void)hipStreamDestroy(h->st2); }
+    if (h->st3) {
+        (void)hipStreamSynchronize(h->st3);
+        (void)hipEventDestroy(h->ev_gate); (void)hipEventDestroy(h->ev_front[0]); (void)hipEventDestroy(h->ev_front[1]);
+        (void)hipStreamDestroy(h->st3);
+    }
     delete[] h->pair;
     delete[] h->st;
     delete h;
@@ -574,15 +590,18 @@
     want(&h->p, P * cp * 4); want(&h->pstatic, P * cp * 4);
     want(&h->acm, (size_t)B * cp * NP * NP * 4); want(&h->bcm, (size_t)B * cp * NP * NP * 4); want(&h->xcm, (size_t)B * cp * NP * NP * 4);
     want(&h->ipa_bias, (size_t)d.n_structure_layer * H * P * 4);
-    want(&h->xsingle, M * ldx * 4);
-    want(&h->s0, M * cs * 4); want(&h->s, M * cs * 4); want(&h->s1, M * cs * 4); want(&h->s2, M * cs * 4);
+    for (StepFront& F : h->front) {
+        want(&F.tsteps, (size_t)B * 4); want(&F.xsingle, M * ldx * 4); want(&F.s0, M * cs * 4); want(&F.pij, M * 2 * cp * 4);
+        want(&F.proj0, M * ipa_proj_n(d) * 4);
+    }
+    want(&h->s, M * cs * 4); want(&h->s1, M * cs * 4); want(&h->s2, M * cs * 4);
     want(&h->h1, M * cs * 4); want(&h->h2, M * cs * 4);
-    want(&h->pij, M * 2 * cp * 4); want(&h->proj, M * ipa_proj_n(d) * 4); want(&h->cat, M * ipa_cat_n(d) * 4);
+    want(&h->proj, M * ipa_proj_n(d) * 4); want(&h->cat, M * ipa_cat_n(d) * 4);
     want(&h->kT, M * H * C * 4); want(&h->v, M * H * C * 4); want(&h->qp, M * H * Pq * 3 * 4);
     want(&h->kpT, M * H * Pq * 3 * 4); want(&h->vp, M * H * Pv * 3 * 4);
     want(&h->vf, ipa_vf_floats(d, B, N) * 4); want(&h->vmax, M * 2 * 4);
     want(&h->rots_w, M * 9 * 4); want(&h->trans_w, M * 3 * 4); want(&h->loop_z, M * 3 * 4);
-    want(&h->tsteps, (size_t)B * 4); want(&h->rmaskf, M * 4); want(&h->pmax, 4); want(&h->spart, 3 * M * cs * 4);
+    want(&h->rmaskf, M * 4); want(&h->pmax, 4); want(&h->spart, 3 * M * cs * 4);
     want(&h->f_aatype, M * 20 * 4); want(&h->f_rmask, M * 4); want(&h->f_ridx, M * 4); want(&h->f_cidx, M * 4);
     want(&h->f_pos, M * 3 * 4); want(&h->f_fsm, M); want(&h->f_fstm, P); want(&h->f_ifm, M);
     if (d.n_head_tri > 0) {
@@ -629,25 +648,39 @@
     return GENIE_OK;
 }
 
-static int denoise_internal(genie_ctx* h, hipStream_t st, const float* trans, const float* rots, const int32_t* ts_dev,
-                            const int8_t* codes, float* z_out, const genie_taps_t* taps) {
+static void launch_step_front(genie_ctx* h, hipStream_t st, const StepFront& F, const int32_t* ts_dev, int step) {
+    const genie_dims_t& d = h->d;
+    const int M = h->B * h->N, cs = d.c_s, cp = d.c_p, nproj = ipa_proj_n(d);
+    const int ldx = (single_in(d) + 7) / 8 * 8;
+    if (!ts_dev) { launch_fill_i32(h, st, F.tsteps, h->B, step); ts_dev = F.tsteps; }
+    launch_single_input(h, st, ts_dev, F.xsingle);
+    launch_gemm_rows(h, st, F.xsingle, ldx, M, ldx, h->single_w, cs, nullptr, nullptr, 0, h->rmaskf, 0, F.s0, cs);
+    launch_gemm_rows(h, st, F.s0, cs, M, cs, h->pij_w, 2 * cp, nullptr, nullptr, 0, nullptr, 0, F.pij, 2 * cp);
+    const StructLayerW& S = h->st[0];
+    launch_gemm_rows(h, st, F.s0, cs, M, cs, S.proj_w, nproj, S.proj_b, nullptr, 0, nullptr, 0, F.proj0, nproj);
+}
+
+static int denoise_internal(genie_ctx* h, hipStream_t st, const float* trans, const float* rots, const int32_t* ts_dev, int step,
+                            const int8_t* codes, float* z_out, const genie_taps_t* taps, int slot = 0, bool front_ready = false,
+                            int next_step = 0, bool frames_ready = false) {
     const genie_dims_t& d = h->d;
     const int B = h->B, N = h->N, M = B * N;
     const size_t P = (size_t)M * N;
     const int cs = d.c_s, cp = d.c_p;
-    const int ldx = (single_in(d) + 7) / 8 * 8;
+    const StepFront& F = h->front[slot];
     auto d2d = [&](void* dst, const void* src, size_t bytes) { return hipMemcpyAsync(dst, src, bytes, hipMemcpyDeviceToDevice, st); };
 
     h->hx_launches = 1;
-    launch_scale_copy(h, st, trans, h->trans_w, M * 3, d.rescale);
-    HIP_TRY(h, d2d(h->rots_w, rots, (size_t)M * 9 * 4));
-
-    launch_single_input(h, st, ts_dev);
-    launch_gemm_rows(h, st, h->xsingle, ldx, M, ldx, h->single_w, cs, nullptr, nullptr, 0, h->rmaskf, 0, h->s0, cs);
-    if (taps && taps->s) HIP_TRY(h, d2d(taps->s, h->s0, (size_t)M * cs * 4));
-
-    launch_gemm_rows(h, st, h->s0, cs, M, cs, h->pij_w, 2 * cp, nullptr, nullptr, 0, nullptr, 0, h->pij, 2 * cp);
-    launch_pair_init(h, st, h->trans_w, h->rots_w, codes);
+    if (!frames_ready) {
+        launch_scale_copy(h, st, trans, h->trans_w, M * 3, d.rescale);
+        HIP_TRY(h, d2d(h->rots_w, rots, (size_t)M * 9 * 4));
+    }
+
+    if (front_ready) HIP_TRY(h, hipStreamWaitEvent(st, h->ev_front[slot], 0));
+    else launch_step_front(h, st, F, ts_dev, step);
+    if (taps && taps->s) HIP_TRY(h, d2d(taps->s, F.s0, (size_t)M * cs * 4));
+
+    launch_pair_init(h, st, h->trans_w, h->rots_w, codes, F.pij);
     if (taps && taps->p_init) HIP_TRY(h, d2d(taps->p_init, h->p, P * cp * 4));
 
     const bool fused = launch_pair_stack_fused(h, st, taps ? taps->p_trimul_out0 : nullptr, taps ? taps->p_layer0 : nullptr);
@@ -666,8 +699,7 @@
     if (taps && taps->p) HIP_TRY(h, d2d(taps->p, h->p, P * cp * 4));
 
     launch_ipa_bias(h, st);
-    HIP_TRY(h, d2d(h->s, h->s0, (size_t)M * cs * 4));
-    if (taps && taps->states) HIP_TRY(h, d2d(taps->states, h->s0, (size_t)M * cs * 4));
+    if (taps && taps->states) HIP_TRY(h, d2d(taps->states, F.s0, (size_t)M * cs * 4));
     int n_state = 1;
     const int nproj = ipa_proj_n(d), ncat = ipa_cat_n(d);
     bool split = h->st2 && B >= 2 && M >= 1024 && ipa_attn_splits(h) && !getenv("GENIE_NO_STRUCT_SPLIT");
@@ -688,16 +720,24 @@
             for (int l = 0; l < d.n_structure_layer; ++l, ++li) {
                 const StructLayerW& S = h->st[l];
                 const bool last = li == n_layers - 1;
-                launch_gemm_rows(h, hs, h->s + r0 * cs, cs, (int)nr, cs, S.proj_w, nproj, S.proj_b, nullptr, 0, nullptr, 0, h->proj + r0 * nproj, nproj);
-                launch_ipa_prep(h, hs, b0, nb);
-                launch_ipa_attn(h, hs, l, S.head_w, b0, nb);
+                const float* s_in = li == 0 ? F.s0 : h->s;
+                const float* proj = li == 0 ? F.proj0 : h->proj;
+                if (li > 0) launch_gemm_rows(h, hs, h->s + r0 * cs, cs, (int)nr, cs, S.proj_w, nproj, S.proj_b, nullptr, 0, nullptr, 0, h->proj + r0 * nproj, nproj);
+                launch_ipa_prep(h, hs, proj, b0, nb);
+                launch_ipa_attn(h, hs, l, S.head_w, proj, b0, nb);
+                if (last && half == 0 && next_step > 0) {
+                    HIP_TRY(h, hipEventRecord(h->ev_gate, st));
+                    HIP_TRY(h, hipStreamWaitEvent(h->st3, h->ev_gate, 0));
+                    launch_step_front(h, h->st3, h->front[slot ^ 1], nullptr, next_step);
+                    HIP_TRY(h, hipEventRecord(h->ev_front[slot ^ 1], h->st3));
+                }
                 if (li == 0 && taps && taps->ipa_cat0) HIP_TRY(h, hipMemcpyAsync(taps->ipa_cat0 + r0 * ncat, h->cat + r0 * ncat, nr * ncat * 4, hipMemcpyDeviceToDevice, hs));
                 auto state_tap = [&]() -> hipError_t {
                     return (taps && taps->states) ? hipMemcpyAsync(taps->states + (size_t)(1 + li) * M * cs + r0 * cs, h->s + r0 * cs, nr * cs * 4, hipMemcpyDeviceToDevice, hs)
                                                   : hipSuccess;
                 };
-                if (launch_struct_tail(h, hs, S, last ? trans : nullptr, last ? z_out : nullptr, b0, nb)) { HIP_TRY(h, state_tap()); continue; }
-                launch_gemm_rows(h, hs, h->cat, ncat, M, ncat, S.out_w, cs, S.out_b, h->s, cs, nullptr, 0, h->s1, cs);
+                if (launch_struct_tail(h, hs, S, s_in, last ? trans : nullptr, last ? z_out : nullptr, b0, nb)) { HIP_TRY(h, state_tap()); continue; }
+                launch_gemm_rows(h, hs, h->cat, ncat, M, ncat, S.out_w, cs, S.out_b, s_in, cs, nullptr, 0, h->s1, cs);
                 launch_layernorm_rows(h, hs, h->s1, h->s2, M, cs, S.ln_ipa_g, S.ln_ipa_b);
                 launch_gemm_rows(h, hs, h->s2, cs, M, cs, S.t1_w, cs, S.t1_b, nullptr, 0, nullptr, 1, h->h1, cs);
                 launch_gemm_rows(h, hs, h->h1, cs, M, cs, S.t2_w, cs, S.t2_b, nullptr, 0, nullptr, 1, h->h2, cs);
@@ -736,7 +776,7 @@
                   const int8_t* quat_codes, float* z_out, const genie_taps_t* taps) {
     if (int rc = check_ready(h, "genie_denoise")) return rc;
     if (!trans || !rots || !timesteps || !z_out) { SET_ERR(h, "genie_denoise: null tensor"); return GENIE_E_ARG; }
-    return denoise_internal(h, (hipStream_t)stream, trans, rots, timesteps, quat_codes, z_out, taps);
+    return denoise_internal(h, (hipStream_t)stream, trans, rots, timesteps, 0, quat_codes, z_out, taps);
 }
 
 int genie_frenet(genie_handle_t h, genie_stream_t stream, const float* trans, float* rots_out) {
@@ -802,11 +842,11 @@
     }
     int it = 0;
     for (int step = first_step; step >= last_step; --step, ++it) {
-        launch_fill_i32(h, st, h->tsteps, h->B, step);
         const int8_t* codes = quat_codes ? quat_codes + (size_t)it * nn : nullptr;
-        if (int rc = denoise_internal(h, st, trans_io, rots_io, h->tsteps, codes, h->loop_z, nullptr)) return rc;
+        const int next_step = (h->st3 && step > last_step) ? step - 1 : 0;
+        if (int rc = denoise_internal(h, st, trans_io, rots_io, nullptr, step, codes, h->loop_z, nullptr, it & 1, h->st3 && it > 0, next_step, it > 0)) return rc;
         const float* eps = (step == 1) ? nullptr : noise + (size_t)(T - step + 1) * n3;
-        launch_frenet(h, st, 1, step, scale, trans_io, rots_io, h->loop_z, eps);
+        launch_frenet(h, st, 1, step, scale, trans_io, rots_io, h->loop_z, eps, step > last_step);
         if (record) HIP_TRY(h, hipMemcpyAsync(record + (size_t)it * n3, trans_io, n3 * 4, hipMemcpyDeviceToDevice, st));
     }
     HIP_TRY(h, hipGetLastError());
@@ -852,11 +892,11 @@
         launch_frenet(h, st, 0, 0, 0.f, trans_io, rots_io, nullptr, nullptr);
     }
     for (int it = 0; it < n_iter; ++it) {
-        launch_fill_i32(h, st, h->tsteps, h->B, steps[it]);
         const int8_t* codes = quat_codes ? quat_codes + (size_t)it * nn : nullptr;
-        if (int rc = denoise_internal(h, st, trans_io, rots_io, h->tsteps, codes, h->loop_z, nullptr)) return rc;
+        const int next_step = (h->st3 && it + 1 < n_iter) ? steps[it + 1] : 0;
+        if (int rc = denoise_internal(h, st, trans_io, rots_io, nullptr, steps[it], codes, h->loop_z, nullptr, it & 1, h->st3 && it > 0, next_step, it > 0)) return rc;
         const float* eps = (it == n_iter - 1) ? nullptr : noise + (size_t)(it + 1) * n3;
-        launch_reverse_step(h, st, coef[3 * it], coef[3 * it + 1], coef[3 * it + 2], trans_io, rots_io, h->loop_z, eps);
+        launch_reverse_step(h, st, coef[3 * it], coef[3 * it + 1], coef[3 * it + 2], trans_io, rots_io, h->loop_z, eps, it + 1 < n_iter);
         if (record) HIP_TRY(h, hipMemcpyAsync(record + (size_t)it * n3, trans_io, n3 * 4, hipMemcpyDeviceToDevice, st));
     }
     HIP_TRY(h, hipGetLastError());
diff --git a/genie2_amd/csrc/genie_train.hip b/genie2_amd/csrc/genie_train.hip
--- a/genie2_amd/csrc/genie_train.hip
+++ b/genie2_amd/csrc/genie_train.hip
@@ -197,8 +197,8 @@
     const int L = d.n_pair_transform_layer, SL = d.n_structure_layer;
     Arena& K = r.K; Arena& T = r.T;
 
-    if (!dry) launch_single_input(h, st, ts_dev);
-    const float* xs = h->xsingle;
+    if (!dry) launch_single_input(h, st, ts_dev, h->front[0].xsingle);
+    const float* xs = h->front[0].xsingle;
     float* tr = K.f((size_t)M * 3);
     { const float sc = d.rescale; r.ew((long long)M * 3, [=] __device__(long long i) { tr[i] = trans0[i] * sc; }); }
     float* s0 = K.f((size_t)M * cs);
diff --git a/genie2_amd/csrc/pair_kernels.hip b/genie2_amd/csrc/pair_kernels.hip
--- a/genie2_amd/csrc/pair_kernels.hip
+++ b/genie2_amd/csrc/pair_kernels.hip
@@ -212,8 +212,10 @@
 }
 
 #define LDF 52
+#define PI_LD 136
+#define PI_CHUNK 256
 template <bool TABLE>
-__global__ __launch_bounds__(256) void k_pair_init(const float* __restrict__ trans, const float* __restrict__ rots,
+__global__ __launch_bounds__(256, 4) void k_pair_init(const float* __restrict__ trans, const float* __restrict__ rots,
                                                    const int8_t* __restrict__ codes, const float* __restrict__ rmask,
                                                    const uint8_t* __restrict__ fstm, const float* __restrict__ pij,
                                                    const float* __restrict__ pstatic, const float* __restrict__ wt,
@@ -221,30 +223,38 @@
                                                    const int32_t* __restrict__ ridx, const int32_t* __restrict__ cidx,
                                                    const float* __restrict__ relpos_t, int relpos_k) {
     __shared__ __attribute__((aligned(16))) float ft[64 * LDF];
-    __shared__ float pmk[64];
-    __shared__ int dsel[64];
-    __shared__ float same[64];
+    __shared__ __attribute__((aligned(16))) float stg[32 * PI_LD];
+    __shared__ float4 qv[PI_CHUNK];
+    __shared__ float4 mt[PI_CHUNK];
+    __shared__ float fv[PI_CHUNK];
     const int tid = threadIdx.x, lane = tid & 63, wave = tid >> 6;
-    const int ntile = (N + 63) >> 6;
-    const int st = blockIdx.x % ntile;
-    const int i = (blockIdx.x / ntile) % N;
-    const int b = blockIdx.x / (ntile * N);
-    const int t0 = st * 64;
-    const int nvalid = min(64, N - t0);
-    {
-        const int jl = tid >> 2, part = tid & 3;
-        float* frow = ft + jl * LDF;
-        if (jl < nvalid) {
-            const int j = t0 + jl;
-            const float pm = rmask[b * N + i] * rmask[b * N + j];
-            const float* xi = trans + ((size_t)b * N + i) * 3;
-            const float* xj = trans + ((size_t)b * N + j) * 3;
-            const float dx = xi[0] - xj[0], dy = xi[1] - xj[1], dz = xi[2] - xj[2];
-            const float d = sqrtf(1e-10f + ((dx * dx + dy * dy) + dz * dz));
-            soft_bins(frow, d, dmin, dstep, nbin, pm, part);
-            if (part == 0) {
-                const float* Ri = rots + ((size_t)b * N + i) * 9;
-                const float* Rj = rots + ((size_t)b * N + j) * 9;
+    const int i = blockIdx.x % N;
+    const int b = blockIdx.x / N;
+    const size_t row = (size_t)b * N + i;
+    const float rm_i = rmask[row];
+    const float xi0 = trans[row * 3 + 0], xi1 = trans[row * 3 + 1], xi2 = trans[row * 3 + 2];
+    float Ri[9];
+#pragma unroll
+    for (int k = 0; k < 9; ++k) Ri[k] = rots[row * 9 + k];
+    const int ci = TABLE ? cidx[row] : 0, ri = TABLE ? ridx[row] : 0;
+    const int c4 = (tid & 31) * 4;
+    const float4 pi4 = *reinterpret_cast<const float4*>(pij + row * 256 + c4);
+    const float4 ws4 = TABLE ? *reinterpret_cast<const float4*>(relpos_t + (2 * relpos_k + 2) * 128 + c4) : make_float4(0.f, 0.f, 0.f, 0.f);
+    float4 wfr[6];
+#pragma unroll
+    for (int kb = 0; kb < 6; ++kb) wfr[kb] = wfrag(wt, 6, wave, kb, lane);
+
+    for (int c0 = 0; c0 < N; c0 += PI_CHUNK) {
+        if (c0) __syncthreads();
+        {
+            const int j = c0 + tid;
+            if (j < N) {
+                const size_t rj = (size_t)b * N + j;
+                const float pm = rm_i * rmask[rj];
+                const float* xj = trans + rj * 3;
+                const float dx = xi0 - xj[0], dy = xi1 - xj[1], dz = xi2 - xj[2];
+                const float d = sqrtf(1e-10f + ((dx * dx + dy * dy) + dz * dz));
+                const float* Rj = rots + rj * 9;
                 float r[9];
 #pragma unroll
                 for (int a = 0; a < 3; ++a)
@@ -252,49 +262,85 @@
                     for (int c = 0; c < 3; ++c)
                         r[a * 3 + c] = Rj[a * 3 + 0] * Ri[0 * 3 + c] + Rj[a * 3 + 1] * Ri[1 * 3 + c] + Rj[a * 3 + 2] * Ri[2 * 3 + c];
                 float q[4];
-                const size_t pidx = ((size_t)b * N + i) * N + j;
+                const size_t pidx = row * N + j;
                 rot_to_quat_dev(r, codes ? (int)codes[pidx] : 0, q);
-                const float f = fstm[pidx] ? 1.f : 0.f;
-                frow[nbin + 0] = q[0] * pm; frow[nbin + 1] = q[1] * pm; frow[nbin + 2] = q[2] * pm; frow[nbin + 3] = q[3] * pm;
-                frow[nbin + 4] = f; frow[nbin + 5] = f;
-                for (int k = nbin + 6; k < 48; ++k) frow[k] = 0.f;
-                pmk[jl] = pm;
+                qv[tid] = make_float4(q[0] * pm, q[1] * pm, q[2] * pm, q[3] * pm);
+                fv[tid] = fstm[pidx] ? 1.f : 0.f;
+                float same = 0.f;
+                int dsel = 0;
                 if (TABLE) {
-                    const bool sc = cidx[b * N + i] == cidx[b * N + j];
-                    int dd = ridx[b * N + i] - ridx[b * N + j] + relpos_k;
+                    const bool sc = ci == cidx[rj];
+                    int dd = ri - ridx[rj] + relpos_k;
                     dd = max(0, min(dd, 2 * relpos_k));
-                    dsel[jl] = sc ? dd : 2 * relpos_k + 1;
-                    same[jl] = sc ? 1.f : 0.f;
+                    dsel = sc ? dd : 2 * relpos_k + 1;
+                    same = sc ? 1.f : 0.f;
                 }
-            }
-        } else {
-            for (int k = part; k < 48; k += 4) frow[k] = 0.f;
-            if (part == 0) pmk[jl] = 0.f;
-        }
-    }
-    __syncthreads();
-    f32x16 a0 = zero16(), a1 = zero16();
-#pragma unroll
-    for (int kb = 0; kb < 6; ++kb) {
-        const float4 w = wfrag(wt, 6, wave, kb, lane);
-        a0 = mfma_8k(lfrag(ft, LDF, 0, kb, lane), w, a0);
-        a1 = mfma_8k(lfrag(ft, LDF, 32, kb, lane), w, a1);
-    }
-    const int ch = wave * 32 + (lane & 31);
-    const float pi_c = pij[((size_t)b * N + i) * 256 + ch];
-    const float w_same = TABLE ? relpos_t[(2 * relpos_k + 2) * 128 + ch] : 0.f;
-    const size_t prow0 = ((size_t)b * N + i) * N + t0;
-#pragma unroll
-    for (int r = 0; r < 16; ++r) {
-#pragma unroll
-        for (int hf = 0; hf < 2; ++hf) {
-            const int t = acc_row(r, lane) + 32 * hf;
-            if (t < nvalid) {
-                const float acc = hf ? a1[r] : a0[r];
-                const float pj_c = pij[((size_t)b * N + t0 + t) * 256 + 128 + ch];
-                const size_t o = (prow0 + t) * 128 + ch;
-                const float stat = TABLE ? (relpos_t[dsel[t] * 128 + ch] + same[t] * w_same) + 0.f : pstatic[o];
-                p[o] = (acc + pi_c + pj_c + stat) * pmk[t];
+                mt[tid] = make_float4(pm, same, __int_as_float(dsel), d);
+            }
+        }
+        __syncthreads();
+        const int ntl = (min(PI_CHUNK, N - c0) + 63) >> 6;
+        for (int tl = 0; tl < ntl; ++tl) {
+            const int t0 = c0 + tl * 64;
+            const int nvalid = min(64, N - t0);
+            {
+                const int jl = tid >> 2, part = tid & 3;
+                float* frow = ft + jl * LDF;
+                if (jl < nvalid) {
+                    const float4 m = mt[tl * 64 + jl];
+                    soft_bins(frow, m.w, dmin, dstep, nbin, m.x, part);
+                    if (part == 0) {
+                        const float4 q = qv[tl * 64 + jl];
+                        frow[nbin + 0] = q.x; frow[nbin + 1] = q.y; frow[nbin + 2] = q.z; frow[nbin + 3] = q.w;
+                    } else if (part == 1) {
+                        const float f = fv[tl * 64 + jl];
+                        frow[nbin + 4] = f; frow[nbin + 5] = f;
+                    } else if (part == 2) {
+                        for (int k = nbin + 6; k < 48; ++k) frow[k] = 0.f;
+                    }
+                } else {
+                    for (int k = part; k < 48; k += 4) frow[k] = 0.f;
+                }
+            }
+            __syncthreads();
+            f32x16 a0 = zero16(), a1 = zero16();
+#pragma unroll
+            for (int kb = 0; kb < 6; ++kb) {
+                a0 = mfma_8k(lfrag(ft, LDF, 0, kb, lane), wfr[kb], a0);
+                a1 = mfma_8k(lfrag(ft, LDF, 32, kb, lane), wfr[kb], a1);
+            }
+#pragma unroll
+            for (int hf = 0; hf < 2; ++hf) {
+                if (hf) __syncthreads();
+                {
+                    float* srow = stg + (4 * (lane >> 5)) * PI_LD + wave * 32 + (lane & 31);
+#pragma unroll
+                    for (int r = 0; r < 16; ++r) srow[((r & 3) + 8 * (r >> 2)) * PI_LD] = hf ? a1[r] : a0[r];
+                }
+                __syncthreads();
+#pragma unroll
+                for (int u = 0; u < 4; ++u) {
+                    const int tr = u * 8 + (tid >> 5);
+                    const int t = 32 * hf + tr;
+                    if (t < nvalid) {
+                        const float4 acc = *reinterpret_cast<const float4*>(stg + tr * PI_LD + c4);
+                        const float4 m = mt[tl * 64 + t];
+                        const float4 pj = *reinterpret_cast<const float4*>(pij + ((size_t)b * N + t0 + t) * 256 + 128 + c4);
+                        const size_t o = (row * N + t0 + t) * 128 + c4;
+                        float4 stat;
+                        if (TABLE) {
+                            const float4 rel = *reinterpret_cast<const float4*>(relpos_t + __float_as_int(m.z) * 128 + c4);
+                            stat.x = (rel.x + m.y * ws4.x) + 0.f; stat.y = (rel.y + m.y * ws4.y) + 0.f;
+                            stat.z = (rel.z + m.y * ws4.z) + 0.f; stat.w = (rel.w + m.y * ws4.w) + 0.f;
+                        } else {
+                            stat = *reinterpret_cast<const float4*>(pstatic + o);
+                        }
+                        float4 out;
+                        out.x = (acc.x + pi4.x + pj.x + stat.x) * m.x; out.y = (acc.y + pi4.y + pj.y + stat.y) * m.x;
+                        out.z = (acc.z + pi4.z + pj.z + stat.z) * m.x; out.w = (acc.w + pi4.w + pj.w + stat.w) * m.x;
+                        *reinterpret_cast<float4*>(p + o) = out;
+                    }
+                }
             }
         }
     }
@@ -394,16 +440,16 @@
                            h->d.template_dist_step, h->d.template_dist_n_bin);
 }
 
-void launch_pair_init(genie_ctx* h, hipStream_t st, const float* trans, const float* rots, const int8_t* codes) {
+void launch_pair_init(genie_ctx* h, hipStream_t st, const float* trans, const float* rots, const int8_t* codes, const float* pij) {
     ProfScope ps(h, st, KC_PAIR_INIT);
-    const int N = h->N, ntile = (N + 63) / 64;
+    const int N = h->N;
     if (!h->has_motif)
-        hipLaunchKernelGGL(k_pair_init<true>, dim3(h->B * N * ntile), dim3(256), 0, st, trans, rots, codes, h->rmaskf, h->f_fstm,
-                           h->pij, h->pstatic, h->templ_w, h->p, N, h->d.template_dist_min, h->d.template_dist_step,
+        hipLaunchKernelGGL(k_pair_init<true>, dim3(h->B * N), dim3(256), 0, st, trans, rots, codes, h->rmaskf, h->f_fstm,
+                           pij, h->pstatic, h->templ_w, h->p, N, h->d.template_dist_min, h->d.template_dist_step,
                            h->d.template_dist_n_bin, h->f_ridx, h->f_cidx, h->relpos_t, h->d.relpos_k);
     else
-        hipLaunchKernelGGL(k_pair_init<false>, dim3(h->B * N * ntile), dim3(256), 0, st, trans, rots, codes, h->rmaskf, h->f_fstm,
-                           h->pij, h->pstatic, h->templ_w, h->p, N, h->d.template_dist_min, h->d.template_dist_step,
+        hipLaunchKernelGGL(k_pair_init<false>, dim3(h->B * N), dim3(256), 0, st, trans, rots, codes, h->rmaskf, h->f_fstm,
+                           pij, h->pstatic, h->templ_w, h->p, N, h->d.template_dist_min, h->d.template_dist_step,
                            h->d.template_dist_n_bin, h->f_ridx, h->f_cidx, h->relpos_t, h->d.relpos_k);
 }
 
diff --git a/genie2_amd/csrc/single_kernels.hip b/genie2_amd/csrc/single_kernels.hip
--- a/genie2_amd/csrc/single_kernels.hip
+++ b/genie2_amd/csrc/single_kernels.hip
@@ -999,7 +999,8 @@
                                                          const float* __restrict__ z, const float* __restrict__ eps,
                                                          const int32_t* __restrict__ rmask, const int32_t* __restrict__ cidx,
                                                          int N, float alpha, float sqrt_alpha, float somac, float sqrt_beta,
-                                                         float scale, float a, float bz, float c_scaled) {
+                                                         float scale, float a, float bz, float c_scaled,
+                                                         float* __restrict__ trans_w, float* __restrict__ rots_w, float rescale) {
     extern __shared__ __attribute__((aligned(16))) float sm[];
     float* x = sm;
     float* tv = x + 3 * N;
@@ -1036,6 +1037,8 @@
     } else {
         for (int u = tid; u < 3 * N; u += 256) x[u] = tr[u];
     }
+    if (trans_w)
+        for (int u = tid; u < 3 * N; u += 256) trans_w[(size_t)b * N * 3 + u] = x[u] * rescale;
     __syncthreads();
     const int len = s_len;
     for (int n = tid; n < N - 1; n += 256) {
@@ -1079,6 +1082,9 @@
         }
 #pragma unroll
         for (int q = 0; q < 9; ++q) ro[9 * n + q] = st1[9 * k + q];
+        if (rots_w)
+#pragma unroll
+            for (int q = 0; q < 9; ++q) rots_w[(size_t)b * N * 9 + 9 * n + q] = st1[9 * k + q];
     }
 }
 
@@ -1548,11 +1554,11 @@
                        (float)(1.0 - b1), (float)b2, (float)(1.0 - b2), (float)eps, (float)(lr / bc1), (float)sqrt(bc2));
 }
 
-void launch_single_input(genie_ctx* h, hipStream_t st, const int32_t* timesteps) {
+void launch_single_input(genie_ctx* h, hipStream_t st, const int32_t* timesteps, float* xsingle) {
     ProfScope ps(h, st, KC_SINGLE_INPUT);
     const genie_dims_t& d = h->d;
     const int ldx = (d.c_pos_emb + d.c_chain_emb + d.c_timestep_emb + 23 + 7) / 8 * 8;
-    hipLaunchKernelGGL(k_single_input, dim3(h->B * h->N), dim3(256), 0, st, h->xsingle, ldx, h->pos_tab, h->n_pos, d.c_pos_emb,
+    hipLaunchKernelGGL(k_single_input, dim3(h->B * h->N), dim3(256), 0, st, xsingle, ldx, h->pos_tab, h->n_pos, d.c_pos_emb,
                        h->chain_tab, h->n_chain, d.c_chain_emb, h->t_tab, d.c_timestep_emb, timesteps, h->f_ridx, h->f_cidx,
                        h->f_aatype, h->f_fsm, h->f_ifm, h->N, d.n_timestep);
 }
@@ -1579,17 +1585,17 @@
 }
 
 static bool ipa_attn_mfma_av(const genie_ctx* h);
-void launch_ipa_prep(genie_ctx* h, hipStream_t st, int b0, int nb) {
+void launch_ipa_prep(genie_ctx* h, hipStream_t st, const float* proj, int b0, int nb) {
     ProfScope ps(h, st, KC_IPA_PREP);
     const genie_dims_t& d = h->d;
     if (nb < 0) { b0 = 0; nb = h->B; }
     const int ldp = d.n_head_ipa * (3 * d.c_hidden_ipa + 3 * d.n_qk_point + 3 * (d.n_qk_point + d.n_v_point));
     if (ipa_attn_mfma_av(h)) {
-        hipLaunchKernelGGL(k_ipa_prep_frag, dim3(nb * ((h->N + 7) / 8)), dim3(256), 0, st, h->proj, ldp, h->rots_w, h->trans_w, h->kT, h->qp,
+        hipLaunchKernelGGL(k_ipa_prep_frag, dim3(nb * ((h->N + 7) / 8)), dim3(256), 0, st, proj, ldp, h->rots_w, h->trans_w, h->kT, h->qp,
                            h->kpT, h->vf, h->vmax, h->N, d.n_head_ipa, d.c_hidden_ipa, d.n_qk_point, d.n_v_point, b0);
         return;
     }
-    hipLaunchKernelGGL(k_ipa_prep, dim3(nb * h->N), dim3(256), 0, st, h->proj, ldp, h->rots_w, h->trans_w, h->kT, h->v, h->qp,
+    hipLaunchKernelGGL(k_ipa_prep, dim3(nb * h->N), dim3(256), 0, st, proj, ldp, h->rots_w, h->trans_w, h->kT, h->v, h->qp,
                        h->kpT, h->vp, h->N, d.n_head_ipa, d.c_hidden_ipa, d.n_qk_point, d.n_v_point, b0 * h->N);
 }
 
@@ -1619,13 +1625,13 @@
     return ipa_is_base(d) ? (size_t)B * d.n_head_ipa * (1 + (3 * d.n_v_point + 15) / 16) * ((N + 31) / 32) * 512 : 64;
 }
 bool ipa_attn_splits(const genie_ctx* h) { return ipa_is_base(h->d) && ipa_use_q(h->d, h->N); }
-void launch_ipa_attn(genie_ctx* h, hipStream_t st, int layer, const float* head_w, int b0, int nb) {
+void launch_ipa_attn(genie_ctx* h, hipStream_t st, int layer, const float* head_w, const float* proj, int b0, int nb) {
     ProfScope ps(h, st, KC_IPA_ATTN);
     const genie_dims_t& d = h->d;
     if (nb < 0 || !ipa_attn_splits(h)) { b0 = 0; nb = h->B; }
     const int ldp = d.n_head_ipa * (3 * d.c_hidden_ipa + 3 * d.n_qk_point + 3 * (d.n_qk_point + d.n_v_point));
     if (ipa_is_base(d) && !ipa_use_q(d, h->N)) {
-        hipLaunchKernelGGL((k_ipa_attn_t<12, 16, 4, 8>), dim3(h->B * h->N), dim3(256), ipa_attn_t1_lds(d, h->N), st, h->proj, ldp,
+        hipLaunchKernelGGL((k_ipa_attn_t<12, 16, 4, 8>), dim3(h->B * h->N), dim3(256), ipa_attn_t1_lds(d, h->N), st, proj, ldp,
                            h->kT, h->v, h->qp, h->kpT, h->vp, h->ipa_bias, h->p, h->rots_w, h->trans_w, h->rmaskf, head_w, h->cat,
                            h->B, h->N, layer);
         return;
@@ -1634,16 +1640,16 @@
         const dim3 grid(nb * ((h->N + IPA_Q - 1) / IPA_Q));
         const int rev = (int)((layer ^ h->hx_launches ^ 1) & 1);
         if (h->hx)
-            hipLaunchKernelGGL((k_ipa_attn_q<12, 16, 4, 8, IPA_Q, 1>), grid, dim3(512), ipa_attn_q_lds(d, h->N, true), st, h->proj, ldp,
+            hipLaunchKernelGGL((k_ipa_attn_q<12, 16, 4, 8, IPA_Q, 1>), grid, dim3(512), ipa_attn_q_lds(d, h->N, true), st, proj, ldp,
                                h->kT, h->v, h->qp, h->kpT, h->vp, h->ipa_bias, h->p, h->rots_w, h->trans_w, h->rmaskf, head_w, h->cat,
                                h->B, h->N, layer, rev, h->pmax, b0, h->vf, h->vmax);
         else
-            hipLaunchKernelGGL((k_ipa_attn_q<12, 16, 4, 8, IPA_Q, 0>), grid, dim3(512), ipa_attn_q_lds(d, h->N), st, h->proj, ldp,
+            hipLaunchKernelGGL((k_ipa_attn_q<12, 16, 4, 8, IPA_Q, 0>), grid, dim3(512), ipa_attn_q_lds(d, h->N), st, proj, ldp,
                                h->kT, h->v, h->qp, h->kpT, h->vp, h->ipa_bias, h->p, h->rots_w, h->trans_w, h->rmaskf, head_w, h->cat,
                                h->B, h->N, layer, rev, h->pmax, b0, nullptr, nullptr);
         return;
     }
-    hipLaunchKernelGGL(k_ipa_attn, dim3(h->B * h->N), dim3(256), ipa_attn_lds(d, h->N), st, h->proj, ldp, h->kT, h->v, h->qp,
+    hipLaunchKernelGGL(k_ipa_attn, dim3(h->B * h->N), dim3(256), ipa_attn_lds(d, h->N), st, proj, ldp, h->kT, h->v, h->qp,
                        h->kpT, h->vp, h->ipa_bias, h->p, h->rots_w, h->trans_w, h->rmaskf, head_w, h->cat, h->B, h->N,
                        d.n_head_ipa, d.c_hidden_ipa, d.n_qk_point, d.n_v_point, d.c_p, layer);
 }
@@ -1665,7 +1671,7 @@
     if (!h->hx || h->d.c_s != 384 || getenv("GENIE_NO_STRUCT_FUSE")) return false;
     return hx_image(h, S.out_w) && hx_image(h, S.t1_w) && hx_image(h, S.t2_w) && hx_image(h, S.t3_w);
 }
-bool launch_struct_tail(genie_ctx* h, hipStream_t st, const StructLayerW& S, const float* trans_in, float* z_out, int b0, int nb) {
+bool launch_struct_tail(genie_ctx* h, hipStream_t st, const StructLayerW& S, const float* s_in, const float* trans_in, float* z_out, int b0, int nb) {
     if (!struct_tail_fused(h, S)) return false;
     const HxGemmW *w0 = hx_image(h, S.out_w), *w1 = hx_image(h, S.t1_w), *w2 = hx_image(h, S.t2_w), *w3 = hx_image(h, S.t3_w);
     if (nb < 0) { b0 = 0; nb = h->B; }
@@ -1678,7 +1684,7 @@
     }
     ProfScope ps(h, st, KC_STRUCT_ROWS);
     const int nrb = (M + 31) / 32;
-    hipLaunchKernelGGL((k_struct_rows_hx<12>), dim3(nrb + 64), dim3(768), struct_rows_lds(), st, h->spart + r0 * cs, SR_KSPLIT, zs, S.out_b, h->s + r0 * cs,
+    hipLaunchKernelGGL((k_struct_rows_hx<12>), dim3(nrb + 64), dim3(768), struct_rows_lds(), st, h->spart + r0 * cs, SR_KSPLIT, zs, S.out_b, s_in + r0 * cs,
                        S.ln_ipa_g, S.ln_ipa_b, w1->img, w1->inv_s, S.t1_b, w2->img, w2->inv_s, S.t2_b, w3->img, w3->inv_s, S.t3_b,
                        S.ln_tr_g, S.ln_tr_b, S.bb_w, S.bb_b, h->s + r0 * cs, h->rots_w + r0 * 9, h->trans_w + r0 * 3, M, trans_in ? trans_in + r0 * 3 : nullptr,
                        z_out ? z_out + r0 * 3 : nullptr, 1.0f / h->d.rescale, nrb);
@@ -1698,7 +1704,7 @@
 }
 
 void launch_frenet(genie_ctx* h, hipStream_t st, int mode, int step, float scale, float* trans, float* rots, const float* z,
-                   const float* eps) {
+                   const float* eps, bool to_work) {
     ProfScope ps(h, st, KC_P_SAMPLE);
     float al = 1.f, sa = 1.f, so = 1.f, sb = 0.f;
     if (mode == 1) {
@@ -1710,15 +1716,15 @@
     }
     const size_t lds = (size_t)(3 + 3 + 9 + 9) * h->N * sizeof(float);
     hipLaunchKernelGGL(k_p_sample_frenet, dim3(h->B), dim3(256), lds, st, mode, trans, rots, z, eps, h->f_rmask, h->f_cidx, h->N,
-                       al, sa, so, sb, scale, 0.f, 0.f, 0.f);
+                       al, sa, so, sb, scale, 0.f, 0.f, 0.f, to_work ? h->trans_w : nullptr, to_work ? h->rots_w : nullptr, h->d.rescale);
 }
 
 void launch_reverse_step(genie_ctx* h, hipStream_t st, float a, float bz, float c_scaled, float* trans, float* rots, const float* z,
-                         const float* eps) {
+                         const float* eps, bool to_work) {
     ProfScope ps(h, st, KC_P_SAMPLE);
     const size_t lds = (size_t)(3 + 3 + 9 + 9) * h->N * sizeof(float);
     hipLaunchKernelGGL(k_p_sample_frenet, dim3(h->B), dim3(256), lds, st, 2, trans, rots, z, eps, h->f_rmask, h->f_cidx, h->N,
-                       1.f, 1.f, 1.f, 0.f, 0.f, a, bz, c_scaled);
+                       1.f, 1.f, 1.f, 0.f, 0.f, a, bz, c_scaled, to_work ? h->trans_w : nullptr, to_work ? h->rots_w : nullptr, h->d.rescale);
 }
 
 int genie_frenet_frames(genie_stream_t stream, int B, int N, const float* coords, const int32_t* chains, const int32_t* mask,
@@ -1729,7 +1735,8 @@
     if (lds > 64 * 1024)
         (void)hipFuncSetAttribute(reinterpret_cast<const void*>(k_p_sample_frenet), hipFuncAttributeMaxDynamicSharedMemorySize, (int)lds);
     hipLaunchKernelGGL(k_p_sample_frenet, dim3(B), dim3(256), lds, (hipStream_t)stream, 0, const_cast<float*>(coords), rots_out,
-                       (const float*)nullptr, (const float*)nullptr, mask, chains, N, 1.f, 1.f, 1.f, 0.f, 0.f, 0.f, 0.f, 0.f);
+                       (const float*)nullptr, (const float*)nullptr, mask, chains, N, 1.f, 1.f, 1.f, 0.f, 0.f, 0.f, 0.f, 0.f,
+                       (float*)nullptr, (float*)nullptr, 1.f);
     return hipGetLastError() == hipSuccess ? GENIE_OK : GENIE_E_HIP;
 }
 
```

Result: no change. 113.4 batch-steps/s, median of 6 (+1.6%).
